# lh3/pangene

Measured on AMD Instinct MI355X. Metric: M PAF hits/sec through filter+overlap+graph, higher is better.
Workload: dtype int32

## Files before the change

include/pangene_hip.h:

```cpp
#ifndef PANGENE_HIP_H
#define PANGENE_HIP_H

#include <stddef.h>
#include <stdint.h>

#ifdef __cplusplus
extern "C" {
#endif

#define PGA_F_REV        0x001u
#define PGA_F_FLT        0x002u
#define PGA_F_ISO_SUB    0x004u
#define PGA_F_ISO_OV     0x008u
#define PGA_F_CHAIN      0x010u
#define PGA_F_PSEUDO     0x020u
#define PGA_F_VTX        0x040u
#define PGA_F_SHADOW     0x080u
#define PGA_F_REP        0x100u
#define PGA_F_WEAK_SHIFT 9
#define PGA_F_WEAK_MASK  0x600u

enum { PGA_FLT_PSEUDO = 0, PGA_FLT_VTX0 = 1, PGA_FLT_WEAK2 = 2, PGA_FLT_SHADOW = 3 };

enum {
	PGA_OK = 0,
	PGA_ERR_NO_DEVICE = -1,
	PGA_ERR_RANGE = -2,
	PGA_ERR_ARG = -3,
	PGA_ERR_NOMEM = -4,
	PGA_ERR_INVARIANT = -5
};

#define PGA_BLOCK_PLANES 10
typedef struct {
	int32_t n_hit, n_exon, n_ctg;
	int32_t max_cs, max_cm, max_score_adj;
	int32_t any_neg_score_adj, any_multi_exon;
	const int32_t *data;
	size_t n_words;
	const int32_t *vfirst;
	const int64_t *vbase;
} pga_genome_block_t;

#define PGA_ABI_VERSION 20u
typedef struct {
	uint32_t abi_version;
	int32_t n_genome;
	int32_t n_genome_global;
	const int32_t *genome_global;
	int32_t n_prot, n_gene;
	int64_t n_hit, n_exon;
	const pga_genome_block_t *block;
	const int32_t *prot_gid;
	const uint8_t *gene_pref;
} pga_shard_t;

typedef struct {
	double  min_ov_ratio;
	int32_t check_strand;
	int32_t drop_sgl_exon;
	int32_t reserved[4];
} pga_params_t;

typedef struct {
	uint32_t *flags;
	int32_t *rank, *score_dom, *pid_dom, *pid_dom0;
	int32_t *pos_x;
	int32_t *pos_y;
	uint64_t *flt_x_bits;
} pga_hit_state_t;

typedef struct {
	uint64_t x;
	int32_t  n_genome, tot_cnt;
	uint64_t sum_dist;
	int64_t  sum_s1, sum_s2;
} pga_arc_part_t;

typedef struct pga_ctx pga_ctx_t;

typedef struct {
	int64_t h1_head_tie;
	int64_t h2_cm_tie;
	int64_t h2_cs_tie;
	int64_t h3_dom_tie;
} pga_hazard_t;

#define PGA_HAZARD_CAP 4096

#define PGA_DECLARE(pfx) \
	 \
	int  pfx##_create(pga_ctx_t **ctx, const pga_shard_t *sh, const pga_params_t *par); \
	void pfx##_destroy(pga_ctx_t *ctx); \
	 \
	int  pfx##_begin(pga_ctx_t *ctx); \
	 \
	int  pfx##_ingest(pga_ctx_t *ctx, int32_t *stats); \
	 \
	int  pfx##_post_partials(pga_ctx_t *ctx, int32_t **max_ori, int64_t **sums); \
	 \
	int  pfx##_post_apply(pga_ctx_t *ctx, const uint8_t *prot_rep, const uint8_t *prot_pj, int64_t *n_pseudo); \
	 \
	int  pfx##_shadow(pga_ctx_t *ctx, int32_t cal_dom_sc, int32_t *stats); \
	 \
	int  pfx##_set_filter(pga_ctx_t *ctx, int32_t which); \
	 \
	int  pfx##_vtx_partials(pga_ctx_t *ctx, int32_t **cnt, uint64_t **records, int64_t *n_records); \
	 \
	int  pfx##_flag_vtx(pga_ctx_t *ctx, const int32_t *g2s, int32_t n_seg, int32_t then_filter); \
	 \
	int  pfx##_arc_round(pga_ctx_t *ctx, int32_t use_ori, int32_t **seg_cnt, pga_arc_part_t **arcs, int64_t *n_arcs); \
	 \
	int  pfx##_arc_merge(pga_ctx_t *ctx, const pga_arc_part_t *gathered, const int64_t *count, int32_t W, int64_t slot, \
	                     pga_arc_part_t **out, int64_t *n_out); \
	 \
	int  pfx##_arc_set_current(pga_ctx_t *ctx, const pga_arc_part_t *arcs, int64_t n_arc, int32_t n_seg, int32_t *deg); \
	 \
	int  pfx##_arc_round_local(pga_ctx_t *ctx, int32_t use_ori, int32_t n_seg, int32_t *seg_cnt, int32_t *deg); \
	int  pfx##_arc_round_finish(pga_ctx_t *ctx, int32_t n_seg, int32_t *seg_cnt, int32_t *deg);  \
	 \
	int  pfx##_arc_table(pga_ctx_t *ctx, const pga_arc_part_t **arcs, int64_t *n_arc); \
	 \
	int  pfx##_rep_pos(pga_ctx_t *ctx); \
	 \
	int  pfx##_n_local(pga_ctx_t *ctx, const int32_t *pairs, int64_t n, int32_t local_dist, int32_t local_count, \
	                   int32_t frag_mode, int32_t **cnt); \
	 \
	int  pfx##_branch_pairs(pga_ctx_t *ctx, const uint64_t *arc_x, const int32_t *arc_s1, int64_t n_arc, const int32_t *seg_gid, int32_t n_seg, \
	                        double branch_diff, int32_t local_dist, int32_t local_count, int32_t frag_mode, int32_t **cnt, int64_t *n_pairs); \
	int  pfx##_branch_decide(pga_ctx_t *ctx, double branch_diff, double branch_diff_dist, double branch_diff_cut, uint8_t *arc_weak, \
	                         int32_t *n_dist_loci, int64_t *n_flt1, int64_t *n_flt2); \
	 \
	int  pfx##_branch_decide_filter(pga_ctx_t *ctx, double branch_diff, double branch_diff_dist, double branch_diff_cut, int32_t do_filter, \
	                                int32_t max_tot_cnt, int32_t max_degree, int32_t max_dist_loci, uint8_t *del); \
	 \
	int  pfx##_mark_hits(pga_ctx_t *ctx, const uint64_t *arc_x, const uint8_t *arc_weak, int64_t n_arc, int64_t *n_marked, int32_t then_filter); \
	 \
	int  pfx##_override_order(pga_ctx_t *ctx, int32_t which, int32_t n_seg, const int32_t *seg_genome, const int32_t *seg_start, \
	                          const int64_t *seg_off, const int32_t *file_idx); \
	 \
	int  pfx##_set_head(pga_ctx_t *ctx, const int32_t *head_file); \
	 \
	int  pfx##_fetch(pga_ctx_t *ctx, void *dst_host, const void *src_backend, size_t nbytes); \
	int  pfx##_put(pga_ctx_t *ctx, void *dst_backend, const void *src_host, size_t nbytes); \
	int  pfx##_copy(pga_ctx_t *ctx, void *dst_backend, const void *src_backend, size_t nbytes); \
	 \
	int  pfx##_scratch(pga_ctx_t *ctx, size_t nbytes, void **ptr); \
	 \
	int  pfx##_sync(pga_ctx_t *ctx); \
	 \
	int  pfx##_fetch_later(pga_ctx_t *ctx, const void *src_backend, size_t nbytes, const void **host_view); \
	 \
	int  pfx##_ctg_counts(pga_ctx_t *ctx, int32_t *cnt); \
	int  pfx##_gene_matrix(pga_ctx_t *ctx, const int32_t *asm_of_ctg, int32_t n_asm, int32_t n_seg, int32_t *mat); \
	 \
	int  pfx##_download(pga_ctx_t *ctx, const pga_hit_state_t *out); \
	int  pfx##_hazards(pga_ctx_t *ctx, pga_hazard_t *out); \
	 \
	int  pfx##_hazard_segs(pga_ctx_t *ctx, int32_t *segs, int32_t cap, int64_t *n_total); \
	 \
	int  pfx##_is_device(void); \
	 \
	int  pfx##_host_alloc(size_t nbytes, void **ptr); \
	void pfx##_host_free(void *ptr); \
	const char *pfx##_strerror(int code);

PGA_DECLARE(pga)

typedef struct { int32_t bo, walk, st_off, en_off; } pga_call_rec_t;
typedef struct {
	const int32_t *step; const int64_t *walk_off; int32_t n_walk; int32_t n_seg;
	const int32_t *bub_vs, *bub_ve; int32_t n_bub;
} pga_call_in_t;
typedef struct {
	int64_t n_rec; const pga_call_rec_t *rec; const int32_t *rep, *cnt;
	int64_t n_gene; const int32_t *gene_bub, *gene_seg; const int64_t *gene_first;
} pga_call_out_t;
int pga_call_bubbles(const pga_call_in_t *in, pga_call_out_t *out);

typedef struct {
	const uint32_t *bits; const int32_t *order;
	int32_t n_gene, n_asm, n_perm;
} pga_curves_in_t;
typedef struct { const int32_t *count; } pga_curves_out_t;
int pga_pan_curves(const pga_curves_in_t *in, pga_curves_out_t *out);

typedef struct {
	const uint32_t *bits;
	int32_t n_item, n_asm;
} pga_shared_in_t;
typedef struct { const int32_t *shared; } pga_shared_out_t;
int pga_pan_shared(const pga_shared_in_t *in, pga_shared_out_t *out);

typedef struct {
	const uint32_t *bits;
	int32_t n_gene, n_asm, min_count, r_permille, sign;
	int64_t max_pair;
} pga_assoc_in_t;
typedef struct {
	int64_t n_pair;
	const int32_t *pair;
	const int32_t *count;
} pga_assoc_out_t;
int pga_pan_assoc(const pga_assoc_in_t *in, pga_assoc_out_t *out);

typedef struct {
	const uint32_t *bits;
	const uint32_t *label;
	int32_t n_gene, n_col, min_count, n_perm;
	uint32_t seed;
	uint32_t *perm_rows;
} pga_trait_in_t;
typedef struct { const int32_t *a, *s, *k; } pga_trait_out_t;
int pga_pan_trait(const pga_trait_in_t *in, pga_trait_out_t *out);
int32_t pga_trait_batch(void);

typedef struct {
	const int32_t *q;
	int32_t n, method;
} pga_join_in_t;
typedef struct { const int64_t *rec; int32_t n_rec; } pga_join_out_t;
int pga_pan_join(const pga_join_in_t *in, pga_join_out_t *out);

typedef struct {
	const uint32_t *bits;
	int32_t n_item, n_asm, metric, method;
	uint32_t seed;
	int32_t first, n_rep;
	int32_t *draws;
} pga_boot_in_t;
typedef struct { const int64_t *rec; int32_t n_rec; } pga_boot_out_t;
int pga_pan_boot(const pga_boot_in_t *in, pga_boot_out_t *out);
int32_t pga_boot_batch(int32_t n_asm);

typedef struct {
	const uint8_t *op;
	const uint32_t *bits;
	const int8_t *label;
	int32_t n_gene, n_leaf, n_row;
} pga_pairs_in_t;
typedef struct { const int32_t *out; } pga_pairs_out_t;
int pga_pan_pairs(const pga_pairs_in_t *in, pga_pairs_out_t *out);

typedef struct {
	const uint32_t *bits;
	const int16_t *c2;
	int32_t n_gene, n_col, min_count, n_perm;
	uint32_t seed;
	int16_t *perm_rows;
	int32_t *d_rows;
} pga_qtrait_in_t;
typedef struct { const int32_t *a, *d, *k; } pga_qtrait_out_t;
int pga_pan_qtrait(const pga_qtrait_in_t *in, pga_qtrait_out_t *out);
int32_t pga_qtrait_batch(void);

typedef struct {
	const int32_t *q;
	int32_t n, k, max_iter;
} pga_medoids_in_t;
typedef struct {
	const int32_t *medoid, *label, *dist, *size;
	const int64_t *sums, *rec;
	int64_t td;
	int32_t n_rec, n_swap, converged;
} pga_medoids_out_t;
int pga_pan_medoids(const pga_medoids_in_t *in, pga_medoids_out_t *out);

typedef struct {
	const int32_t *q;
	const uint32_t *label;
	int32_t n, shift, q_max, n1, n_perm;
	uint32_t seed;
	int64_t *a_rows, *b_rows;
	uint32_t *perm_rows;
} pga_permanova_in_t;
typedef struct { int64_t t, a, b, k; } pga_permanova_out_t;
int pga_pan_permanova(const pga_permanova_in_t *in, pga_permanova_out_t *out);
int32_t pga_permanova_batch(void);

typedef struct {
	const int32_t *a, *b;
	int32_t n, max_a, max_b, n_perm;
	uint32_t seed;
	int64_t *z_rows;
	uint16_t *ord_rows;
} pga_mantel_in_t;
typedef struct { int64_t z, n_ge, n_le; } pga_mantel_out_t;
int pga_pan_mantel(const pga_mantel_in_t *in, pga_mantel_out_t *out);
int32_t pga_mantel_batch(void);

typedef struct {
	const uint8_t *op;
	const uint32_t *bits;
	const int32_t *par;
	int32_t n_gene, n_leaf, gain, loss, mode;
	uint64_t *st_rows;
} pga_gainloss_in_t;
typedef struct { const int32_t *gene; const int64_t *node; } pga_gainloss_out_t;
int pga_pan_gainloss(const pga_gainloss_in_t *in, pga_gainloss_out_t *out);
int32_t pga_gainloss_chunk(int32_t n_leaf);

typedef struct {
	const uint8_t *op;
	const uint32_t *bits;
	const int32_t *par;
	int32_t n_gene, n_leaf, gain, loss, mode;
	int32_t min_events, r_permille, sign;
	int64_t max_pair;
	uint32_t *ev_rows;
	int64_t ev_cap;
} pga_coevo_in_t;
typedef struct { const int32_t *events; int64_t n_pair; const int32_t *pair; } pga_coevo_out_t;
int pga_pan_coevo(const pga_coevo_in_t *in, pga_coevo_out_t *out);
int32_t pga_coevo_chunk(int32_t n_leaf);

struct pga_branch_par_s; struct pga_loop_xchg_s;
typedef struct {
	const char *name;
	int  (*create)(pga_ctx_t **, const pga_shard_t *, const pga_params_t *);
	void (*destroy)(pga_ctx_t *);
	int  (*begin)(pga_ctx_t *);
	int  (*ingest)(pga_ctx_t *, int32_t *);
	int  (*post_partials)(pga_ctx_t *, int32_t **, int64_t **);
	int  (*post_apply)(pga_ctx_t *, const uint8_t *, const uint8_t *, int64_t *);
	int  (*shadow)(pga_ctx_t *, int32_t, int32_t *);
	int  (*set_filter)(pga_ctx_t *, int32_t);
	int  (*vtx_partials)(pga_ctx_t *, int32_t **, uint64_t **, int64_t *);
	int  (*flag_vtx)(pga_ctx_t *, const int32_t *, int32_t, int32_t);
	int  (*arc_round)(pga_ctx_t *, int32_t, int32_t **, pga_arc_part_t **, int64_t *);
	int  (*arc_merge)(pga_ctx_t *, const pga_arc_part_t *, const int64_t *, int32_t, int64_t, pga_arc_part_t **, int64_t *);
	int  (*arc_set_current)(pga_ctx_t *, const pga_arc_part_t *, int64_t, int32_t, int32_t *);
	int  (*rep_pos)(pga_ctx_t *);
	int  (*n_local)(pga_ctx_t *, const int32_t *, int64_t, int32_t, int32_t, int32_t, int32_t **);
	int  (*branch_pairs)(pga_ctx_t *, const uint64_t *, const int32_t *, int64_t, const int32_t *, int32_t, double, int32_t, int32_t, int32_t, int32_t **, int64_t *);
	int  (*branch_decide)(pga_ctx_t *, double, double, double, uint8_t *, int32_t *, int64_t *, int64_t *);
	int  (*mark_hits)(pga_ctx_t *, const uint64_t *, const uint8_t *, int64_t, int64_t *, int32_t);
	int  (*override_order)(pga_ctx_t *, int32_t, int32_t, const int32_t *, const int32_t *, const int64_t *, const int32_t *);
	int  (*set_head)(pga_ctx_t *, const int32_t *);
	int  (*fetch)(pga_ctx_t *, void *, const void *, size_t);
	int  (*put)(pga_ctx_t *, void *, const void *, size_t);
	int  (*copy)(pga_ctx_t *, void *, const void *, size_t);
	int  (*scratch)(pga_ctx_t *, size_t, void **);
	int  (*download)(pga_ctx_t *, const pga_hit_state_t *);
	int  (*hazards)(pga_ctx_t *, pga_hazard_t *);
	int  (*is_device)(void);
	const char *(*strerror)(int);
	int  (*timing_reset)(pga_ctx_t *);
	int  (*timing_get)(pga_ctx_t *, int32_t, double *, int64_t *, int64_t *);
	int  (*sync)(pga_ctx_t *);
	int  (*fetch_later)(pga_ctx_t *, const void *, size_t, const void **);
	int  (*hazard_segs)(pga_ctx_t *, int32_t *, int32_t, int64_t *);
	int  (*host_alloc)(size_t, void **);
	void (*host_free)(void *);
	int  (*arc_round_local)(pga_ctx_t *, int32_t, int32_t, int32_t *, int32_t *);
	int  (*ctg_counts)(pga_ctx_t *, int32_t *);
	int  (*gene_matrix)(pga_ctx_t *, const int32_t *, int32_t, int32_t, int32_t *);
	int  (*arc_table)(pga_ctx_t *, const pga_arc_part_t **, int64_t *);
	int  (*arc_round_finish)(pga_ctx_t *, int32_t, int32_t *, int32_t *);
	int  (*branch_decide_filter)(pga_ctx_t *, double, double, double, int32_t, int32_t, int32_t, int32_t, uint8_t *);
	int  (*branch_loop)(pga_ctx_t *, int32_t, const struct pga_branch_par_s *, const int32_t *, const int32_t *, const int32_t *, uint8_t *, const struct pga_loop_xchg_s *, int32_t *, int32_t *);
	void (*host_trim)(size_t);
	int  (*set_device)(int32_t);
	int  (*device_count)(void);
	int  (*arc_round_x)(pga_ctx_t *, int32_t, int32_t, const struct pga_loop_xchg_s *, int32_t *, int32_t *, int64_t *);
	int  (*copy_gbps)(size_t, int32_t, double *);
	int  (*warm)(void);
	int  (*reserve)(int64_t, int64_t, int32_t, int32_t, int32_t, int64_t);
	int  (*stage)(const void *, size_t);
	void (*stage_drop)(const void *);
	int  (*call_bubbles)(const pga_call_in_t *, pga_call_out_t *);
	int  (*pan_curves)(const pga_curves_in_t *, pga_curves_out_t *);
	int  (*pan_shared)(const pga_shared_in_t *, pga_shared_out_t *);
	int  (*pan_assoc)(const pga_assoc_in_t *, pga_assoc_out_t *);
	int  (*pan_trait)(const pga_trait_in_t *, pga_trait_out_t *);
	int  (*pan_join)(const pga_join_in_t *, pga_join_out_t *);
	int  (*pan_boot)(const pga_boot_in_t *, pga_boot_out_t *);
	int  (*pan_pairs)(const pga_pairs_in_t *, pga_pairs_out_t *);
	int  (*pan_qtrait)(const pga_qtrait_in_t *, pga_qtrait_out_t *);
	int  (*pan_medoids)(const pga_medoids_in_t *, pga_medoids_out_t *);
	int  (*pan_permanova)(const pga_permanova_in_t *, pga_permanova_out_t *);
	int  (*pan_mantel)(const pga_mantel_in_t *, pga_mantel_out_t *);
	int  (*final_arcs)(pga_ctx_t *, const void **, int64_t *);
	int  (*pan_gainloss)(const pga_gainloss_in_t *, pga_gainloss_out_t *);
	int  (*pan_coevo)(const pga_coevo_in_t *, pga_coevo_out_t *);
} pga_backend_t;

const pga_backend_t *pga_backend(void);

typedef struct pga_loop_xchg_s {
	void *user;
	int32_t rank, world;
	int64_t arc_cap_hint;
	int (*allreduce_i32_sum)(void *user, void *buf, int64_t count);
	int (*allgather)(void *user, const void *in, void *out, int64_t bytes_per_rank);
} pga_loop_xchg_t;
void pga_host_trim(size_t keep_bytes);
int pga_set_device(int32_t device);
int pga_device_count(void);
int pga_copy_gbps(size_t bytes, int32_t reps, double *gbps);
int pga_warm(void);

typedef struct pga_branch_par_s {
	double branch_diff, branch_diff_dist, branch_diff_cut; int32_t local_dist, local_count, frag_mode, use_ori;
	int32_t pre_on, pre_max_tot_cnt, pre_max_degree, pre_max_dist_loci;
	int32_t final_on;
} pga_branch_par_t;
int pga_arc_round_x(pga_ctx_t *ctx, int32_t use_ori, int32_t n_seg, const pga_loop_xchg_t *x, int32_t *seg_cnt, int32_t *deg, int64_t *n_arc);
int pga_branch_loop(pga_ctx_t *ctx, int32_t n_round, const pga_branch_par_t *par, const int32_t *max_tot_cnt, const int32_t *max_degree,
                    const int32_t *max_dist_loci, uint8_t *seg_alive, const pga_loop_xchg_t *x, int32_t *seg_cnt , int32_t *n_dist_loci );

int pga_final_arcs(pga_ctx_t *ctx, const void **host_view, int64_t *n_arc);

int pga_set_stream(pga_ctx_t *ctx, void *hip_stream);
void *pga_active_stream(void);

int pga_reserve(int64_t n_hit, int64_t n_exon, int32_t n_prot, int32_t n_gene, int32_t n_genome, int64_t raw_words);
int pga_stage_h2d(const void *host, size_t bytes);
void pga_stage_drop(const void *host);
int pga_timing_reset(pga_ctx_t *ctx);
int pga_timing_get(pga_ctx_t *ctx, int32_t which, double *total_ms, int64_t *n_launch, int64_t *units);

#ifdef __cplusplus
}
#endif
#endif
```

pangene_amd/csrc/hip/k_stage_b.hpp:

```cpp
#pragma once

__global__ __launch_bounds__(BLOCK) void k_post_part(const uint32_t *flags, const int32_t *pid, const int32_t *rank, const int32_t *sori, const int32_t *sadj,
                                                       const int32_t *nex, int n, int P, int32_t *max_ori, unsigned long long *sums)
{
	int h = blockIdx.x * BLOCK + threadIdx.x;
	if (h >= n) return;
	int p = pid[h];
	const int so = sori[h];
	if (max_ori[p] < so) atomicMax(&max_ori[p], so);
	if (rank[h] == 0 && !(flags[h] & PGA_F_FLT)) {
		int w = nex[h] == 1 ? 0 : 1;
		atomicAdd(&sums[p], (unsigned long long)(long long)sadj[h]);
		atomicAdd(&sums[(int64_t)(2 + w) * P + p], 1ull);
		atomicAdd(&sums[(int64_t)(4 + w) * P + p], (unsigned long long)(long long)sori[h]);
	}
}
constexpr int PP_T = 1024;
__global__ __launch_bounds__(PP_T) void k_post_part_lds(const uint32_t *flags, const int32_t *pid, const int32_t *rank, const int32_t *sori, const int32_t *sadj,
                                                          const int32_t *nex, int n, int P, int p_tiles, int PT , int32_t *max_ori, unsigned long long *sums)
{
	extern __shared__ unsigned long long pp_lds[];
	unsigned long long *s_adj = pp_lds, *s_o0 = pp_lds + PT, *s_o1 = pp_lds + 2 * (size_t)PT;
	unsigned int *s_cnt = (unsigned int *)(pp_lds + 3 * (size_t)PT);
	const int t = blockIdx.x % p_tiles, chunk = blockIdx.x / p_tiles, n_chunk = gridDim.x / p_tiles;
	const int p0 = t * PT, p1 = p0 + PT < P ? p0 + PT : P;
	for (int i = threadIdx.x; i < PT; i += PP_T) s_adj[i] = 0, s_o0[i] = 0, s_o1[i] = 0, s_cnt[i] = 0;
	__syncthreads();
	const int64_t per = ((int64_t)n + n_chunk - 1) / n_chunk, h0 = (int64_t)chunk * per, h1 = h0 + per < n ? h0 + per : n;
	for (int64_t h = h0 + threadIdx.x; h < h1; h += PP_T) {
		const int p = pid[h], so = sori[h];
		if (t == 0 && max_ori[p] < so) atomicMax(&max_ori[p], so);
		if (p < p0 || p >= p1 || rank[h] != 0 || (flags[h] & PGA_F_FLT)) continue;
		const int w = nex[h] == 1 ? 0 : 1, i = p - p0;
		atomicAdd(&s_adj[i], (unsigned long long)(long long)sadj[h]);
		{
			const unsigned old = atomicAdd(&s_cnt[i], w ? 65536u : 1u);
			if ((w ? old >> 16 : old & 0xffffu) == 0x7fffu) { atomicAdd(&sums[(int64_t)(2 + w) * P + p], 0x8000ull); atomicSub(&s_cnt[i], w ? 0x80000000u : 0x8000u); }
		}
		atomicAdd(w ? &s_o1[i] : &s_o0[i], (unsigned long long)(long long)so);
	}
	__syncthreads();
	for (int i = threadIdx.x; i < p1 - p0; i += PP_T) {
		const unsigned int cw = s_cnt[i];
		const unsigned long long a = s_adj[i], o0 = s_o0[i], o1 = s_o1[i];
		const int p = p0 + i;
		if (a) atomicAdd(&sums[p], a);
		if (cw & 0xffffu) atomicAdd(&sums[(int64_t)2 * P + p], (unsigned long long)(cw & 0xffffu));
		if (cw >> 16) atomicAdd(&sums[(int64_t)3 * P + p], (unsigned long long)(cw >> 16));
		if (o0) atomicAdd(&sums[(int64_t)4 * P + p], o0);
		if (o1) atomicAdd(&sums[(int64_t)5 * P + p], o1);
	}
}
__global__ __launch_bounds__(BLOCK) void k_post_count(unsigned long long *sums, int P)
{
	const int p = blockIdx.x * BLOCK + threadIdx.x;
	if (p < P) sums[(int64_t)P + p] = sums[(int64_t)2 * P + p] + sums[(int64_t)3 * P + p];
}

__global__ __launch_bounds__(BLOCK) void k_post_apply(uint32_t *flags, const int32_t *pid, const int32_t *nex, int32_t *sdom, int n,
                                                        const int32_t *max_ori, const uint8_t *rep, const uint8_t *pj, int64_t *cnt)
{
	int h = blockIdx.x * BLOCK + threadIdx.x;
	if (h >= n) return;
	int p = pid[h];
	int mo = max_ori[p];
	if (sdom[h] > mo) sdom[h] = mo;
	uint32_t f = flags[h], nf = rep[p] ? (f | PGA_F_REP) : (f & ~PGA_F_REP);
	if (!(f & (PGA_F_FLT | PGA_F_PSEUDO)) && nex[h] == 1 && pj[p]) {
		nf |= PGA_F_PSEUDO;
		if (cnt) atomicAdd((unsigned long long *)cnt, 1ull);
	}
	if (nf != f) flags[h] = nf;
}

__global__ __launch_bounds__(BLOCK) void k_set_filter(uint32_t *flags, int n, int which)
{
	int h = blockIdx.x * BLOCK + threadIdx.x;
	if (h >= n) return;
	uint32_t f = flags[h];
	bool hit = which == PGA_FLT_PSEUDO ? (f & PGA_F_PSEUDO) != 0
	         : which == PGA_FLT_VTX0 ? (f & PGA_F_VTX) == 0
	         : which == PGA_FLT_WEAK2 ? ((f & PGA_F_WEAK_MASK) >> PGA_F_WEAK_SHIFT) == 2
	         : (f & PGA_F_SHADOW) != 0;
	if (hit && !(f & PGA_F_FLT)) flags[h] = f | PGA_F_FLT;
}
```

pangene_amd/csrc/hip/pga_backend.hip:

```cpp
#include <hip/hip_runtime.h>
#include <hip/hip_ext.h>
#include <stdint.h>
#include <stdio.h>
#include <string.h>
#include <time.h>
#include <vector>
#include <mutex>
#include <atomic>
#include <condition_variable>
#include <algorithm>
#include "pangene_hip.h"
#include "dev_prims.hpp"

using namespace pgd;

#define HIPCHK(x) do { hipError_t e_ = (x); if (e_ != hipSuccess) { \
	fprintf(stderr, "[E::pga] %s:%d: %s\n", __FILE__, __LINE__, hipGetErrorString(e_)); return PGA_ERR_NO_DEVICE; } } while (0)

static bool env_has(const char *name, const char *word)
{
	const char *e = getenv(name);
	const size_t n = strlen(word);
	for (; e && *e; ) { const char *c = strchr(e, ','); const size_t len = c ? (size_t)(c - e) : strlen(e); if (len == n && strncmp(e, word, n) == 0) return true; e = c ? c + 1 : nullptr; }
	return false;
}
static long long xloop_cap(int which)
{
	const char *e = getenv("PANGENE_XLOOP_CAP");
	if (!e) return 0;
	if (which == 0) return atoll(e);
	const char *c = strchr(e, ',');
	return c ? atoll(c + 1) : 0;
}
static bool poison_on() { static const bool f = getenv("PANGENE_POISON") != nullptr; return f; }

#define F_HEAD 0x80000000u
#define F_MULTI 0x40000000u
#define F_CSTIE 0x20000000u
#define F_MEMBER 0x10000000u
#define F_PUBLIC 0x7ffu

#include "pga_host_context.hpp"

extern "C" int pga_is_device(void) { return 1; }

extern "C" int pga_host_alloc(size_t nbytes, void **ptr)
{
	*ptr = nullptr;
	return hipHostMalloc(ptr, nbytes ? nbytes : 1, hipHostMallocDefault) == hipSuccess ? 0 : PGA_ERR_NOMEM;
}
extern "C" void pga_host_free(void *ptr) { if (ptr) (void)hipHostFree(ptr); }

extern "C" int pga_set_device(int32_t device) { if (hipSetDevice(device) != hipSuccess) return PGA_ERR_NO_DEVICE; g_last_dev.store(device); return 0; }
extern "C" int pga_device_count(void) { int n = 0; return hipGetDeviceCount(&n) == hipSuccess ? n : 0; }

static void pan_release_all();

extern "C" void pga_host_trim(size_t keep_bytes)
{
	if (keep_bytes == 0) {
		pan_release_all();
		std::lock_guard<std::mutex> lk(g_dev_mu);
		for (DevBlock &b : g_dev_cache) (void)hipFree(b.p);
		g_dev_cache.clear();
	}
	std::lock_guard<std::mutex> lk(g_pin_mu);
	size_t kept = 0, n_keep = 0;
	for (; n_keep < g_pin_cache.size() && kept + g_pin_cache[n_keep].cap <= keep_bytes; ++n_keep) kept += g_pin_cache[n_keep].cap;
	for (size_t i = n_keep; i < g_pin_cache.size(); ++i) (void)hipHostFree(g_pin_cache[i].p);
	g_pin_cache.resize(n_keep);
}

extern "C" const char *pga_strerror(int code)
{
	switch (code) {
	case PGA_OK: return "ok";
	case PGA_ERR_NO_DEVICE: return "no usable HIP device / HIP runtime error (this library has no CPU fallback)";
	case PGA_ERR_RANGE: return "value out of range for the device layout";
	case PGA_ERR_ARG: return "bad argument";
	case PGA_ERR_NOMEM: return "out of device memory";
	case PGA_ERR_INVARIANT: return "reference invariant violated";
	}
	return "unknown";
}

#include "k_common.hpp"
#include "k_perm.hpp"
#include "k_ingest.hpp"
#include "k_sweep.hpp"
#include "k_segsort.hpp"
#include "k_stage_b.hpp"
#include "k_vertex.hpp"
#include "k_arcs.hpp"
#include "k_branch.hpp"
#include "k_genes.hpp"
#include "k_order.hpp"
#include "k_call.hpp"
#include "k_curves.hpp"
#include "k_dist.hpp"
#include "k_assoc.hpp"
#include "k_trait.hpp"
#include "k_qtrait.hpp"
#include "k_permanova.hpp"
#include "k_mantel.hpp"
#include "k_join.hpp"
#include "k_medoids.hpp"
#include "k_boot.hpp"
#include "k_pairs.hpp"
#include "k_gainloss.hpp"
#include "k_coevo.hpp"
#include "pga_host_common.hpp"
#include "pga_host_stage_a.hpp"
#include "pga_host_stage_b.hpp"
#include "pga_host_arcs.hpp"
#include "pga_host_branch.hpp"
#include "pga_host_order.hpp"
#include "pga_host_io.hpp"
#include "pga_host_call.hpp"
#include "pga_host_pan.hpp"
#include "pga_host_curves.hpp"
#include "pga_host_dist.hpp"
#include "pga_host_assoc.hpp"
#include "pga_host_trait.hpp"
#include "pga_host_qtrait.hpp"
#include "pga_host_permanova.hpp"
#include "pga_host_mantel.hpp"
#include "pga_host_join.hpp"
#include "pga_host_medoids.hpp"
#include "pga_host_boot.hpp"
#include "pga_host_pairs.hpp"
#include "pga_host_gainloss.hpp"
#include "pga_host_coevo.hpp"

extern "C" const pga_backend_t *pga_backend(void)
{
	static const pga_backend_t b = {
		"hip-gfx950", pga_create, pga_destroy, pga_begin, pga_ingest, pga_post_partials, pga_post_apply, pga_shadow, pga_set_filter,
		pga_vtx_partials, pga_flag_vtx, pga_arc_round, pga_arc_merge, pga_arc_set_current, pga_rep_pos, pga_n_local, pga_branch_pairs, pga_branch_decide, pga_mark_hits, pga_override_order, pga_set_head, pga_fetch, pga_put, pga_copy, pga_scratch,
		pga_download, pga_hazards, pga_is_device, pga_strerror, pga_timing_reset, pga_timing_get, pga_sync, pga_fetch_later, pga_hazard_segs, pga_host_alloc, pga_host_free, pga_arc_round_local, pga_ctg_counts, pga_gene_matrix, pga_arc_table, pga_arc_round_finish, pga_branch_decide_filter, pga_branch_loop, pga_host_trim, pga_set_device, pga_device_count, pga_arc_round_x, pga_copy_gbps, pga_warm, pga_reserve, pga_stage_h2d, pga_stage_drop, pga_call_bubbles, pga_pan_curves, pga_pan_shared, pga_pan_assoc, pga_pan_trait, pga_pan_join, pga_pan_boot, pga_pan_pairs,
		pga_pan_qtrait, pga_pan_medoids, pga_pan_permanova, pga_pan_mantel, pga_final_arcs, pga_pan_gainloss, pga_pan_coevo
	};
	return &b;
}
#include "pga_host_selftest.hpp"
```

pangene_amd/csrc/hip/pga_host_common.hpp:

```cpp
#pragma once


static int sync_st(pga_ctx *c)
{
	static const bool poll = [] { const char *e = getenv("PANGENE_WAIT"); return !(e && strcmp(e, "sync") == 0); }();
	++c->sync_epoch;
	if (poll) {
		timespec t0; clock_gettime(CLOCK_MONOTONIC, &t0);
		for (unsigned long long it = 1;; ++it) {
			const hipError_t e = hipStreamQuery(c->st);
			if (e == hipSuccess) return 0;
			if (e != hipErrorNotReady) HIPCHK(e);
			__builtin_ia32_pause();
			if ((it & 0x3f) == 0) {
				timespec t; clock_gettime(CLOCK_MONOTONIC, &t);
				if ((t.tv_sec - t0.tv_sec) + (t.tv_nsec - t0.tv_nsec) * 1e-9 > 200e-6) break;
			}
		}
	}
	HIPCHK(hipStreamSynchronize(c->st));
	return 0;
}

static int bits_for(uint32_t maxv) { int b = 1; while (b < 32 && (maxv >> b)) ++b; return b; }

static int make_sweep_view(pga_ctx *c, SweepView *v)
{
	v->A = c->recA, v->B = c->recB, v->C = c->recC, v->sori = c->sori, v->exon = c->exon, v->flags = c->flags, v->pdom = c->pdom, v->sdom = c->sdom, v->pdom0 = c->pdom0;
	v->n = c->N, v->min_ov = c->par.min_ov_ratio, v->check_strand = c->par.check_strand, v->hz = c->dcnt + 4, v->stage_c = c->any_multi;
	v->init_dom = c->sweep_init ? 1 : 0;
	v->literal = c->exon_regular && getenv("PANGENE_MERGE_LITERAL") == nullptr ? 0 : 1;
	v->gate = c->gate;
	v->xmap = nullptr;
	v->slow_cnt = nullptr, v->slow_list = (int32_t *)c->pool.get(S_SLOW, sizeof(int32_t) * (size_t)c->N);
	v->hz_list = (int32_t *)c->pool.get(S_HZLIST, sizeof(int32_t) * PGA_HAZARD_CAP);
	if (!v->slow_list || !v->hz_list) return PGA_ERR_NOMEM;
	return 0;
}

constexpr int SW_LEAN_BELOW = 1024;
static int measure_list_density(pga_ctx *c)
{
	c->density_known = true;
	if (c->N == 0) return 0;
	const char *e = getenv("PANGENE_SWEEP_LISTS");
	if (e && (strcmp(e, "lds") == 0 || strcmp(e, "global") == 0)) { c->lists_in_lds = e[0] == 'l'; return 0; }
	const int nt = (int)nblk(c->N, SW_TILE), stride = std::max(1, nt / 256), ns = (nt + stride - 1) / stride;
	HIPCHK(hipMemsetAsync(c->dcnt + 16, 0, sizeof(int64_t), c->st));
	hipLaunchKernelGGL(k_list_density, dim3(ns), dim3(SW_TILE), 0, c->st, c->recA, c->recC, c->N, stride, c->dcnt + 16);
	HIPCHK(hipMemcpyAsync(c->h_cnt + 16, c->dcnt + 16, sizeof(int64_t), hipMemcpyDeviceToHost, c->st));
	{ const int rc = sync_st(c); if (rc) return rc; }
	c->lists_in_lds = c->h_cnt[16] >= (int64_t)SW_LEAN_BELOW * ns, c->list_density = (double)c->h_cnt[16] / ns, c->density_tiles = ns;
	if (getenv("PANGENE_TIMING")) fprintf(stderr, "[pga] exon lists of the sweeps: %.0f a tile to stage (%d tiles sampled) -> %s\n", (double)c->h_cnt[16] / ns, ns, c->lists_in_lds ? "LDS (k_sweep)" : "global memory (k_sweep_lean)");
	return 0;
}

static void pack_records(pga_ctx *c)
{
	if (c->N) hipLaunchKernelGGL(k_pack_rec, dim3(nblk(c->N)), dim3(BLOCK), 0, c->st, c->seg, c->cs, c->ce, c->pm, c->rk, c->gid, c->cds, c->rank, c->nex, c->offx,
	                             c->pid, c->sori, c->N, c->recA, c->recB, c->recC, c->flags);
}

template <int MODE> static int launch_sweep(pga_ctx *c, int timed_which)
{
	SweepView v;
	if (c->N == 0) return 0;
	{ const int rc = make_sweep_view(c, &v); if (rc) return rc; }
	TimedLaunch t; t.which = timed_which; t.units = c->N;
	constexpr int reps = 1;
	static_assert(MODE == 0 || MODE == 1 || MODE == 3, "sweep modes");
	static const bool no_compact = env_has("PANGENE_LIVE", "fullsweep");
	if (MODE == 0 && c->live_on && c->z_valid && !no_compact) v.A = c->cA, v.B = c->cB, v.C = c->cC, v.n = c->NL, v.xmap = c->cx;
	const int n_sw = v.n;
	const bool timed = (timed_which == 0 || timed_which == 1) && c->timing_on;
	if (timed) {
		HIPCHK(hipEventCreate(&t.a)); HIPCHK(hipEventCreate(&t.b));
		if (reps != 1) HIPCHK(hipEventRecord(t.a, c->st));
	}
	c->walk_valid = false, c->ha_valid = false, c->shadow_queued = false;
	const int nt = std::max(1, (int)nblk(n_sw, SW_TILE));
	v.prof = nullptr; v.dbg = 0;
#ifdef PGA_SW_PROFILE
	{ const char *e = getenv("PGA_SW_DBG"); v.dbg = e ? atoi(e) : 0; }
	HIPCHK(hipMalloc((void **)&v.prof, sizeof(long long) * SW_NSTAMP * SW_NW * (size_t)nt)); HIPCHK(hipMemset(v.prof, 0, sizeof(long long) * SW_NSTAMP * SW_NW * (size_t)nt));
#endif
	for (int rep = 0; rep < reps; ++rep) {
		v.slow_cnt = c->dcnt + 12 + (c->sweep_seq & 1);
		hipEvent_t ea = timed && reps == 1 ? t.a : nullptr, eb = timed && reps == 1 ? t.b : nullptr;
		if (c->any_multi && MODE != 0 && !c->lists_in_lds) hipExtLaunchKernelGGL((k_sweep_lean<MODE == 0 ? 1 : MODE>), dim3(nt), dim3(SW_TILE), 0, c->st, ea, eb, 0, v);
		else if (c->any_multi) hipExtLaunchKernelGGL((k_sweep<MODE, true>), dim3(nt), dim3(SW_TILE), 0, c->st, ea, eb, 0, v);
		else hipExtLaunchKernelGGL((k_sweep<MODE, false>), dim3(nt), dim3(SW_TILE), 0, c->st, ea, eb, 0, v);
		hipLaunchKernelGGL((k_sweep_slow<MODE>), dim3((unsigned)std::min<int64_t>(2 * c->n_cu, std::max<int64_t>(64, nblk(n_sw)))), dim3(BLOCK), 0, c->st, v, (long long *)(c->dcnt + 12 + ((c->sweep_seq + 1) & 1)), MODE == 0 ? c->ga_ctl : (int32_t *)nullptr);
		++c->sweep_seq;
	}
#ifdef PGA_SW_PROFILE
	{
		std::vector<long long> hp((size_t)SW_NSTAMP * SW_NW * nt);
		HIPCHK(hipStreamSynchronize(c->st));
		HIPCHK(hipMemcpy(hp.data(), v.prof, hp.size() * sizeof(long long), hipMemcpyDeviceToHost));
		(void)hipFree(v.prof);
		double d[SW_NSTAMP] = { 0 };
		for (size_t w = 0; w < (size_t)SW_NW * nt; ++w)
			for (int k = 1; k < 10; ++k) { const long long x = hp[w * SW_NSTAMP + k], y = hp[w * SW_NSTAMP + k - 1]; if (x && y) d[k] += (double)(x - y); }
		const double q = 1.0 / ((double)SW_NW * nt);
		{ double mx = 0, sm = 0; for (size_t w = 0; w < (size_t)SW_NW * nt; ++w) mx += (double)hp[w * SW_NSTAMP + 10], sm += (double)hp[w * SW_NSTAMP + 11]; fprintf(stderr, "[sweep<%d> epilogue merges: steps of the longest lane %.1f, of all lanes %.1f per wave]\n", MODE, mx * q, sm * q); }
		fprintf(stderr, "[sweep<%d> profile, n %d, ticks/wave] records->LDS %.0f | barrier %.0f | want+scan %.0f | barrier+offsets+sources %.0f | barrier+gather %.0f | barrier %.0f | runs %.0f | list+eval %.0f | finish %.0f\n", MODE, c->N,
		        d[1] * q, d[2] * q, d[3] * q, d[4] * q, d[5] * q, d[6] * q, d[7] * q, d[8] * q, d[9] * q);
	}
#endif
	if (timed) {
		if (reps != 1) HIPCHK(hipEventRecord(t.b, c->st));
		c->timed.push_back(t);
	}
	return 0;
}

static int radix_sort_pool(pga_ctx *c, uint64_t *keys, uint32_t *vals, int64_t n, int n_bits, uint64_t **kres, uint32_t **vres)
{
	RadixBufs b;
	if (n > std::max<int64_t>(2 * (int64_t)c->N + 2, (int64_t)c->P + 2)) return PGA_ERR_ARG;
	b.k_alt = (uint64_t *)c->pool.get(S_KEY_B, 0);
	b.v_alt = (uint32_t *)c->pool.get(S_VAL_B, 0);
	b.table = (uint32_t *)c->pool.get(S_TABLE, 0);
	b.tile_buf = (int32_t *)c->pool.get(S_TILE, tile_buf_bytes(n));
	if (!b.k_alt || !b.v_alt || !b.table || !b.tile_buf) return PGA_ERR_NOMEM;
	device_radix_sort(keys, vals, n, n_bits, b, kres, vres, c->st);
	return 0;
}

extern "C" void pga_destroy(pga_ctx_t *c)
{
	if (c == nullptr) return;
	if (c->st) (void)hipStreamSynchronize(c->st);
	if (getenv("PANGENE_TIMING")) {
		size_t n_own = 0, b_own = 0;
		for (size_t i = 0; i < c->pool.p.size(); ++i) if (c->pool.p[i] && c->pool.own[i]) ++n_own, b_own += c->pool.cap[i];
		fprintf(stderr, "[pga_destroy] %d hits: temporaries used %.1f of %.1f MB of their arena, %zu slots (%.1f MB) had to be allocated on their own\n",
		        c->N, c->pool.arena_off / 1048576.0, c->pool.arena_cap / 1048576.0, n_own, b_own / 1048576.0);
	}
	for (auto &t : c->timed) { (void)hipEventDestroy(t.a); (void)hipEventDestroy(t.b); }
	if (c->span_a) (void)hipEventDestroy(c->span_a);
	for (void *q : c->owned) (void)hipFree(q);
	dev_big_free(c->arena, c->arena_cap), c->arena = nullptr;
	c->pool.release();
	for (int k = 0; k < 2; ++k) if (c->ov_ev[k]) { (void)hipEventDestroy(c->ov_ev[k]); c->ov_ev[k] = nullptr; }
	c->pin.release();
	if (c->g2s_done) (void)hipEventDestroy(c->g2s_done);
	if (c->z_ev) (void)hipEventDestroy(c->z_ev);
	if (c->own_stream && c->st) (void)hipStreamDestroy(c->st);
	delete c;
}

static hipStream_t g_active_stream = nullptr;

extern "C" void *pga_active_stream(void) { return (void *)g_active_stream; }

extern "C" int pga_set_stream(pga_ctx_t *c, void *hip_stream)
{
	if (c == nullptr) return PGA_ERR_ARG;
	if (c->st) HIPCHK(hipStreamSynchronize(c->st));
	if (c->own_stream && c->st) (void)hipStreamDestroy(c->st);
	c->st = (hipStream_t)hip_stream, c->own_stream = false;
	g_active_stream = c->st;
	return 0;
}

static void zero_multi(pga_ctx *c, void *p0, size_t b0, void *p1 = nullptr, size_t b1 = 0, void *p2 = nullptr, size_t b2 = 0, void *p3 = nullptr, size_t b3 = 0)
{
	ZeroList z = { { p0, p1, p2, p3 }, { (b0 + 3) / 4, (b1 + 3) / 4, (b2 + 3) / 4, (b3 + 3) / 4 } };
	const unsigned long long tot = z.dwords[0] + z.dwords[1] + z.dwords[2] + z.dwords[3];
	if (tot) hipLaunchKernelGGL(k_zero_multi, dim3((unsigned)((tot + BLOCK - 1) / BLOCK)), dim3(BLOCK), 0, c->st, z);
}

template <class T> static int upload(pga_ctx *c, T *dst, const T *src, size_t n)
{
	if (n == 0) return 0;
	HIPCHK(hipMemcpyAsync(dst, src, n * sizeof(T), hipMemcpyHostToDevice, c->st));
	return 0;
}

#define TRY(x) do { int rc_ = (x); if (rc_) return rc_; } while (0)

static int stage_upload(pga_ctx *c, void *d0, const void *s0, size_t n0, void *d1 = nullptr, const void *s1 = nullptr, size_t n1 = 0);
```

pangene_amd/csrc/hip/pga_host_context.hpp:

```cpp
#pragma once


static inline size_t tile_buf_bytes(int64_t n) { return std::max<size_t>(sizeof(int64_t) * (size_t)(scan_tiles(std::max<int64_t>(rs_table_len(n), n)) + 8), 256 * sizeof(uint32_t) + 64); }

static inline unsigned nblk(int64_t n, int per = BLOCK) { return (unsigned)((n + per - 1) / per); }

struct DevBlock { void *p; size_t cap; int dev; };
static std::atomic<int> g_last_dev{-1};
static int cur_dev() { int d = 0; return hipGetDevice(&d) == hipSuccess ? d : 0; }
static std::mutex g_dev_mu;
static std::vector<DevBlock> g_dev_cache;
static std::condition_variable g_dev_cv; static int g_dev_reserving = 0;
static bool dev_cache_on() { static const bool on = [] { const char *e = getenv("PANGENE_DEV_CACHE"); return !(e && *e == '0'); }(); return on; }

static void *dev_big_alloc(size_t want, size_t *got)
{
	{
		std::unique_lock<std::mutex> lk(g_dev_mu);
		g_dev_cv.wait(lk, [] { return g_dev_reserving == 0; });
		size_t best = (size_t)-1;
		const int dev = cur_dev();
		for (size_t i = 0; i < g_dev_cache.size(); ++i)
			if (g_dev_cache[i].dev == dev && g_dev_cache[i].cap >= want && g_dev_cache[i].cap <= 2 * want + ((size_t)64 << 20) && (best == (size_t)-1 || g_dev_cache[i].cap < g_dev_cache[best].cap)) best = i;
		if (best != (size_t)-1) {
			DevBlock b = g_dev_cache[best];
			g_dev_cache.erase(g_dev_cache.begin() + (long)best);
			*got = b.cap;
			return b.p;
		}
	}
	void *q = nullptr;
	if (dev_cache_on() && want >= ((size_t)1 << 20)) {
		const size_t padded = (want + want / 8 + ((size_t)64 << 20) - 1) & ~(((size_t)64 << 20) - 1);
		if (hipMalloc(&q, padded) == hipSuccess) { *got = padded; return q; }
		(void)hipGetLastError(), q = nullptr;
	}
	if (hipMalloc(&q, want) != hipSuccess) {
		(void)hipGetLastError();
		{
			std::lock_guard<std::mutex> lk(g_dev_mu);
			for (DevBlock &b : g_dev_cache) (void)hipFree(b.p);
			g_dev_cache.clear();
		}
		if (hipMalloc(&q, want) != hipSuccess) { (void)hipGetLastError(); return nullptr; }
	}
	*got = want;
	return q;
}

static void dev_big_free(void *p, size_t cap)
{
	if (p == nullptr) return;
	if (dev_cache_on() && cap >= ((size_t)1 << 20)) {
		std::lock_guard<std::mutex> lk(g_dev_mu);
		if (g_dev_cache.size() >= 2) {
			size_t small = 0;
			for (size_t i = 1; i < g_dev_cache.size(); ++i) if (g_dev_cache[i].cap < g_dev_cache[small].cap) small = i;
			if (g_dev_cache[small].cap >= cap) { (void)hipFree(p); return; }
			(void)hipFree(g_dev_cache[small].p);
			g_dev_cache.erase(g_dev_cache.begin() + (long)small);
		}
		g_dev_cache.push_back(DevBlock{p, cap, cur_dev()});
		return;
	}
	(void)hipFree(p);
}

struct DevPool {
	std::vector<void *> p; std::vector<size_t> cap; std::vector<char> own;
	char *arena = nullptr; size_t arena_cap = 0, arena_off = 0;
	void *get(int slot, size_t bytes)
	{
		if ((int)p.size() <= slot) p.resize(slot + 1, nullptr), cap.resize(slot + 1, 0), own.resize(slot + 1, 0);
		if (bytes == 0) bytes = 16;
		if (cap[slot] < bytes) {
			if (p[slot] && own[slot]) (void)hipFree(p[slot]);
			size_t want = (bytes + bytes / 4 + 256 + 255) & ~(size_t)255;
			if (arena && arena_off + want <= arena_cap) { p[slot] = arena + arena_off, arena_off += want, own[slot] = 0; }
			else if (hipMalloc(&p[slot], want) == hipSuccess) { own[slot] = 1; if (poison_on()) (void)hipMemset(p[slot], 0x5a, want); }
			else { p[slot] = nullptr; cap[slot] = 0; own[slot] = 0; return nullptr; }
			cap[slot] = want;
		}
		return p[slot];
	}
	void release()
	{
		for (size_t i = 0; i < p.size(); ++i) if (p[i] && own[i]) (void)hipFree(p[i]);
		dev_big_free(arena, arena_cap);
		p.clear(); cap.clear(); own.clear(); arena = nullptr; arena_cap = arena_off = 0;
	}
};

struct PinBlock { char *p; size_t cap; };
static std::mutex g_pin_mu;
static std::vector<PinBlock> g_pin_cache;
struct PinArena {
	std::vector<PinBlock> blocks; size_t off = 0;
	void *get(size_t bytes)
	{
		bytes = (bytes + 255) & ~(size_t)255;
		if (blocks.empty() || off + bytes > blocks.back().cap) {
			PinBlock b = { nullptr, 0 };
			{
				std::lock_guard<std::mutex> lk(g_pin_mu);
				for (size_t i = 0; i < g_pin_cache.size(); ++i)
					if (g_pin_cache[i].cap >= bytes) { b = g_pin_cache[i]; g_pin_cache.erase(g_pin_cache.begin() + (long)i); break; }
			}
			if (b.p == nullptr) {
				b.cap = std::max<size_t>(bytes, (size_t)8 << 20);
				if (hipHostMalloc((void **)&b.p, b.cap, hipHostMallocDefault) != hipSuccess) return nullptr;
			}
			blocks.push_back(b), off = 0;
		}
		void *r = blocks.back().p + off;
		off += bytes;
		if (poison_on()) memset(r, 0x5a, bytes);
		return r;
	}
	void release()
	{
		std::lock_guard<std::mutex> lk(g_pin_mu);
		for (PinBlock &b : blocks) { if (g_pin_cache.size() < 16) g_pin_cache.push_back(b); else (void)hipHostFree(b.p); }
		blocks.clear(), off = 0;
	}
};

enum {
	S_KEY_A, S_KEY_B, S_VAL_A, S_VAL_B, S_TABLE, S_TILE, S_I32_A, S_I32_B, S_I32_C, S_TAB_A, S_TAB_B, S_TAB_C, S_TAB_D,
	S_TDIST, S_TS1, S_TS2, S_TGEN, S_SDIST, S_SS1, S_SS2, S_SGEN, S_HEAD, S_SLOT, S_ARCS, S_SEGCNT, S_BITS, S_TRIPLES,
	S_WALK_VAL, S_WALK_PREV, S_PERM, S_OVPOS, S_OVFILE, S_RUNSTART, S_CDN, S_MG_KEY, S_MG_VAL, S_MG_SRC, S_MG_OUT, S_MG_HEAD, S_MG_SLOT, S_MG_RUN, S_BR_S1, S_BR_GID, S_BR_VS, S_BR_VE, S_BR_PC, S_BR_POFF, S_BR_GRP, S_BR_NDL, S_BR_SEGGID, S_PAIRS, S_NLCNT, S_ARCX, S_ARCW, S_WEAKNEW, S_RP_SEG, S_RP_R, S_RP_CM, S_RP_POS, S_RP_IV, S_DL, S_SCRATCH, S_UPLOAD, S_RAW, S_ARC_STAGE, S_GMETA, S_GOFF, S_DEG, S_BIGLIST, S_STAGE_SID, S_STATS, S_G2S, S_MISC, S_SLOW, S_HZLIST, S_VWK, S_XG_BUF, S_XG_OUT, S_XG_OUT2, S_XSTAT, S_GSLIST, S_UPLOAD2, S_BINS, S_FIN_ID,
	S_COUNT
};

constexpr int LIVE_CNT_N = 1024;
struct TimedLaunch { hipEvent_t a, b; int which; int64_t units; };

struct pga_ctx {
	hipStream_t st = nullptr; bool own_stream = false;
	int32_t n_genome = 0, n_genome_global = 0, P = 0, Q = 0, n_seg_ctg = 0;
	int32_t N = 0, E = 0;
	int n_cu = 256;
	uint32_t sweep_seq = 0;
	pga_params_t par;
	std::vector<int32_t> h_goff, h_ggl;
	int32_t *fidx = 0, *gnm = 0, *seg = 0, *pid = 0, *gid = 0, *cs = 0, *ce = 0, *cm = 0, *cds = 0, *nex = 0, *offx = 0, *sori = 0, *sadj = 0, *pm = 0;
	int32_t *rk = 0;
	int sc_bits = 64;
	int rk_shift = -1;
	int32_t *hrank = 0;
	bool any_multi = true;
	bool exon_regular = true;
	double list_density = 0; int64_t density_tiles = 0;
	bool lists_in_lds = true, density_known = false;
	int rp_form = 0;
	int32_t *vfirst = 0; int64_t *vbase = 0;
	int4 *recA = 0, *recB = 0, *recC = 0;
	int32_t *rank = 0, *sdom = 0, *pdom = 0, *pdom0 = 0; uint32_t *flags = 0;
	int32_t *yperm = 0, *goff = 0, *ggl = 0, *ctg_base = 0, *inv = 0, *headpos = 0, *eoff = 0; int64_t *woff = 0;
	int cs_bits = 1, cm_bits = 1, seg_bits = 1, ctg_bits = 1;
	bool inv_valid = false;
	bool sweep_init = false;
	bool bin_on = false; int32_t *up_grouped = nullptr; int4 *bins = nullptr; int bin_n_small = 0, bin_n_big = 0, bin_np_small = 64, bin_np_big = 64, bin_ctg_bits = 1;
	bool gs_ok = false; int gs_np = 64; int32_t *gs_list = nullptr; int gs_n[3] = { 0, 0, 0 }, gs_np_of[3] = { 64, 64, 64 };
	int2 *exon = 0; int32_t *prot_gid = 0; uint8_t *gene_pref = 0;
	int32_t *max_ori = 0; int64_t *sums = 0; int32_t *vtx_cnt = 0; int32_t *g2s = 0; int32_t n_seg = 0;
	uint64_t sync_epoch_reset = 0;
	bool gf_ok = false;
	bool gf_k32 = false; int gf_pos_bits = 0;
	bool x_redo = false;
	int64_t x_pairs_seen = 0, x_arcs_seen = 0;
	int64_t x_pairs_run = 0, x_arcs_run = 0;
	int64_t x_pair_floor = 0, x_arc_floor = 0;
	int64_t *dcnt = 0;
	int64_t *h_cnt = 0;
	int64_t *h_box = 0;
	void *h_stage = nullptr; size_t h_stage_cap = 0;
	void *h_fetch = nullptr; size_t h_fetch_cap = 0;
	int32_t *h_g2s = nullptr; size_t h_g2s_cap = 0; hipEvent_t g2s_done = nullptr;
	DevPool pool; PinArena pin;
	bool walk_valid = false;
	int32_t *zx = 0, *zy = 0, *zg = 0; int2 *zst = 0; int32_t *zpos = 0, *zoff = 0;
	bool live_on = false;
	int32_t NL = 0;
	int32_t *lx = 0;
	int32_t *ylist_buf = 0;
	const int32_t *ylist = 0;
	bool z_early = false; hipEvent_t z_ev = nullptr;
	int32_t *ga_ctl = 0;
	int4 *cA = 0, *cB = 0, *cC = 0; int32_t *cx = 0;
	int2 *tg = 0; bool tg_valid = false;
	int64_t *live_cnt = 0;
	int64_t live_hint = -1;
	int4 *wrec = 0; bool wrec_valid = false;
	uint32_t *hfk = 0, *hbk = 0; int4 *hfp = 0, *hbp = 0;
	bool z_valid = false, ha_valid = false; uint32_t round_tag = 0; int ha_ori = -1;
	Gate gate = Gate{nullptr, 0};
	int32_t *loopctl = nullptr;
	int loop_round = 0;
	bool in_loop = false;
	bool loop_room_given = false;
	bool loop_gated = false;
	int32_t *h_loopctl = nullptr;
	int32_t *h_ov = nullptr; size_t h_ov_cap = 0;
	hipEvent_t ov_ev[2] = { nullptr, nullptr }; bool ov_ev_used[2] = { false, false }; unsigned ov_seq = 0;
	bool zposy_stale = false;
	const pga_arc_part_t *cur_tab = nullptr; int64_t cur_tab_n = 0;
	bool table_sparse = false;
	int32_t *h_round = nullptr; size_t h_round_cap = 0;
	void *h_fin = nullptr; int64_t h_fin_cap = 0, fin_cap = 0, fin_n = 0; bool fin_on = false;
	int ride_want = 0, ride_cpg = 1, ride_done = 0; uint32_t ride_tag = 0;
	bool shadow_queued = false;
	unsigned long long sync_epoch = 0, arc_epoch = 0; bool arc_deferred = false, arc_done = false, force_sort_once = false, sweep_done = false; std::vector<int32_t> def_host;
	int4 *yrecA = 0, *yrecB = 0; bool yrec_valid = false;
	int64_t br_np_seen = 0;
	int64_t br_n = 0, br_np = 0, br_cap = 0; int32_t br_S = 0;
	struct { double diff; int32_t local_dist, local_count, frag_mode; } br_par = { 0, 0, 0, 0 };
	int32_t *h_ndl = nullptr; size_t h_ndl_cap = 0;
	std::vector<TimedLaunch> timed; bool timing_on = false;
	bool timing_rounds = false;
	hipEvent_t span_a = nullptr;
	std::vector<void *> owned; void *arena = nullptr; size_t arena_cap = 0;
	std::vector<std::pair<void **, size_t>> plan;
};

template <class T> static int dalloc(pga_ctx *c, T **p, size_t n)
{
	c->plan.emplace_back((void **)p, (((n ? n : 1) * sizeof(T)) + 255) & ~(size_t)255);
	return 0;
}

static int dalloc_commit(pga_ctx *c)
{
	size_t tot = 0;
	if (getenv("PANGENE_NO_ARENA")) {
		for (auto &e : c->plan) { void *q = nullptr; if (hipMalloc(&q, e.second) != hipSuccess) return PGA_ERR_NOMEM; *e.first = q; c->owned.push_back(q); if (poison_on()) (void)hipMemset(q, 0x5a, e.second); }
		c->plan.clear();
		return 0;
	}
	for (auto &e : c->plan) tot += e.second;
	size_t got = 0;
	void *base = dev_big_alloc(tot ? tot : 256, &got);
	if (base == nullptr) return PGA_ERR_NOMEM;
	c->arena = base, c->arena_cap = got;
	if (poison_on()) (void)hipMemset(base, 0x5a, tot ? tot : 256);
	size_t off = 0;
	for (auto &e : c->plan) *e.first = (char *)base + off, off += e.second;
	c->plan.clear();
	return 0;
}
```

pangene_amd/csrc/hip/pga_host_selftest.hpp:

```cpp
#pragma once


extern "C" int pga_selftest_sort(uint64_t *keys, uint32_t *vals, int64_t n, int32_t n_bits)
{
	int ndev = 0;
	if (hipGetDeviceCount(&ndev) != hipSuccess || ndev <= 0) return PGA_ERR_NO_DEVICE;
	uint64_t *ka, *kb; uint32_t *va, *vb, *table; int32_t *tile;
	HIPCHK(hipMalloc((void **)&ka, sizeof(uint64_t) * (size_t)(n + 1))); HIPCHK(hipMalloc((void **)&kb, sizeof(uint64_t) * (size_t)(n + 1)));
	HIPCHK(hipMalloc((void **)&va, sizeof(uint32_t) * (size_t)(n + 1))); HIPCHK(hipMalloc((void **)&vb, sizeof(uint32_t) * (size_t)(n + 1)));
	HIPCHK(hipMalloc((void **)&table, sizeof(uint32_t) * (size_t)(rs_table_len(n) + 1)));
	HIPCHK(hipMalloc((void **)&tile, tile_buf_bytes(n)));
	HIPCHK(hipMemcpy(ka, keys, sizeof(uint64_t) * (size_t)n, hipMemcpyHostToDevice));
	HIPCHK(hipMemcpy(va, vals, sizeof(uint32_t) * (size_t)n, hipMemcpyHostToDevice));
	RadixBufs b = { kb, vb, table, tile };
	uint64_t *kr; uint32_t *vr;
	device_radix_sort(ka, va, n, n_bits, b, &kr, &vr, 0);
	HIPCHK(hipDeviceSynchronize());
	HIPCHK(hipMemcpy(keys, kr, sizeof(uint64_t) * (size_t)n, hipMemcpyDeviceToHost));
	HIPCHK(hipMemcpy(vals, vr, sizeof(uint32_t) * (size_t)n, hipMemcpyDeviceToHost));
	(void)hipFree(ka); (void)hipFree(kb); (void)hipFree(va); (void)hipFree(vb); (void)hipFree(table); (void)hipFree(tile);
	return 0;
}

extern "C" int pga_selftest_merge(const pga_arc_part_t *gathered, const int64_t *count, int32_t W, int64_t slot_sz, pga_arc_part_t *out, int64_t *n_out)
{
	int ndev = 0;
	if (hipGetDeviceCount(&ndev) != hipSuccess || ndev <= 0) return PGA_ERR_NO_DEVICE;
	pga_ctx c;
	HIPCHK(hipStreamCreateWithFlags(&c.st, hipStreamNonBlocking));
	TRY(dalloc(&c, &c.dcnt, 16)); TRY(dalloc_commit(&c));
	HIPCHK(hipHostMalloc((void **)&c.h_cnt, 16 * sizeof(int64_t), hipHostMallocDefault));
	pga_arc_part_t *dg = nullptr, *res = nullptr;
	HIPCHK(hipMalloc((void **)&dg, sizeof(pga_arc_part_t) * (size_t)(W * slot_sz + 1)));
	HIPCHK(hipMemcpy(dg, gathered, sizeof(pga_arc_part_t) * (size_t)(W * slot_sz), hipMemcpyHostToDevice));
	int rc = pga_arc_merge(&c, dg, count, W, slot_sz, &res, n_out);
	if (rc == 0 && *n_out) rc = hipMemcpyAsync(out, res, sizeof(pga_arc_part_t) * (size_t)*n_out, hipMemcpyDeviceToHost, c.st) == hipSuccess ? 0 : PGA_ERR_NO_DEVICE;
	(void)hipStreamSynchronize(c.st);
	(void)hipFree(dg); (void)hipFree(c.dcnt); (void)hipHostFree(c.h_cnt);
	c.pool.release();
	(void)hipStreamDestroy(c.st);
	return rc;
}

__device__ __forceinline__ int64_t cal_perm(int64_t i, int64_t n, int64_t window)
{
	const int64_t base = i & ~(window - 1), span = base + window <= n ? window : 0;
	return span ? base + (((i - base) * 40503 + 12345) & (window - 1)) : i;
}
__global__ __launch_bounds__(BLOCK) void k_cal_read16(const int4 *__restrict__ src, int64_t n, int32_t *sink)
{
	int acc = 0;
	for (int64_t i = (int64_t)blockIdx.x * BLOCK + threadIdx.x; i < n; i += (int64_t)gridDim.x * BLOCK) { const int4 v = src[i]; acc ^= v.x ^ v.y ^ v.z ^ v.w; }
	if (acc == 0x7fffffff) sink[0] = acc;
}
__global__ __launch_bounds__(BLOCK) void k_cal_read4(const int32_t *__restrict__ src, int64_t n, int32_t *sink)
{
	int acc = 0;
	for (int64_t i = (int64_t)blockIdx.x * BLOCK + threadIdx.x; i < n; i += (int64_t)gridDim.x * BLOCK) acc ^= src[i];
	if (acc == 0x7fffffff) sink[0] = acc;
}
__global__ __launch_bounds__(BLOCK) void k_cal_gather4(const int32_t *__restrict__ src, int64_t n, int64_t window, int32_t *sink)
{
	int acc = 0;
	for (int64_t i = (int64_t)blockIdx.x * BLOCK + threadIdx.x; i < n; i += (int64_t)gridDim.x * BLOCK) acc ^= src[cal_perm(i, n, window)];
	if (acc == 0x7fffffff) sink[0] = acc;
}
__global__ __launch_bounds__(BLOCK) void k_cal_gather16(const int4 *__restrict__ src, int64_t n, int64_t window, int32_t *sink)
{
	int acc = 0;
	for (int64_t i = (int64_t)blockIdx.x * BLOCK + threadIdx.x; i < n; i += (int64_t)gridDim.x * BLOCK) { const int4 v = src[cal_perm(i, n, window)]; acc ^= v.x ^ v.w; }
	if (acc == 0x7fffffff) sink[0] = acc;
}
__global__ __launch_bounds__(BLOCK) void k_cal_write16(int4 *__restrict__ dst, int64_t n)
{
	for (int64_t i = (int64_t)blockIdx.x * BLOCK + threadIdx.x; i < n; i += (int64_t)gridDim.x * BLOCK) dst[i] = make_int4((int)i, 1, 2, 3);
}
__global__ __launch_bounds__(BLOCK) void k_cal_write4(int32_t *__restrict__ dst, int64_t n)
{
	for (int64_t i = (int64_t)blockIdx.x * BLOCK + threadIdx.x; i < n; i += (int64_t)gridDim.x * BLOCK) dst[i] = (int)i;
}
__global__ __launch_bounds__(BLOCK) void k_cal_scatter4(int32_t *__restrict__ dst, int64_t n, int64_t window)
{
	for (int64_t i = (int64_t)blockIdx.x * BLOCK + threadIdx.x; i < n; i += (int64_t)gridDim.x * BLOCK) dst[cal_perm(i, n, window)] = (int)i;
}
__global__ __launch_bounds__(BLOCK) void k_cal_scatter16(int4 *__restrict__ dst, int64_t n, int64_t window)
{
	for (int64_t i = (int64_t)blockIdx.x * BLOCK + threadIdx.x; i < n; i += (int64_t)gridDim.x * BLOCK) dst[cal_perm(i, n, window)] = make_int4((int)i, 1, 2, 3);
}

extern "C" int pga_selftest_traffic(int64_t n, int64_t window)
{
	int ndev = 0;
	if (hipGetDeviceCount(&ndev) != hipSuccess || ndev <= 0) return PGA_ERR_NO_DEVICE;
	if (n < 1024) return PGA_ERR_ARG;
	if (window <= 0) { window = 1; while (window * 2 <= n) window *= 2; }
	if (window & (window - 1)) return PGA_ERR_ARG;
	int4 *a = nullptr, *b = nullptr; int32_t *sink = nullptr;
	HIPCHK(hipMalloc((void **)&a, sizeof(int4) * (size_t)n)); HIPCHK(hipMalloc((void **)&b, sizeof(int4) * (size_t)n)); HIPCHK(hipMalloc((void **)&sink, 256));
	HIPCHK(hipMemset(a, 1, sizeof(int4) * (size_t)n)); HIPCHK(hipMemset(b, 2, sizeof(int4) * (size_t)n));
	HIPCHK(hipDeviceSynchronize());
	const unsigned grid = (unsigned)std::min<int64_t>((n + BLOCK - 1) / BLOCK, (int64_t)256 * 64);
	hipLaunchKernelGGL(k_cal_read16, dim3(grid), dim3(BLOCK), 0, 0, (const int4 *)a, n, sink);
	hipLaunchKernelGGL(k_cal_read4, dim3(grid), dim3(BLOCK), 0, 0, (const int32_t *)b, n, sink);
	hipLaunchKernelGGL(k_cal_gather4, dim3(grid), dim3(BLOCK), 0, 0, (const int32_t *)a, n, window, sink);
	hipLaunchKernelGGL(k_cal_gather16, dim3(grid), dim3(BLOCK), 0, 0, (const int4 *)b, n, window, sink);
	hipLaunchKernelGGL(k_cal_write16, dim3(grid), dim3(BLOCK), 0, 0, a, n);
	hipLaunchKernelGGL(k_cal_write4, dim3(grid), dim3(BLOCK), 0, 0, (int32_t *)b, n);
	hipLaunchKernelGGL(k_cal_scatter4, dim3(grid), dim3(BLOCK), 0, 0, (int32_t *)a, n, window);
	hipLaunchKernelGGL(k_cal_scatter16, dim3(grid), dim3(BLOCK), 0, 0, b, n, window);
	HIPCHK(hipDeviceSynchronize());
	(void)hipFree(a); (void)hipFree(b); (void)hipFree(sink);
	return 0;
}

extern "C" int pga_selftest_scan(const int32_t *in, const int32_t *seg, int32_t *out, int64_t n, int32_t mode)
{
	int ndev = 0;
	if (hipGetDeviceCount(&ndev) != hipSuccess || ndev <= 0) return PGA_ERR_NO_DEVICE;
	int32_t *di, *ds, *dout; int64_t *tile;
	HIPCHK(hipMalloc((void **)&di, sizeof(int32_t) * (size_t)(n + 1))); HIPCHK(hipMalloc((void **)&ds, sizeof(int32_t) * (size_t)(n + 1)));
	HIPCHK(hipMalloc((void **)&dout, sizeof(int32_t) * (size_t)(n + 1))); HIPCHK(hipMalloc((void **)&tile, sizeof(int64_t) * (size_t)(scan_tiles(n) + 8)));
	HIPCHK(hipMemcpy(di, in, sizeof(int32_t) * (size_t)n, hipMemcpyHostToDevice));
	if (seg) HIPCHK(hipMemcpy(ds, seg, sizeof(int32_t) * (size_t)n, hipMemcpyHostToDevice));
	if (mode == 0) device_scan<I32>(InI32{di}, OutExclI32{dout}, n, (I32 *)tile, OpSum{}, I32{0}, 0);
	else if (mode == 1) device_scan<I32>(InI32{di}, OutExclI32{dout}, n, (I32 *)tile, OpMax{}, I32{-1}, 0);
	else device_scan<SegMax>(InSegMax{ds, di}, OutSegMax{dout}, n, (SegMax *)tile, OpSegMax{}, SegMax{SEG_EMPTY, 0}, 0);
	HIPCHK(hipDeviceSynchronize());
	HIPCHK(hipMemcpy(out, dout, sizeof(int32_t) * (size_t)n, hipMemcpyDeviceToHost));
	(void)hipFree(di); (void)hipFree(ds); (void)hipFree(dout); (void)hipFree(tile);
	return 0;
}

typedef struct {
	int32_t *recA, *recB, *recC;
	uint32_t *flags;
	int32_t *fidx, *gnm, *yperm;
	int32_t *headpos;
	uint32_t f_head, f_multi, f_cstie;
	int32_t route;
	int32_t n_unit[3];
	int32_t n_cu;
} pga_selftest_stage_a_t;
extern "C" int pga_selftest_stage_a(pga_ctx_t *c, pga_selftest_stage_a_t *out)
{
	if (c == nullptr || out == nullptr) return PGA_ERR_ARG;
	TRY(sync_st(c));
	const size_t N = (size_t)c->N, GL = (size_t)c->n_genome;
	auto fetch = [&](void *dst, const void *src, size_t bytes) { return (dst == nullptr || bytes == 0 || hipMemcpy(dst, src, bytes, hipMemcpyDeviceToHost) == hipSuccess) ? 0 : PGA_ERR_NO_DEVICE; };
	TRY(fetch(out->recA, c->recA, sizeof(int4) * N)); TRY(fetch(out->recB, c->recB, sizeof(int4) * N)); TRY(fetch(out->recC, c->recC, sizeof(int4) * N));
	TRY(fetch(out->flags, c->flags, sizeof(uint32_t) * N));
	TRY(fetch(out->fidx, c->fidx, sizeof(int32_t) * N)); TRY(fetch(out->gnm, c->gnm, sizeof(int32_t) * N)); TRY(fetch(out->yperm, c->yperm, sizeof(int32_t) * N));
	if (N) TRY(fetch(out->headpos, c->headpos, sizeof(int32_t) * (GL + 1)));
	out->f_head = F_HEAD, out->f_multi = F_MULTI, out->f_cstie = F_CSTIE;
	out->route = c->bin_on ? 2 : c->gs_ok ? 1 : 0, out->n_cu = c->n_cu;
	for (int k = 0; k < 3; ++k) out->n_unit[k] = out->route == 1 ? c->gs_n[k] : 0;
	if (out->route == 2) out->n_unit[0] = c->bin_n_small, out->n_unit[1] = c->bin_n_big;
	return 0;
}

extern "C" int pga_selftest_arc_final(const pga_arc_part_t *in, int64_t n, int32_t *out)
{
	int ndev = 0;
	if (hipGetDeviceCount(&ndev) != hipSuccess || ndev <= 0) return PGA_ERR_NO_DEVICE;
	if (n <= 0 || in == nullptr || out == nullptr) return PGA_ERR_ARG;
	pga_arc_part_t *di; int4 *dout;
	HIPCHK(hipMalloc((void **)&di, sizeof(pga_arc_part_t) * (size_t)n)); HIPCHK(hipMalloc((void **)&dout, sizeof(int4) * (size_t)n));
	HIPCHK(hipMemcpy(di, in, sizeof(pga_arc_part_t) * (size_t)n, hipMemcpyHostToDevice));
	hipLaunchKernelGGL(k_arc_final_probe, dim3(nblk(n)), dim3(BLOCK), 0, 0, (const pga_arc_part_t *)di, n, dout);
	HIPCHK(hipDeviceSynchronize());
	HIPCHK(hipMemcpy(out, dout, sizeof(int4) * (size_t)n, hipMemcpyDeviceToHost));
	(void)hipFree(di); (void)hipFree(dout);
	return 0;
}
```

pangene_amd/csrc/hip/pga_host_stage_b.hpp:

```cpp
#pragma once


extern "C" int pga_post_partials(pga_ctx_t *c, int32_t **max_ori, int64_t **sums)
{
	zero_multi(c, c->max_ori, sizeof(int32_t) * (size_t)std::max(1, c->P), c->sums, sizeof(int64_t) * 6 * (size_t)std::max(1, c->P));
	static const bool pp_atomics = env_has("PANGENE_POST", "atomics");
	static const bool pp_force = env_has("PANGENE_POST", "lds");
	bool lds_done = false;
	if (c->N && c->P && !pp_atomics && (c->N >= (1 << 19) || pp_force)) {
		const size_t room = (size_t)144 << 10;
		const int p_tiles = (size_t)c->P * 28 <= room ? 1 : (size_t)((c->P + 1) / 2) * 28 <= room ? 2 : 0;
		if (p_tiles) {
			const int PT = (c->P + p_tiles - 1) / p_tiles;
			const size_t lds = (size_t)PT * 28 + 16;
			static size_t lds_set = 0;
			bool ok = true;
			if (lds > lds_set) { ok = hipFuncSetAttribute(reinterpret_cast<const void *>(k_post_part_lds), hipFuncAttributeMaxDynamicSharedMemorySize, (int)lds) == hipSuccess; if (ok) lds_set = lds; else (void)hipGetLastError(); }
			if (ok) {
				const int n_chunk = (int)std::max<int64_t>(1, std::min<int64_t>(c->n_cu, c->N / 32768));
				hipLaunchKernelGGL(k_post_part_lds, dim3((unsigned)(n_chunk * p_tiles)), dim3(PP_T), lds, c->st, c->flags, c->pid, c->rank, c->sori, c->sadj, c->nex, c->N, c->P, p_tiles, PT,
				                   c->max_ori, (unsigned long long *)c->sums);
				lds_done = true;
			}
		}
	}
	if (c->N && !lds_done) hipLaunchKernelGGL(k_post_part, dim3(nblk(c->N)), dim3(BLOCK), 0, c->st, c->flags, c->pid, c->rank, c->sori, c->sadj, c->nex, c->N, c->P,
	                             c->max_ori, (unsigned long long *)c->sums);
	if (c->N && c->P) hipLaunchKernelGGL(k_post_count, dim3(nblk(c->P)), dim3(BLOCK), 0, c->st, (unsigned long long *)c->sums, c->P);
	*max_ori = c->max_ori, *sums = c->sums;
	return 0;
}

extern "C" int pga_post_apply(pga_ctx_t *c, const uint8_t *prot_rep, const uint8_t *prot_pj, int64_t *n_pseudo)
{
	c->yrec_valid = false, c->wrec_valid = false;
	uint8_t *d = (uint8_t *)c->pool.get(S_MISC, 2 * (size_t)c->P + 16);
	if (!d) return PGA_ERR_NOMEM;
	c->walk_valid = false, c->ha_valid = false;
	TRY(stage_upload(c, d, prot_rep, (size_t)c->P, d + c->P, prot_pj, (size_t)c->P));
	if (n_pseudo) HIPCHK(hipMemsetAsync(c->dcnt + 2, 0, sizeof(int64_t), c->st));
	if (c->N) hipLaunchKernelGGL(k_post_apply, dim3(nblk(c->N)), dim3(BLOCK), 0, c->st, c->flags, c->pid, c->nex, c->sdom, c->N, c->max_ori, d, d + c->P, n_pseudo ? c->dcnt + 2 : (int64_t *)nullptr);
	if (n_pseudo) {
		HIPCHK(hipMemcpyAsync(c->h_cnt, c->dcnt, 16 * sizeof(int64_t), hipMemcpyDeviceToHost, c->st));
		TRY(sync_st(c));
		*n_pseudo = c->h_cnt[2];
	}
	return 0;
}

extern "C" int pga_shadow(pga_ctx_t *c, int32_t cal_dom_sc, int32_t *stats)
{
	c->yrec_valid = false, c->wrec_valid = false;
	if (cal_dom_sc) TRY(launch_sweep<1>(c, -1)); else TRY(launch_sweep<0>(c, 2));
	if (stats) {
		int32_t *d_stats = (int32_t *)c->pool.get(S_STATS, sizeof(int32_t) * 4 * (size_t)c->n_genome + 16);
		if (!d_stats) return PGA_ERR_NOMEM;
		HIPCHK(hipMemsetAsync(d_stats, 0, sizeof(int32_t) * 2 * (size_t)c->n_genome + 16, c->st));
		if (c->N) hipLaunchKernelGGL(k_count_shadow, dim3(nblk(c->N)), dim3(BLOCK), 0, c->st, c->flags, c->gnm, c->N, d_stats);
		HIPCHK(hipMemcpyAsync(stats, d_stats, sizeof(int32_t) * 2 * (size_t)c->n_genome, hipMemcpyDeviceToHost, c->st));
		return sync_st(c);
	}
	return 0;
}

extern "C" int pga_set_filter(pga_ctx_t *c, int32_t which)
{
	if (which < 0 || which > 3) return PGA_ERR_ARG;
	const bool queued = c->shadow_queued;
	c->shadow_queued = false;
	if (queued && which == PGA_FLT_SHADOW) return 0;
	c->walk_valid = false, c->ha_valid = false;
	if (c->N) hipLaunchKernelGGL(k_set_filter, dim3(nblk(c->N)), dim3(BLOCK), 0, c->st, c->flags, c->N, which);
	return 0;
}

static int check_invariant(pga_ctx *c, bool flushed = false)
{
	if (!flushed) hipLaunchKernelGGL(k_mail_flush, dim3(1), dim3(64), 0, c->st, c->dcnt, c->h_box);
	TRY(sync_st(c));
	return c->h_cnt[3] ? PGA_ERR_INVARIANT : 0;
}

extern "C" int pga_vtx_partials(pga_ctx_t *c, int32_t **cnt, uint64_t **records, int64_t *n_records)
{
	const int N = c->N, Q = c->Q, GL = c->n_genome;
	const int64_t wpg = (Q + 31) / 32, n_slot = (int64_t)std::max(1, Q) * VTX_K;
	const int nw = (c->n_genome_global + 63) / 64;
	static const long long first_cap = [] { const char *e = getenv("PANGENE_VTX_SPILL_CAP"); return e && atoll(e) > 0 ? atoll(e) : 65536ll; }();
	long long ovf_cap = first_cap;
	uint32_t *bits = (uint32_t *)c->pool.get(S_BITS, sizeof(uint32_t) * (size_t)(wpg * GL) + 16);
	if (!bits) return PGA_ERR_NOMEM;
	*n_records = 0, *cnt = c->vtx_cnt;
	for (int attempt = 0;; ++attempt) {
		const size_t b_tab = sizeof(int32_t) * (size_t)n_slot, b_bits = sizeof(uint64_t) * (size_t)n_slot * (size_t)nw, b_rec = sizeof(uint64_t) * (size_t)(n_slot + ovf_cap) * (size_t)(1 + nw);
		char *blk = (char *)c->pool.get(S_TRIPLES, 2 * b_tab + b_bits + b_rec + 64);
		if (!blk) return PGA_ERR_NOMEM;
		int32_t *dom_tab = (int32_t *)blk, *slot = (int32_t *)(blk + b_tab);
		unsigned long long *pbits = (unsigned long long *)(blk + 2 * b_tab), *rec = (unsigned long long *)(blk + 2 * b_tab + b_bits);
		zero_multi(c, bits, sizeof(uint32_t) * (size_t)(wpg * GL) + 16, c->vtx_cnt, sizeof(int32_t) * 2 * (size_t)std::max(1, Q), c->dcnt, sizeof(int64_t), pbits, b_bits);
		HIPCHK(hipMemsetAsync(dom_tab, 0xff, b_tab, c->st));
		HIPCHK(hipMemsetAsync(c->live_cnt, 0, sizeof(int64_t) * LIVE_CNT_N, c->st));
		*records = (uint64_t *)rec;
		if (N == 0) return sync_st(c);
		{
			static const bool vx_atomics = env_has("PANGENE_POST", "atomics"), vx_force = env_has("PANGENE_POST", "lds");
			const size_t lds = sizeof(int) * 2 * (size_t)std::max(1, Q);
			static size_t lds_set = 0;
			bool ok = !vx_atomics && (N >= (1 << 19) || vx_force) && lds <= ((size_t)144 << 10);
			if (ok && lds > lds_set) { ok = hipFuncSetAttribute(reinterpret_cast<const void *>(k_vtx1_lds), hipFuncAttributeMaxDynamicSharedMemorySize, (int)lds) == hipSuccess; if (ok) lds_set = lds; else (void)hipGetLastError(); }
			if (ok) {
				const int n_chunk = (int)std::max<int64_t>(1, std::min<int64_t>(2 * c->n_cu, N / 32768));
				hipLaunchKernelGGL(k_vtx1_lds, dim3((unsigned)n_chunk), dim3(VX_T), lds, c->st, c->flags, c->gnm, c->gid, c->rank, c->pdom, N, Q, c->vtx_cnt, bits, wpg, c->dcnt, c->live_cnt);
			} else
			hipLaunchKernelGGL(k_vtx1, dim3(nblk(N)), dim3(BLOCK), 0, c->st, c->flags, c->gnm, c->gid, c->rank, c->pdom, N, Q, c->vtx_cnt, bits, wpg, c->dcnt, c->live_cnt);
		}
		hipLaunchKernelGGL(k_live_sum, dim3(1), dim3(BLOCK), 0, c->st, (const int64_t *)c->live_cnt, c->dcnt);
		hipLaunchKernelGGL(k_vtx_fold, dim3(nblk(N)), dim3(BLOCK), 0, c->st, c->flags, c->gnm, c->gid, c->rank, c->pdom, c->prot_gid, c->ggl, N, bits, wpg,
		                   dom_tab, pbits, nw, rec + n_slot * (1 + nw), ovf_cap, c->dcnt);
		I32 *tile = (I32 *)c->pool.get(S_TILE, tile_buf_bytes(n_slot));
		if (!tile) return PGA_ERR_NOMEM;
		device_scan<I32>(InDomSet{dom_tab}, OutExclI32{slot}, n_slot, tile, OpSum{}, I32{0}, c->st);
		hipLaunchKernelGGL(k_vtx_compact, dim3(nblk(n_slot)), dim3(BLOCK), 0, c->st, dom_tab, slot, n_slot, pbits, nw, rec, c->dcnt, c->h_box);
		TRY(sync_st(c));
		if (c->h_cnt[3]) return PGA_ERR_INVARIANT;
		c->live_hint = c->h_cnt[8];
		const int64_t n_rec = c->h_cnt[10], n_ovf = c->h_cnt[0];
		if (n_ovf > ovf_cap) {
			if (ovf_cap >= (long long)N) return PGA_ERR_RANGE;
			ovf_cap = attempt == 0 ? std::min<long long>(N, 2 * n_ovf + 64) : (long long)N;
			continue;
		}
		if (n_ovf) {
			HIPCHK(hipMemcpyAsync(rec + n_rec * (1 + nw), rec + n_slot * (1 + nw), sizeof(uint64_t) * (size_t)n_ovf * (size_t)(1 + nw), hipMemcpyDeviceToDevice, c->st));
			TRY(sync_st(c));
		}
		*n_records = n_rec + n_ovf;
		c->z_early = !c->z_valid;
		return 0;
	}
}

static int stage_upload(pga_ctx *c, void *d0, const void *s0, size_t n0, void *d1, const void *s1, size_t n1)
{
	const size_t a0 = (n0 + 15) & ~(size_t)15, nb = a0 + n1;
	if (nb == 0) return 0;
	if (c->h_g2s_cap < nb) {
		if (c->h_g2s) HIPCHK(hipStreamSynchronize(c->st));
		c->h_g2s = (int32_t *)c->pin.get(nb + nb / 2 + 64);
		if (!c->h_g2s) return PGA_ERR_NOMEM;
		c->h_g2s_cap = nb + nb / 2;
	}
	if (!c->g2s_done) HIPCHK(hipEventCreateWithFlags(&c->g2s_done, hipEventDisableTiming));
	else HIPCHK(hipEventSynchronize(c->g2s_done));
	char *h = (char *)c->h_g2s;
	if (n0) memcpy(h, s0, n0);
	if (n1) memcpy(h + a0, s1, n1);
	if (nb <= ((size_t)1 << 20)) {
		char *hd = nullptr;
		HIPCHK(hipHostGetDevicePointer((void **)&hd, h, 0));
		CopyIn l = { { d0, d1 }, { (const uint32_t *)hd, (const uint32_t *)(hd + a0) }, { n0, n1 } };
		hipLaunchKernelGGL(k_copy_in, dim3(nblk((std::max(n0, n1) + 3) / 4)), dim3(BLOCK), 0, c->st, l);
	} else {
		if (n0) HIPCHK(hipMemcpyAsync(d0, h, n0, hipMemcpyHostToDevice, c->st));
		if (n1) HIPCHK(hipMemcpyAsync(d1, h + a0, n1, hipMemcpyHostToDevice, c->st));
	}
	HIPCHK(hipEventRecord(c->g2s_done, c->st));
	return 0;
}
```

pangene_amd/csrc/host/graph_driver.cpp:

```cpp
#include <sys/mman.h>
#include <sys/time.h>
#include <sys/resource.h>
#include <algorithm>
#include <cmath>
#include <cstdlib>
#include <cstring>
#include <atomic>
#include <climits>
#include <condition_variable>
#include <mutex>
#include <thread>
#include "pg_internal.hpp"
#include "ksort_exact.hpp"

int pg_verbose = 3;

namespace pgx {

pg_exchange_t g_xchg; bool g_has_xchg = false;
static int64_t g_n_coll = 0;
double g_phase[PH_COUNT];
static int g_err = 0; static char g_errstr[256] = "";
static double g_path_sec = 0.0, g_upload_sec = 0.0, g_pack_sec = 0.0, g_t_path0 = 0.0; static int64_t g_path_hits = 0; static int g_attempts = 0;

// ... 232 lines not shown
		if (ext->packs[(size_t)j].buf == nullptr) todo.push_back(j), hits += d->genome[j].n_hit;
	}
	unsigned nt = hits > 100000 ? host_threads(64u) : 1u;
	if (nt > todo.size()) nt = (unsigned)todo.size();
	if (nt <= 1) { for (int32_t j : todo) pack_one(d, ext, j); }
	else {
		std::atomic<size_t> next{0};
		std::vector<std::thread> th;
		for (unsigned t = 0; t < nt; ++t)
			th.emplace_back([&]() { for (;;) { const size_t i = next.fetch_add(1); if (i >= todo.size()) break; pack_one(d, ext, todo[i]); } });
		for (auto &x : th) x.join();
	}
	std::lock_guard<std::mutex> lk(ext->slab_mu);
	ext->pack_sec += (now_sec() - t0) * time_share;
}

static std::mutex g_slab_mu;
static std::vector<HostSlab> g_slab_cache;
static size_t g_slab_cached = 0;
static const size_t SLAB_BYTES = [] { const char *e = std::getenv("PANGENE_SLAB_MB"); return (size_t)(e && std::atoi(e) > 0 ? std::atoi(e) : 64) << 20; }();
static const size_t SLAB_CACHE_MAX = (size_t)4 << 30;

static std::condition_variable g_slab_cv;
static int g_prefetch_left = 0;

static std::atomic<bool> g_device_up{false};
bool device_is_up() { return g_device_up.load(); }

static HostSlab slab_get(size_t min_bytes, bool allow_pin = true)
{
	allow_pin = allow_pin && g_device_up.load();
	{
		std::unique_lock<std::mutex> lk(g_slab_mu);
		for (;;) {
			for (size_t i = 0; i < g_slab_cache.size(); ++i)
				if (g_slab_cache[i].cap >= min_bytes) {
					HostSlab s = g_slab_cache[i];
					g_slab_cache.erase(g_slab_cache.begin() + (long)i);
					g_slab_cached -= s.cap, s.off = 0, s.fresh = false, s.pending = 0, s.closed = false, s.staged = false;
					return s;
				}
			if (g_prefetch_left <= 0 || min_bytes > SLAB_BYTES) break;
			g_slab_cv.wait(lk);
		}
	}
	HostSlab s;
	s.cap = std::max(min_bytes, SLAB_BYTES);
	const pga_backend_t *be = backend_default();
	void *q = nullptr;
	if (allow_pin && be->host_alloc && be->host_alloc(s.cap, &q) == 0) s.pinned = true;
	else {
		void *m = nullptr;
		if (posix_memalign(&m, (size_t)2 << 20, s.cap) == 0) { (void)madvise(m, s.cap, MADV_HUGEPAGE); q = m; }
		else q = std::malloc(s.cap);
		s.pinned = false;
	}
	s.p = (char *)q;
	s.fresh = true;
	return s;
}

void slab_prefetch(size_t bytes, std::thread *helper)
{
	const pga_backend_t *be = backend_default();
	if (be->host_alloc == nullptr || !be->is_device() || !g_device_up.load()) return;
	{ const char *e = std::getenv("PANGENE_PIN_BUDGET_MB"); if (e && std::atoi(e) <= 0) return; }
	size_t have = 0;
	int n = 0;
	{
		std::lock_guard<std::mutex> lk(g_slab_mu);
		for (const HostSlab &c : g_slab_cache) have += c.cap;
		if (bytes > have) n = (int)std::min<size_t>((bytes - have + SLAB_BYTES - 1) / SLAB_BYTES, SLAB_CACHE_MAX / SLAB_BYTES);
		g_prefetch_left += n;
	}
	if (n == 0) return;
	*helper = std::thread([be, n]() {
		std::atomic<int> next{0};
		auto lock_slabs = [&]() {
			while (next.fetch_add(1) < n) {
				void *q = nullptr;
				const bool ok = be->host_alloc(SLAB_BYTES, &q) == 0;
				std::lock_guard<std::mutex> lk(g_slab_mu);
				--g_prefetch_left;
				if (ok) { HostSlab s; s.p = (char *)q, s.cap = SLAB_BYTES, s.pinned = true; g_slab_cache.push_back(s), g_slab_cached += s.cap; }
				g_slab_cv.notify_all();
			}
		};
		std::thread second(lock_slabs);
		lock_slabs();
		second.join();
	});
}

static void stage_slab(DataExt *ext, char *p, size_t n)
{
	const pga_backend_t *be = backend_default();
	static const bool off = [] { const char *e = std::getenv("PANGENE_STAGE"); return e && *e == '0'; }();
	bool ok = !off && be->stage != nullptr && be->is_device() && g_device_up.load() && n > 0 && be->stage(p, n) == 0;
	if (ok) return;
	std::lock_guard<std::mutex> lk(ext->slab_mu);
	for (HostSlab &x : ext->slabs) if (x.p == p) x.staged = false;
}

static void *block_alloc(DataExt *ext, size_t bytes)
{
	bytes = (bytes + 255) & ~(size_t)255;
	char *st_p = nullptr; size_t st_n = 0;
	void *r;
	{
		std::lock_guard<std::mutex> lk(ext->slab_mu);
		if (ext->slabs.empty() || ext->slabs.back().off + bytes > ext->slabs.back().cap) {
			if (!ext->slabs.empty()) {
				HostSlab &prev = ext->slabs.back();
				prev.closed = true;
				if (prev.pending == 0 && prev.pinned && !prev.staged && prev.off) prev.staged = true, st_p = prev.p, st_n = prev.off;
			}
			static const size_t PIN_BUDGET = [] { const char *e = std::getenv("PANGENE_PIN_BUDGET_MB"); return (size_t)(e ? std::max(0, std::atoi(e)) : 192) << 20; }();
			size_t fresh = 0;
			for (const HostSlab &x : ext->slabs) if (x.pinned && x.fresh) fresh += x.cap;
			HostSlab ns = slab_get(bytes, fresh + SLAB_BYTES <= PIN_BUDGET);
			ext->slabs.push_back(ns);
		}
		HostSlab &s = ext->slabs.back();
		r = s.p + s.off;
		s.off += bytes;
		++s.pending;
	}
	if (st_p) stage_slab(ext, st_p, st_n);
	return r;
}

static void block_done(DataExt *ext, const void *buf)
{
	char *st_p = nullptr; size_t st_n = 0;
	{
		std::lock_guard<std::mutex> lk(ext->slab_mu);
		for (HostSlab &x : ext->slabs)
			if (x.p && (const char *)buf >= x.p && (const char *)buf < x.p + x.cap) {
				if (x.pending > 0) --x.pending;
				if (x.closed && x.pending == 0 && x.pinned && !x.staged && x.off) x.staged = true, st_p = x.p, st_n = x.off;
				break;
			}
	}
	if (st_p) stage_slab(ext, st_p, st_n);
}

static void slab_put(HostSlab &s)
{
	if (s.p == nullptr) return;
	std::lock_guard<std::mutex> lk(g_slab_mu);
	if (s.pinned && g_slab_cached + s.cap <= SLAB_CACHE_MAX) g_slab_cache.push_back(s), g_slab_cached += s.cap;
	else if (s.pinned) backend_default()->host_free(s.p);
	else std::free(s.p);
	s.p = nullptr;
}

void trim_host_caches(size_t keep)
{
	const pga_backend_t *be = backend_default();
	{
		std::lock_guard<std::mutex> lk(g_slab_mu);
		std::sort(g_slab_cache.begin(), g_slab_cache.end(), [](const HostSlab &a, const HostSlab &b) { return a.cap > b.cap; });
		size_t kept = 0, n_keep = 0;
		for (; n_keep < g_slab_cache.size() && kept + g_slab_cache[n_keep].cap <= keep; ++n_keep) kept += g_slab_cache[n_keep].cap;
		for (size_t i = n_keep; i < g_slab_cache.size(); ++i) {
			if (g_slab_cache[i].pinned) be->host_free(g_slab_cache[i].p); else std::free(g_slab_cache[i].p);
		}
		g_slab_cache.resize(n_keep);
		g_slab_cached = kept;
	}
	if (be->host_trim) be->host_trim(keep / 4);
}

void free_packs(DataExt *ext, bool wait)
{
	std::vector<GenomePack> old_packs;
	old_packs.swap(ext->packs);
	ext->packs.resize(old_packs.size());
	std::vector<HostSlab> plain;
	for (HostSlab &s : ext->slabs)
		if (s.p && s.staged) { if (backend_default()->stage_drop) backend_default()->stage_drop(s.p); s.staged = false; }
	{
		std::lock_guard<std::mutex> lk(g_slab_mu);
		const pga_backend_t *be = backend_default();
		for (HostSlab &s : ext->slabs) {
			if (s.p == nullptr) continue;
			if (s.pinned && g_slab_cached + s.cap <= SLAB_CACHE_MAX) g_slab_cache.push_back(s), g_slab_cached += s.cap;
			else if (s.pinned) be->host_free(s.p);
			else plain.push_back(s);
		}
		ext->slabs.clear();
	}
	auto drop = [](std::vector<HostSlab> pl, std::vector<GenomePack> pk) { for (HostSlab &s : pl) std::free(s.p); pk.clear(); };
	if (wait || (plain.empty() && old_packs.size() < 64)) { drop(std::move(plain), std::move(old_packs)); return; }
	try { std::thread(drop, plain, old_packs).detach(); }
	catch (const std::system_error &) { drop(std::move(plain), std::move(old_packs)); }
}

static int build_backend(const pg_opt_t *opt, pg_data_t *d, DataExt *ext)
{
	const double t_bb0 = now_sec();
	ext->be = backend_default();
	ext->local_genomes.clear();
	ext->is_local.resize((size_t)d->n_genome, 1);
	ext->hits_sorted.resize((size_t)d->n_genome, 0);
	ext->pos_valid = false, ext->host_full = false, ext->order_touched = false, ext->pos_sig = 0;
	for (int32_t j = 0; j < d->n_genome; ++j)
		if (ext->is_local[(size_t)j]) ext->local_genomes.push_back(j);
	const int32_t nl = (int32_t)ext->local_genomes.size();
	static const bool check_first = [] { const char *e = std::getenv("PANGENE_PACK_CHECK"); return e && std::strcmp(e, "first") == 0; }();
	if (ext->packs.size() < (size_t)d->n_genome) ext->packs.resize((size_t)d->n_genome);
	std::vector<uint8_t> had((size_t)d->n_genome, 0);
	for (int32_t j = 0; j < d->n_genome; ++j) had[(size_t)j] = ext->packs[(size_t)j].buf != nullptr;
	std::vector<int32_t> stale;
	std::thread checker;
	struct Joiner { std::thread &t; ~Joiner() { if (t.joinable()) t.join(); } } joiner{checker};
	if (check_first) pack_genomes(d, ext, 0, d->n_genome);
	else {
		try { checker = std::thread([&]() { stale_packs(d, ext, 0, d->n_genome, stale, &had); }); }
		catch (const std::system_error &) { stale_packs(d, ext, 0, d->n_genome, stale, &had); }
		pack_genomes(d, ext, 0, d->n_genome, 1.0, false);
	}
	static const bool timing = std::getenv("PANGENE_TIMING") != nullptr;
	double t1 = t_bb0, t2 = t_bb0;
	int rc = 0;
	for (int attempt = 0;; ++attempt) {
		auto verdict = [&]() -> bool {
			if (attempt > 0 || check_first) return false;
			if (checker.joinable()) checker.join();
			if (stale.empty()) return false;
			if (ext->ctx) ext->be->destroy(ext->ctx), ext->ctx = nullptr;
			for (int32_t j : stale) ext->packs[(size_t)j] = GenomePack();
			pack_genomes(d, ext, 0, d->n_genome, 1.0, false);
			if (timing) std::fprintf(stderr, "[build_backend] %zu pack(s) no longer matched their genome: packed and uploaded again\n", stale.size());
			return true;
		};
		int64_t N = 0, E = 0;
		ext->hit_off.assign((size_t)nl + 1, 0);
		std::vector<pga_genome_block_t> blk((size_t)nl);
		int err = 0;
		bool limit = false;
		for (int32_t k = 0; k < nl && !err; ++k) {
			const GenomePack &pk = ext->packs[(size_t)ext->local_genomes[(size_t)k]];
			if (pk.err) { err = pk.err; break; }
			blk[(size_t)k] = pk.blk;
			N += pk.blk.n_hit, E += pk.blk.n_exon;
			ext->hit_off[(size_t)k + 1] = N;
		}
		if (!err && (d->n_gene >= (1 << 20) || d->n_genome >= (1 << 24) || E >= INT32_MAX || N >= INT32_MAX)) err = PGA_ERR_RANGE, limit = true;
		if (err) {
			if (verdict()) continue;
			if (!limit) free_packs(ext, false);
			return err;
		}
		ext->vreal.assign((size_t)nl, std::vector<int32_t>()), ext->n_vctg.assign((size_t)nl, 0);
		for (int32_t k = 0; k < nl; ++k) {
			const GenomePack &pk = ext->packs[(size_t)ext->local_genomes[(size_t)k]];
			ext->n_vctg[(size_t)k] = pk.blk.n_ctg;
			if (!pk.vreal.empty()) ext->vreal[(size_t)k] = pk.vreal;
		}
		if (pg_verbose >= 3) {
			int64_t n_cut = 0, n_piece = 0, n_g = 0;
			for (int32_t k = 0; k < nl; ++k) {
				const GenomePack &pk = ext->packs[(size_t)ext->local_genomes[(size_t)k]];
				if (pk.vreal.empty()) continue;
				++n_g;
				for (size_t v = 0; v < pk.vfirst.size(); ++v) n_piece += pk.vfirst[v] != (int32_t)v, n_cut += v + 1 < pk.vfirst.size() && pk.vfirst[v] == (int32_t)v && pk.vfirst[v + 1] == (int32_t)v;
			}
			if (n_g) std::fprintf(stderr, "[M::%s] 64-bit coordinates: %lld genome(s) with virtual contigs, %lld contig(s) cut, %lld extra piece(s)\n", __func__, (long long)n_g, (long long)n_cut, (long long)n_piece);
		}
		std::vector<int32_t> pgid((size_t)d->n_prot);
		std::vector<uint8_t> gpref((size_t)d->n_gene);
		for (int32_t p = 0; p < d->n_prot; ++p) pgid[(size_t)p] = d->prot[p].gid;
		for (int32_t q = 0; q < d->n_gene; ++q) gpref[(size_t)q] = d->gene[q].preferred;
		pga_shard_t sh;
		std::memset(&sh, 0, sizeof(sh));
		sh.abi_version = PGA_ABI_VERSION;
		sh.n_genome = nl, sh.n_genome_global = d->n_genome, sh.genome_global = ext->local_genomes.data();
		sh.n_prot = d->n_prot, sh.n_gene = d->n_gene, sh.n_hit = N, sh.n_exon = E;
		sh.block = blk.data(), sh.prot_gid = pgid.data(), sh.gene_pref = gpref.data();
		pga_params_t par;
		std::memset(&par, 0, sizeof(par));
		par.min_ov_ratio = opt->min_ov_ratio;
		par.check_strand = !!(opt->flag & PG_F_CHECK_STRAND);
		par.drop_sgl_exon = !!(opt->flag & PG_F_DROP_SGL_EXON);
		if (ext->ctx) ext->be->destroy(ext->ctx), ext->ctx = nullptr;
		ext->n_hit_local = N;
		t1 = now_sec();
		rc = ext->be->create(&ext->ctx, &sh, &par);
		if (rc == 0) g_device_up.store(true);
		t2 = now_sec();
		if (verdict()) continue;
		break;
	}
	size_t n_pin = 0, n_plain = 0, n_fresh = 0;
	for (const HostSlab &x : ext->slabs) { if (x.pinned) ++n_pin; else ++n_plain; if (x.fresh) ++n_fresh; }
	free_packs(ext, false);
	if (timing) {
		std::fprintf(stderr, "[build_backend] tables %.3f ms, create %.3f ms, release of the host blocks %.3f ms; block slabs: %zu page-locked, %zu plain, %zu new in this read\n", (t1 - t_bb0) * 1e3, (t2 - t1) * 1e3, (now_sec() - t2) * 1e3, n_pin, n_plain, n_fresh);
	}
	return rc;
}

int sync_host(pg_data_t *d, bool full)
{
	DataExt *ext = ext_of(d, false);
	if (ext == nullptr || ext->ctx == nullptr) return g_err;
	if (!ext->host_stale && !(full && !ext->host_full)) return g_err;
	Phase ph(PH_SYNC_HOST);
	const int64_t N = ext->n_hit_local;
	uint64_t sig_now = ext->pos_sig;
	if (ext->order_touched) {
		exact_shutdown(ext);
		sig_now = order_signature(ext);
		if (sig_now != ext->pos_sig) ext->pos_valid = false;
		ext->order_touched = false;
	}
	const bool need_pos = !ext->pos_valid;
	const size_t nbits = (size_t)((N + 63) / 64) + 1, n_arr = (full ? 5 : 0) + (need_pos ? 2 : 0);
	HostSlab land = slab_get(sizeof(int32_t) * (size_t)N * n_arr + sizeof(uint64_t) * nbits + 64);
	if (land.p == nullptr) { set_error(PGA_ERR_NOMEM, "sync_host"); return g_err; }
	int32_t *w = (int32_t *)land.p;
	uint32_t *flags = nullptr;
	int32_t *rank = nullptr, *sdom = nullptr, *pdom = nullptr, *pdom0 = nullptr, *pxl = nullptr, *py = nullptr;
	if (full) flags = (uint32_t *)w, rank = w + (size_t)N, sdom = w + 2 * (size_t)N, pdom = w + 3 * (size_t)N, pdom0 = w + 4 * (size_t)N, w += 5 * (size_t)N;
	if (need_pos) pxl = w, py = w + (size_t)N, w += 2 * (size_t)N;
	uint64_t *bits = (uint64_t *)(land.p + ((((char *)w - land.p) + 7) & ~(size_t)7));
	pga_hit_state_t st = { flags, rank, sdom, pdom, pdom0, pxl, py, bits };
	{
		const int rc = ext->be->download(ext->ctx, &st);
		if (rc) { slab_put(land); set_error(rc, "download"); return rc; }
	}
	ext->flt_bits.assign(bits, bits + nbits);
	if (need_pos && ext->pos_x.size() != (size_t)N) ext->pos_x.resize((size_t)N);
	struct Land { HostSlab &s; ~Land() { slab_put(s); } } land_guard{land};
	const int32_t *px = ext->pos_x.data();
	ext->y_file.resize((size_t)d->n_genome);
	ext->file_of_host.resize((size_t)d->n_genome);
	ext->host_of_file.resize((size_t)d->n_genome);
	if (need_pos) ext->host_order_valid = false;
	const bool move = full && !ext->host_order_valid;
	auto do_genome = [&](size_t k) {
		int32_t j = ext->local_genomes[k];
		pg_genome_t *g = &d->genome[j];
		const int64_t off = ext->hit_off[k];
		if (need_pos) {
			if (g->n_hit > 0) std::memcpy(ext->pos_x.data() + off, pxl + off, sizeof(int32_t) * (size_t)g->n_hit);
			ext->y_file[(size_t)j].assign((size_t)g->n_hit, 0);
			for (int32_t f = 0; f < g->n_hit; ++f) ext->y_file[(size_t)j][(size_t)py[(size_t)(off + f)]] = f;
		}
		if (move) {
			pg_hit_t *a = (pg_hit_t *)std::malloc(sizeof(pg_hit_t) * (size_t)(g->n_hit > 0 ? g->n_hit : 1));
			if (!ext->hits_sorted[(size_t)j]) {
				for (int32_t f = 0; f < g->n_hit; ++f) a[px[(size_t)(off + f)]] = g->hit[f];
			} else {
				const int32_t *old = ext->file_of_host[(size_t)j].data();
				for (int32_t h = 0; h < g->n_hit; ++h) a[px[(size_t)(off + old[h])]] = g->hit[h];
			}
			if (!ext->arena_owns(g->hit)) std::free(g->hit);
			else {
				const uintptr_t a0 = ((uintptr_t)g->hit + 4095) & ~(uintptr_t)4095, a1 = ((uintptr_t)g->hit + sizeof(pg_hit_t) * (size_t)g->m_hit) & ~(uintptr_t)4095;
				if (a1 > a0) (void)madvise((void *)a0, a1 - a0, MADV_DONTNEED);
			}
			g->hit = a, g->m_hit = g->n_hit;
			ext->hits_sorted[(size_t)j] = 1;
			ext->file_of_host[(size_t)j].assign((size_t)g->n_hit, 0);
			ext->host_of_file[(size_t)j].assign((size_t)g->n_hit, 0);
			for (int32_t f = 0; f < g->n_hit; ++f) {
				ext->file_of_host[(size_t)j][(size_t)px[(size_t)(off + f)]] = f;
				ext->host_of_file[(size_t)j][(size_t)f] = px[(size_t)(off + f)];
			}
		}
		if (!full) return;
		for (int32_t f = 0; f < g->n_hit; ++f) {
			const size_t s = (size_t)(off + f);
			pg_hit_t *h = &g->hit[px[s]];
			const uint32_t fl = flags[s];
			h->flt = !!(fl & PGA_F_FLT), h->flt_iso_sub_self = !!(fl & PGA_F_ISO_SUB), h->flt_iso_ov = !!(fl & PGA_F_ISO_OV);
			h->flt_chain = !!(fl & PGA_F_CHAIN), h->pseudo = !!(fl & PGA_F_PSEUDO), h->vtx = !!(fl & PGA_F_VTX);
			h->shadow = !!(fl & PGA_F_SHADOW), h->rep = !!(fl & PGA_F_REP), h->weak_br = (fl & PGA_F_WEAK_MASK) >> PGA_F_WEAK_SHIFT;
			h->rank = rank[s], h->score_dom = sdom[s], h->pid_dom = pdom[s], h->pid_dom0 = pdom0[s];
		}
	};
	if (need_pos || full) {
		const size_t ng = ext->local_genomes.size();
		unsigned nt = N > 200000 ? host_threads(16u) : 1u;
		if (nt > ng) nt = (unsigned)ng;
		if (nt <= 1) { for (size_t k = 0; k < ng; ++k) do_genome(k); }
		else {
			std::vector<std::thread> th;
			for (unsigned t = 0; t < nt; ++t)
				th.emplace_back([&, t]() { for (size_t k = ng * t / nt; k < ng * (t + 1) / nt; ++k) do_genome(k); });
			for (auto &x : th) x.join();
		}
	}
	if (move) ext->host_order_valid = true;
	if (need_pos) ext->pos_sig = sig_now;
	ext->pos_valid = true;
	ext->host_stale = false;
	ext->host_full = full;
	return 0;
}

static const char *trace_path() { static const char *p = std::getenv("PANGENE_TRACE"); return (p && *p) ? p : nullptr; }
static uint64_t fnv1a(const void *data, size_t n, uint32_t mask)
{
	uint64_t h = 1469598103934665603ull;
	const uint32_t *w = (const uint32_t *)data;
	for (size_t i = 0; i < n; ++i) {
		uint32_t v = w[i] & mask;
		for (int b = 0; b < 4; ++b) h = (h ^ (v & 0xffu)) * 1099511628211ull, v >>= 8;
	}
	return h;
}
static int trace_state(DataExt *ext, const char *step, int round, bool first = false)
{
	if (trace_path() == nullptr || ext == nullptr || ext->ctx == nullptr) return 0;
	const size_t N = (size_t)ext->n_hit_local;
	std::vector<uint32_t> flags(N + 1);
	std::vector<int32_t> rank(N + 1), sdom(N + 1), pdom(N + 1), pdom0(N + 1), px(N + 1), py(N + 1);
	pga_hit_state_t st = { flags.data(), rank.data(), sdom.data(), pdom.data(), pdom0.data(), px.data(), py.data(), nullptr };
	BE_CALL(ext->be->download(ext->ctx, &st), "download(trace)");
	static const bool diff_on = std::getenv("PANGENE_TRACE_DIFF") != nullptr;
	if (diff_on) {
		static std::vector<uint32_t> prev;
		if (prev.size() == N && !first) {
			int64_t n_any = 0, n_walk = 0, n_weak = 0, n_flt = 0;
			std::vector<uint8_t> tile((N + 255) / 256 + 1, 0);
			size_t k = 0;
			for (size_t f = 0; f < N; ++f) {
				const uint32_t x = (flags[f] ^ prev[f]) & 0x7ffu;
				if (!x) continue;
				++n_any, n_walk += (x & (PGA_F_FLT | PGA_F_SHADOW)) != 0, n_weak += (x & PGA_F_WEAK_MASK) != 0, n_flt += (x & PGA_F_FLT) != 0;
				while (k + 1 < ext->hit_off.size() && (int64_t)f >= ext->hit_off[k + 1]) ++k;
				tile[(size_t)(ext->hit_off[k] + px[f]) >> 8] = 1;
			}
			int64_t n_tile = 0;
			for (uint8_t t : tile) n_tile += t;
			int64_t n_live = 0, n_wk = 0;
			for (size_t f = 0; f < N; ++f) n_live += !(flags[f] & PGA_F_FLT), n_wk += !(flags[f] & (PGA_F_FLT | PGA_F_SHADOW));
			std::fprintf(stderr, "[trace_diff] %-18s %3d: %lld of %zu hits changed their flag word (walkable test %lld, flt %lld, weak_br %lld); %lld of %zu tiles of 256 hits dirty; live (flt == 0) %lld = %.3f, walkable %lld = %.3f\n", step, round,
			             (long long)n_any, N, (long long)n_walk, (long long)n_flt, (long long)n_weak, (long long)n_tile, tile.size(), (long long)n_live, (double)n_live / (double)(N ? N : 1), (long long)n_wk, (double)n_wk / (double)(N ? N : 1));
		}
		else {
			int64_t n_live = 0, n_wk = 0;
			for (size_t f = 0; f < N; ++f) n_live += !(flags[f] & PGA_F_FLT), n_wk += !(flags[f] & (PGA_F_FLT | PGA_F_SHADOW));
			std::fprintf(stderr, "[trace_diff] %-18s %3d: %zu hits; live (flt == 0) %lld = %.3f, walkable %lld = %.3f\n", step, round, N, (long long)n_live, (double)n_live / (double)(N ? N : 1), (long long)n_wk, (double)n_wk / (double)(N ? N : 1));
		}
		prev.assign(flags.begin(), flags.begin() + (long)N);
	}
	std::FILE *fp = std::fopen(trace_path(), first ? "w" : "a");
	if (fp == nullptr) return 0;
	std::fprintf(fp, "%s\t%d\tflags=%016llx\trank=%016llx\tscore_dom=%016llx\tpid_dom=%016llx\tpid_dom0=%016llx\tpos_x=%016llx\tpos_y=%016llx\n", step, round,
	             (unsigned long long)fnv1a(flags.data(), N, 0x7ffu), (unsigned long long)fnv1a(rank.data(), N, ~0u), (unsigned long long)fnv1a(sdom.data(), N, ~0u),
	             (unsigned long long)fnv1a(pdom.data(), N, ~0u), (unsigned long long)fnv1a(pdom0.data(), N, ~0u), (unsigned long long)fnv1a(px.data(), N, ~0u),
	             (unsigned long long)fnv1a(py.data(), N, ~0u));
	std::fclose(fp);
	return 0;
}

static bool exact_early(const DataExt *ext)
{
	if (exact_mode() == 2) return true;
	for (const ExactSeg &s : ext->xsegs) if (s.full) return true;
	return false;
}

static int post_process_impl(const pg_opt_t *opt, pg_data_t *d)
{
	DataExt *ext = ext_of(d, true);
	double t0 = now_sec();
	if (ext->read_failed) { set_error(PGA_ERR_NOMEM, "pg_post_process: a pg_read_paf ran out of memory, the data set is incomplete"); return PGA_ERR_NOMEM; }
	if (!(ext->rerun && ext->ctx)) {
		g_pack_sec = ext->pack_sec, ext->pack_sec = 0.0;
		BE_CALL(build_backend(opt, d, ext), "create");
		g_pack_sec += ext->pack_sec, ext->pack_sec = 0.0;
		ext->route_verbose = -1;
		if (sharded()) {
			int32_t v = pg_verbose;
			void *scr;
			BE_CALL(ext->be->scratch(ext->ctx, 16, &scr), "scratch");
			BE_CALL(ext->be->put(ext->ctx, scr, &v, sizeof(v)), "put");
			BE_CALL(xreduce(ext->be, ext->ctx, scr, 1, PG_X_I32, PG_X_MAX), "allreduce(log level)");
			BE_CALL(ext->be->fetch(ext->ctx, &v, scr, sizeof(v)), "fetch");
			ext->route_verbose = v;
		}
		const double tx0 = now_sec();
		const bool cs_opt = !!(opt->flag & PG_F_CHECK_STRAND);
		if (!(ext->xsegs_n_genome == d->n_genome && ext->exact_mode_of_segs == exact_mode() && ext->extra_ctgs.empty() && ext->xreplayed && ext->check_strand == cs_opt && ext->min_ov_ratio == opt->min_ov_ratio)) {
			ext->check_strand = cs_opt, ext->min_ov_ratio = opt->min_ov_ratio;
			exact_init(d, ext);
			ext->exact_mode_of_segs = exact_mode();
		}
		if (std::getenv("PANGENE_TIMING")) std::fprintf(stderr, "[post_process] exact_init %.3f ms\n", (now_sec() - tx0) * 1e3);
	} else if (ext->exact_mode_of_segs != exact_mode() || ext->check_strand != !!(opt->flag & PG_F_CHECK_STRAND) || ext->min_ov_ratio != opt->min_ov_ratio) {
		exact_shutdown(ext);
		ext->check_strand = !!(opt->flag & PG_F_CHECK_STRAND), ext->min_ov_ratio = opt->min_ov_ratio;
		exact_init(d, ext);
		ext->exact_mode_of_segs = exact_mode();
	}
	ext->rerun = false;
	g_upload_sec = now_sec() - t0;
	const pga_backend_t *be = ext->be;
	pga_ctx_t *ctx = ext->ctx;
	g_t_path0 = now_sec();
	for (int i = 0; i < PH_COUNT; ++i) g_phase[i] = 0;
	exact_begin(ext);
	{ Phase ph(PH_BEGIN); BE_CALL(be->begin(ctx), "begin"); }
	if (exact_early(ext)) { Phase ph(PH_EXACT); BE_CALL(exact_sort(ext, 0), "override_order"); }
	const int32_t nl = (int32_t)ext->local_genomes.size(), P = d->n_prot;
	if (pg_verbose >= 3)
		std::fprintf(stderr, "[M::%s::%s] %d genes and %d proteins; %ld hits of %d genomes on backend '%s'\n", __func__, stamp(),
		             d->n_gene, d->n_prot, (long)ext->n_hit_local, nl, be->name);

	std::vector<int32_t> st4((size_t)nl * 4);
	{ Phase ph(PH_INGEST); BE_CALL(be->ingest(ctx, pg_verbose >= 3 ? st4.data() : nullptr), "ingest"); }
	BE_CALL(trace_state(ext, "ingest", 0, true), "trace");
	Phase ph_post(PH_POST);
	if (pg_verbose >= 3)
		for (int32_t k = 0; k < nl; ++k) {
			const pg_genome_t *g = &d->genome[ext->local_genomes[(size_t)k]];
			std::fprintf(stderr, "[M::pg_read_paf::%s] [%d] %s: %d kept and %d+%d+%d+%d filtered\n", stamp(), ext->local_genomes[(size_t)k],
			             g->label ? g->label : "-", g->n_hit, st4[(size_t)k*4], st4[(size_t)k*4+1], st4[(size_t)k*4+2], st4[(size_t)k*4+3]);
		}

	int32_t *b_max; int64_t *b_sum;
	BE_CALL(be->post_partials(ctx, &b_max, &b_sum), "post_partials");
	BE_CALL(xreduce(be, ext->ctx, b_max, P, PG_X_I32, PG_X_MAX), "allreduce(max_score_ori)");
	BE_CALL(xreduce(be, ext->ctx, b_sum, 6 * (int64_t)P, PG_X_I64, PG_X_SUM), "allreduce(protein sums)");
	static thread_local std::vector<int32_t> mx;
	static thread_local std::vector<int64_t> sm;
	mx.resize((size_t)P), sm.resize((size_t)P * 6);
	if (P) {
		const void *mx_view = nullptr;
		BE_CALL(be->fetch_later(ctx, b_max, sizeof(int32_t) * (size_t)P, &mx_view), "fetch_later");
		BE_CALL(be->fetch(ctx, sm.data(), b_sum, sizeof(int64_t) * (size_t)P * 6), "fetch");
		std::memcpy(mx.data(), mx_view, sizeof(int32_t) * (size_t)P);
	}
	const double tp0 = now_sec();
	static thread_local std::vector<pg128_t> z;
	z.resize((size_t)P);
	for (int32_t i = 0; i < d->n_gene; ++i) d->gene[i].rep_pid = -1;
	for (int32_t i = 0; i < P; ++i) {
		d->prot[i].max_score_ori = mx[(size_t)i];
		d->prot[i].rep = 0;
		z[(size_t)i].x = ((uint64_t)sm[(size_t)i] << 32) + (uint64_t)sm[(size_t)P + (size_t)i];
		z[(size_t)i].y = (uint64_t)i;
		d->prot[i].n = (int32_t)(uint32_t)z[(size_t)i].x;
		d->prot[i].avg_score_adj = d->prot[i].n ? (int32_t)((double)(z[(size_t)i].x >> 32) / d->prot[i].n + .499) : 0;
	}
	const double tp1 = now_sec();
	ksort_exact(z.data(), z.size(), [](const pg128_t &a) { return a.x; });
	const double tp2 = now_sec();
	for (int32_t i = P - 1; i >= 0; --i) {
		int32_t pid = (int32_t)z[(size_t)i].y, gid = d->prot[pid].gid;
		if (d->gene[gid].rep_pid < 0) d->gene[gid].rep_pid = pid, d->prot[pid].rep = 1;
	}
	static thread_local std::vector<uint8_t> rep, pj;
	rep.resize((size_t)P), pj.assign((size_t)P, 0);
	for (int32_t i = 0; i < P; ++i) rep[(size_t)i] = (uint8_t)d->prot[i].rep;
	if (!(opt->flag & PG_F_NO_JOINT_PSEUDO)) {
		for (int32_t i = 0; i < P; ++i) {
			const int64_t c0 = sm[2 * (size_t)P + (size_t)i], c1 = sm[3 * (size_t)P + (size_t)i];
			const int64_t s0 = sm[4 * (size_t)P + (size_t)i], s1 = sm[5 * (size_t)P + (size_t)i];
			const int32_t ic1 = (int32_t)c1, ic0 = (int32_t)c0;
			bool a = ic1 > 0 && ic1 >= d->n_genome * opt->min_vertex_ratio && ((double)s1 / ic1) / ((double)s0 / ic0) >= 0.99;
			bool b = (ic1 == 0 || ic1 <= d->n_genome * opt->min_vertex_ratio) && (opt->flag & PG_F_DROP_SGL_EXON);
			pj[(size_t)i] = a || b;
		}
	}
	if (std::getenv("PANGENE_TIMING")) std::fprintf(stderr, "[post] host step between the fetch of the protein sums and post_apply: %.3f ms (%d proteins; sums -> keys %.3f, sort of the proteins %.3f, representatives + joint-pseudo predicate %.3f)\n", (now_sec() - tp0) * 1e3, P, (tp1 - tp0) * 1e3, (tp2 - tp1) * 1e3, (now_sec() - tp2) * 1e3);
	int64_t n_pj = 0;
	BE_CALL(be->post_apply(ctx, rep.data(), pj.data(), (!(opt->flag & PG_F_NO_JOINT_PSEUDO) && pg_verbose >= 3) ? &n_pj : nullptr), "post_apply");
	if (!(opt->flag & PG_F_NO_JOINT_PSEUDO) && pg_verbose >= 3)
		std::fprintf(stderr, "[M::%s::%s] %ld pseudogene hits identified jointly\n", __func__, stamp(), (long)n_pj);
	std::vector<int32_t> st2((size_t)nl * 2);
	BE_CALL(be->shadow(ctx, 0, pg_verbose >= 3 ? st2.data() : nullptr), "shadow");
	if (pg_verbose >= 3)
		for (int32_t k = 0; k < nl; ++k) {
			const pg_genome_t *g = &d->genome[ext->local_genomes[(size_t)k]];
			std::fprintf(stderr, "[M::%s::%s] genome[%d]: %s; %d hits remain, of which %d are shadowed\n", __func__, stamp(),
			             ext->local_genomes[(size_t)k], g->label ? g->label : "-", st2[(size_t)k*2], st2[(size_t)k*2+1]);
		}
	ext->host_stale = true;
	BE_CALL(trace_state(ext, "post_process", 0), "trace");
	return 0;
}

static void gen_g2s(pg_graph_t *q)
{
	const pg_data_t *d = q->d;
	std::free(q->g2s);
	q->g2s = (int32_t *)std::malloc(sizeof(int32_t) * (size_t)(d->n_gene > 0 ? d->n_gene : 1));
	for (int32_t i = 0; i < d->n_gene; ++i) q->g2s[i] = -1;
	for (int32_t i = 0; i < q->n_seg; ++i) q->g2s[q->seg[i].gid] = i;
}

static void arc_index(pg_graph_t *q)
{
	std::free(q->idx);
	q->idx = (uint64_t *)std::calloc((size_t)(q->n_seg > 0 ? q->n_seg * 2 : 1), sizeof(uint64_t));
	for (int32_t i0 = 0, i = 1; i <= q->n_arc; ++i)
		if (i == q->n_arc || q->arc[i].x >> 32 != q->arc[i0].x >> 32)
			q->idx[q->arc[i0].x >> 32] = (uint64_t)i0 << 32 | (uint32_t)(i - i0), i0 = i;
}

static int gen_vtx(const pg_opt_t *opt, pg_graph_t *q, DataExt *ext)
{
	pg_data_t *d = q->d;
	const pga_backend_t *be = ext->be;
	const int32_t Q = d->n_gene, G = d->n_genome;
	Phase ph_vtx(PH_VTX);
	int32_t *b_cnt; uint64_t *b_tri; int64_t n_tri;
	const double tv0 = now_sec();
	BE_CALL(be->vtx_partials(ext->ctx, &b_cnt, &b_tri, &n_tri), "vtx_partials");
	const double tv1 = now_sec();
	BE_CALL(xreduce(be, ext->ctx, b_cnt, 2 * (int64_t)Q, PG_X_I32, PG_X_SUM), "allreduce(n_dom,n_sub)");
	static thread_local std::vector<int32_t> cntv;
	cntv.assign((size_t)Q * 2, 0);
	const void *cntv_view = nullptr;
	if (Q) BE_CALL(be->fetch_later(ext->ctx, b_cnt, sizeof(int32_t) * (size_t)Q * 2, &cntv_view), "fetch_later");
	const uint64_t m20 = (1u << 20) - 1;
	const int64_t nw = ((int64_t)G + 63) / 64;
	static thread_local std::vector<uint64_t> pairs;
	pairs.resize((size_t)(n_tri * (1 + nw)));
	if (n_tri && !sharded()) BE_CALL(be->fetch(ext->ctx, pairs.data(), b_tri, sizeof(uint64_t) * pairs.size()), "fetch");
	const double tv2 = now_sec();
	if (sharded()) {
		BE_CALL(xgather(be, ext->ctx, b_tri, n_tri * (1 + nw), pairs), "allgather(vertex pairs)");
	}
	if (Q) {
		if (n_tri == 0 || sharded()) BE_CALL(be->sync(ext->ctx), "sync");
		std::memcpy(cntv.data(), cntv_view, sizeof(int32_t) * (size_t)Q * 2);
	}
	const int64_t n_rec = (int64_t)(pairs.size() / (size_t)(1 + nw));
	static thread_local std::vector<int64_t> sub_off, sub_rec, cur;
	sub_off.assign((size_t)Q + 1, 0);
	for (int64_t r = 0; r < n_rec; ++r) ++sub_off[(size_t)(pairs[(size_t)(r * (1 + nw))] >> 20) + 1];
	for (int32_t g = 0; g < Q; ++g) sub_off[(size_t)g + 1] += sub_off[(size_t)g];
	sub_rec.resize((size_t)n_rec);
	{
		cur.assign(sub_off.begin(), sub_off.end() - 1);
		for (int64_t r = 0; r < n_rec; ++r) sub_rec[(size_t)cur[(size_t)(pairs[(size_t)(r * (1 + nw))] >> 20)]++] = r;
	}
	static thread_local std::vector<uint64_t> marked;
	static thread_local std::vector<int32_t> mark_slot, ycnt;
	static thread_local std::vector<pg128_t> cnt;
	marked.clear(), mark_slot.assign((size_t)Q, -1), ycnt.assign((size_t)Q, 0), cnt.resize((size_t)Q);
	for (int32_t i = 0; i < Q; ++i) {
		cnt[(size_t)i].x = (uint64_t)(int64_t)d->prot[d->gene[i].rep_pid].avg_score_adj;
		cnt[(size_t)i].y = (uint64_t)i;
		cnt[(size_t)i].x += (uint64_t)cntv[(size_t)i] << 32;
		cnt[(size_t)i].y += (uint64_t)cntv[(size_t)Q + (size_t)i] << 32;
		if (d->gene[i].preferred) cnt[(size_t)i].x |= 1ULL << 63;
	}
	ksort_exact(cnt.data(), cnt.size(), [](const pg128_t &a) { return a.x; });
	q->n_seg = 0;
	if (q->m_seg < Q) {
		const int32_t old_m = q->m_seg;
		q->m_seg = Q + 16;
		q->seg = (pg_seg_t *)std::realloc(q->seg, sizeof(pg_seg_t) * (size_t)q->m_seg);
		std::memset((void *)(q->seg + old_m), 0, sizeof(pg_seg_t) * (size_t)(q->m_seg - old_m));
	}
	marked.reserve((size_t)nw * 1024);
	ext->vtx_sel_text.clear();
	for (int32_t i = Q - 1; i >= 0; --i) {
		const int32_t n_dom = (int32_t)(cnt[(size_t)i].x << 1 >> 33), n_sub = (int32_t)(cnt[(size_t)i].y >> 32);
		const int32_t gid = (int32_t)cnt[(size_t)i].y;
		const int32_t x = cntv[(size_t)gid], y = ycnt[(size_t)gid];
		if (opt->flag & PG_F_WRITE_VTX_SEL) {
			char line[512];
			std::snprintf(line, sizeof(line), "g\t%s\t%d\t%d\t%d\t%d\t%c\t%c\n", d->gene[gid].name, (int32_t)cnt[(size_t)i].x, x, y, n_sub,
			              "NY"[d->gene[gid].included], "NY"[d->gene[gid].preferred]);
			ext->vtx_sel_text += line;
		}
		if (d->gene[gid].included || (n_dom >= G * opt->min_vertex_ratio && y < x)) {
			if (q->n_seg >= q->m_seg) {
				int32_t old = q->m_seg;
				q->m_seg = q->n_seg + 1; q->m_seg += (q->m_seg >> 1) + 16;
				q->seg = (pg_seg_t *)std::realloc(q->seg, sizeof(pg_seg_t) * (size_t)q->m_seg);
				std::memset((void *)(q->seg + old), 0, sizeof(pg_seg_t) * (size_t)(q->m_seg - old));
			}
			pg_seg_t *p = &q->seg[q->n_seg++];
			p->gid = gid, p->n_dom = n_dom, p->n_sub = n_sub;
			if (x > 0)
				for (int64_t k = sub_off[(size_t)gid]; k < sub_off[(size_t)gid + 1]; ++k) {
					const uint64_t *rec = &pairs[(size_t)(sub_rec[(size_t)k] * (1 + nw))];
					const int32_t dom = (int32_t)(rec[0] & m20);
					if (mark_slot[(size_t)dom] < 0) mark_slot[(size_t)dom] = (int32_t)(marked.size() / (size_t)nw), marked.resize(marked.size() + (size_t)nw, 0);
					uint64_t *mk = &marked[(size_t)mark_slot[(size_t)dom] * (size_t)nw];
					for (int64_t w = 0; w < nw; ++w) {
						const uint64_t fresh = rec[1 + w] & ~mk[w];
						mk[w] |= fresh, ycnt[(size_t)dom] += __builtin_popcountll(fresh);
					}
				}
		}
	}
	if (std::getenv("PANGENE_TIMING")) std::fprintf(stderr, "[vtx] partials %.3f ms, fetch %.3f ms (records %ld / %ld), greedy %.3f ms\n", (tv1 - tv0) * 1e3, (tv2 - tv1) * 1e3, (long)n_tri, (long)n_rec, (now_sec() - tv2) * 1e3);
	{
		std::vector<int32_t> at((size_t)Q, -1);
		for (int32_t i = 0; i < q->n_seg; ++i) at[(size_t)q->seg[i].gid] = i;
		std::vector<pg_seg_t> tmp(q->seg, q->seg + q->n_seg);
		int32_t k = 0;
		for (int32_t g = 0; g < Q; ++g) if (at[(size_t)g] >= 0) q->seg[k++] = tmp[(size_t)at[(size_t)g]];
	}
	gen_g2s(q);
	if (pg_verbose >= 3)
		std::fprintf(stderr, "[M::%s::%s] selected %d vertices out of %d genes\n", "pg_gen_vtx", stamp(), q->n_seg, Q);
	return 0;
}

static int loop_allreduce(void *user, void *buf, int64_t count);
static int loop_allgather(void *user, const void *in, void *out, int64_t bytes);

static int gen_arc(const pg_opt_t *opt, pg_graph_t *q, DataExt *ext, bool defer = false)
{
	const pga_backend_t *be = ext->be;
	const int32_t S = q->n_seg;
	int32_t *b_seg; pga_arc_part_t *b_arc; int64_t n_loc;
	{ Phase ph(PH_EXACT); BE_CALL(exact_sort(ext, 1), "override_order"); }
	if (!sharded() && defer && route_v(ext) < 3 && be->arc_round_finish) {
		{ Phase ph(PH_ARC_DEV); BE_CALL(be->arc_round_local(ext->ctx, !!(opt->flag & PG_F_ORI_FOR_BRANCH), S, nullptr, nullptr), "arc_round"); }
		{ Phase ph(PH_EXACT); BE_CALL(exact_sort(ext, 0), "override_order"); }
		ext->arc_pending = true, ext->cur_arcs = nullptr, q->n_arc = 0;
		return 0;
	}
	std::vector<int32_t> sc((size_t)S * 2 + 1);
	ext->deg.assign((size_t)S * 2 + 1, 0);
	ext->arc_via_x = false;
	static const bool no_x = std::getenv("PANGENE_SHARDED_LOOP_HOST") != nullptr;
	if (sharded() && !no_x && be->arc_round_x && be->is_device() && ext->x_arc_slot > 0 && S > 0 && route_v(ext) < 3) {
		pga_loop_xchg_t lx;
		lx.user = ext, lx.rank = g_xchg.rank, lx.world = g_xchg.world, lx.arc_cap_hint = ext->x_arc_slot, lx.allreduce_i32_sum = loop_allreduce, lx.allgather = loop_allgather;
		int64_t n_arc = 0;
		int rc;
		{ Phase ph(PH_ARC_DEV); rc = be->arc_round_x(ext->ctx, !!(opt->flag & PG_F_ORI_FOR_BRANCH), S, &lx, sc.data(), ext->deg.data(), &n_arc); }
		if (rc < 0) { set_error(rc, "arc_round_x"); return rc; }
		if (rc == 0) {
			{ Phase ph(PH_EXACT); BE_CALL(exact_sort(ext, 0), "override_order"); }
			for (int32_t i = 0; i < S; ++i) q->seg[i].n_genome = sc[(size_t)i], q->seg[i].tot_cnt = sc[(size_t)S + (size_t)i];
			ext->cur_arcs = nullptr, q->n_arc = (int32_t)n_arc;
			ext->arc_via_x = true;
			return 0;
		}
	}
	if (!sharded()) {
		int64_t n_arc = 0;
		const pga_arc_part_t *tab = nullptr;
		{ Phase ph(PH_ARC_DEV); BE_CALL(be->arc_round_local(ext->ctx, !!(opt->flag & PG_F_ORI_FOR_BRANCH), S, sc.data(), ext->deg.data()), "arc_round"); }
		if (pg_verbose >= 3) BE_CALL(be->arc_table(ext->ctx, &tab, &n_arc), "arc_table");
		{ Phase ph(PH_EXACT); BE_CALL(exact_sort(ext, 0), "override_order"); }
		for (int32_t i = 0; i < S; ++i) q->seg[i].n_genome = sc[(size_t)i], q->seg[i].tot_cnt = sc[(size_t)S + (size_t)i];
		ext->cur_arcs = tab, q->n_arc = (int32_t)n_arc;
		return 0;
	}
	{ Phase ph(PH_ARC_DEV); BE_CALL(be->arc_round(ext->ctx, !!(opt->flag & PG_F_ORI_FOR_BRANCH), &b_seg, &b_arc, &n_loc), "arc_round"); }
	{ Phase ph(PH_EXACT); BE_CALL(exact_sort(ext, 0), "override_order"); }
	Phase ph_host(PH_ARC_HOST);
	const pga_arc_part_t *cur = b_arc;
	int64_t n_cur = n_loc;
	{
		const int W = g_xchg.world;
		std::vector<int32_t> mine((size_t)W, 0), all((size_t)S * 2 + (size_t)W);
		mine[(size_t)g_xchg.rank] = (int32_t)n_loc;
		void *scr;
		BE_CALL(be->scratch(ext->ctx, sizeof(int32_t) * ((size_t)S * 2 + (size_t)W), &scr), "scratch");
		if (S) BE_CALL(be->copy(ext->ctx, scr, b_seg, sizeof(int32_t) * (size_t)S * 2), "copy");
		BE_CALL(be->put(ext->ctx, (int32_t *)scr + (size_t)S * 2, mine.data(), sizeof(int32_t) * (size_t)W), "put");
		BE_CALL(xreduce(be, ext->ctx, scr, 2 * (int64_t)S + W, PG_X_I32, PG_X_SUM), "allreduce(seg counts, table sizes)");
		BE_CALL(be->fetch(ext->ctx, all.data(), scr, sizeof(int32_t) * all.size()), "fetch");
		std::copy(all.begin(), all.begin() + (size_t)S * 2, sc.begin());
		std::vector<int64_t> cnt((size_t)W);
		int64_t slot = 0, n_mg = 0;
		for (int r = 0; r < W; ++r) cnt[(size_t)r] = all[(size_t)S * 2 + (size_t)r], slot = std::max(slot, cnt[(size_t)r]);
		ext->x_arc_slot = std::max(ext->x_arc_slot, slot);
		pga_arc_part_t *merged = nullptr;
		if (slot) {
			const size_t bytes = (size_t)slot * sizeof(pga_arc_part_t);
			BE_CALL(be->scratch(ext->ctx, bytes * (size_t)(W + 1), &scr), "scratch");
			if (n_loc) BE_CALL(be->copy(ext->ctx, scr, b_arc, (size_t)n_loc * sizeof(pga_arc_part_t)), "copy");
			BE_CALL(xready(be, ext->ctx), "sync");
			++g_n_coll;
			BE_CALL(g_xchg.allgather(g_xchg.user, scr, (char *)scr + bytes, (int64_t)bytes, be->is_device()), "allgather(arcs)");
			BE_CALL(be->arc_merge(ext->ctx, (pga_arc_part_t *)((char *)scr + bytes), cnt.data(), W, slot, &merged, &n_mg), "arc_merge");
		}
		cur = merged, n_cur = n_mg;
	}
	BE_CALL(be->arc_set_current(ext->ctx, cur, n_cur, S, ext->deg.data()), "arc_set_current");
	for (int32_t i = 0; i < S; ++i) q->seg[i].n_genome = sc[(size_t)i], q->seg[i].tot_cnt = sc[(size_t)S + (size_t)i];
	ext->cur_arcs = cur, q->n_arc = (int32_t)n_cur;
	return 0;
}

static int arc_collect(const pg_opt_t *opt, pg_graph_t *q, DataExt *ext)
{
	if (!ext->arc_pending) return 0;
	ext->arc_pending = false;
	const int32_t S = q->n_seg;
	std::vector<int32_t> &sc = ext->sc_buf;
	if (sc.size() < (size_t)S * 2 + 1) sc.resize((size_t)S * 2 + 1);
	if (ext->deg.size() < (size_t)S * 2 + 1) ext->deg.resize((size_t)S * 2 + 1);
	int rc = ext->be->arc_round_finish(ext->ctx, S, sc.data(), ext->deg.data());
	if (rc < 0) { set_error(rc, "arc_round_finish"); return rc; }
	if (rc == 1) BE_CALL(ext->be->arc_round_local(ext->ctx, !!(opt->flag & PG_F_ORI_FOR_BRANCH), S, sc.data(), ext->deg.data()), "arc_round");
	for (int32_t i = 0; i < S; ++i) q->seg[i].n_genome = sc[(size_t)i], q->seg[i].tot_cnt = sc[(size_t)S + (size_t)i];
	return rc;
}

static int fetch_arcs(pg_graph_t *q, DataExt *ext, bool loop_final = false)
{
	Phase ph_host(PH_ARC_HOST);
	if (loop_final && ext->be->final_arcs != nullptr) {
		const void *view = nullptr;
		int64_t n = 0;
		if (ext->be->final_arcs(ext->ctx, &view, &n) == 0) {
			static_assert(sizeof(pg_arc_t) == 32, "the backend writes pg_arc_t records");
			q->n_arc = (int32_t)n;
			if (n > q->m_arc) {
				q->m_arc = (int32_t)n + ((int32_t)n >> 1) + 16;
				q->arc = (pg_arc_t *)std::realloc(q->arc, sizeof(pg_arc_t) * (size_t)q->m_arc);
			}
			if (n) std::memcpy(q->arc, view, sizeof(pg_arc_t) * (size_t)n);
			if (std::getenv("PANGENE_TIMING")) std::fprintf(stderr, "[fetch_arcs] the loop left the final table: %lld arcs, no wait\n", (long long)n);
			return 0;
		}
	}
	{
		int64_t n = 0;
		BE_CALL(ext->be->arc_table(ext->ctx, &ext->cur_arcs, &n), "arc_table");
		q->n_arc = (int32_t)n;
	}
	const pga_arc_part_t *part = nullptr;
	const size_t n_part = (size_t)q->n_arc;
	if (n_part) {
		const void *view = nullptr;
		BE_CALL(ext->be->fetch_later(ext->ctx, ext->cur_arcs, sizeof(pga_arc_part_t) * n_part, &view), "fetch_later");
		BE_CALL(ext->be->sync(ext->ctx), "sync");
		part = (const pga_arc_part_t *)view;
	}
	if ((int64_t)n_part > q->m_arc) {
		q->m_arc = (int32_t)n_part + ((int32_t)n_part >> 1) + 16;
		q->arc = (pg_arc_t *)std::realloc(q->arc, sizeof(pg_arc_t) * (size_t)q->m_arc);
	}
	for (size_t i = 0; i < n_part; ++i) {
		pg_arc_t *p = &q->arc[i];
		std::memset(p, 0, sizeof(*p));
		p->x = part[i].x, p->n_genome = part[i].n_genome, p->tot_cnt = part[i].tot_cnt;
		if (!ext->seg_renumber.empty()) {
			const uint32_t v = (uint32_t)(p->x >> 32), w = (uint32_t)p->x;
			p->x = (uint64_t)((uint32_t)ext->seg_renumber[v >> 1] << 1 | (v & 1u)) << 32 | ((uint32_t)ext->seg_renumber[w >> 1] << 1 | (w & 1u));
		}
		p->avg_dist = (int32_t)(int64_t)((double)(int64_t)part[i].sum_dist / part[i].tot_cnt + .499);
		p->s1 = (int32_t)((double)part[i].sum_s1 / part[i].n_genome + .499);
		p->s2 = (int32_t)((double)part[i].sum_s2 / part[i].n_genome + .499);
	}
	return 0;
}

static int flag_vtx(pg_graph_t *q, DataExt *ext) { return ext->be->flag_vtx(ext->ctx, q->g2s, q->n_seg, 1); }

static int flt_high_occ(int32_t max_avg_occ, int32_t max_degree, int32_t max_dist_loci, pg_graph_t *q, DataExt *ext)
{
	Phase ph(PH_FLT);
	int32_t n_high_occ = 0, n_high_deg = 0, n_high_loci = 0;
	for (int32_t i = 0; i < q->n_seg; ++i)
		if (q->seg[i].tot_cnt > max_avg_occ * q->d->n_genome) q->seg[i].del = 1, ++n_high_occ;
	for (int32_t v = 0; v < 2 * q->n_seg; ++v)
		if (ext->deg[(size_t)v] > max_degree && !q->seg[v >> 1].del) q->seg[v >> 1].del = 1, ++n_high_deg;
	for (int32_t i = 0; i < q->n_seg; ++i) {
		pg_seg_t *s = &q->seg[i];
		int32_t m = s->n_dist_loci[0] > s->n_dist_loci[1] ? s->n_dist_loci[0] : s->n_dist_loci[1];
		if (m > max_dist_loci && !s->del) s->del = 1, ++n_high_loci;
	}
	if (pg_verbose >= 3)
		std::fprintf(stderr, "[M::%s::%s] filtered %d high-occurrence segments, %d high-degree segments and %d segments connecting distant loci\n",
		             "pg_flt_high_occ", stamp(), n_high_occ, n_high_deg, n_high_loci);
	int32_t k = 0;
	for (int32_t i = 0; i < q->n_seg; ++i) {
		if (!q->seg[i].del) q->seg[k++] = q->seg[i];
		else if (pg_verbose >= 3)
			std::fprintf(stderr, "#del\t%s\tavg_occ=%.1f\tdist_deg=%d,%d\n", q->d->gene[q->seg[i].gid].name,
			             (double)q->seg[i].tot_cnt / q->d->n_genome, q->seg[i].n_dist_loci[0], q->seg[i].n_dist_loci[1]);
	}
	q->n_seg = k;
	gen_g2s(q);
	return flag_vtx(q, ext);
}

static int mark_branch_flt_arc(const pg_opt_t *opt, pg_graph_t *q, DataExt *ext)
{
	const pga_backend_t *be = ext->be;
	Phase ph_all(PH_BRANCH_HOST);
	std::vector<int32_t> ndl((size_t)q->n_seg * 2 + 1);
	int64_t n_flt1 = 0, n_flt2 = 0;
	for (int attempt = 0;; ++attempt) {
		BE_CALL(be->rep_pos(ext->ctx), "rep_pos");
		int32_t *b_cnt; int64_t np = 0;
		Phase ph(PH_NLOCAL);
		BE_CALL(be->branch_pairs(ext->ctx, nullptr, nullptr, 0, nullptr, q->n_seg, opt->branch_diff, opt->local_dist, opt->local_count,
		                         !!(opt->flag & PG_F_FRAG_MODE), &b_cnt, sharded() ? &np : nullptr), "branch_pairs");
		BE_CALL(xreduce(be, ext->ctx, b_cnt, np, PG_X_I32, PG_X_SUM), "allreduce(n_local)");
		BE_CALL(be->branch_decide(ext->ctx, opt->branch_diff, opt->branch_diff_dist, opt->branch_diff_cut, nullptr, ndl.data(), pg_verbose >= 3 ? &n_flt1 : nullptr, pg_verbose >= 3 ? &n_flt2 : nullptr), "branch_decide");
		g_phase[PH_BRANCH_HOST] -= now_sec() - ph.t0;
		const int rc = arc_collect(opt, q, ext);
		if (rc < 0) return rc;
		if (rc == 0 || attempt) break;
	}
	for (int32_t j = 0; j < q->n_seg; ++j) q->seg[j].n_dist_loci[0] = ndl[(size_t)j * 2], q->seg[j].n_dist_loci[1] = ndl[(size_t)j * 2 + 1];
	if (pg_verbose >= 3)
		std::fprintf(stderr, "[M::%s::%s] marked %ld locally diverged branches and %ld distantly diverged branches\n", "pg_mark_branch_flt_arc", stamp(), (long)n_flt1, (long)n_flt2);
	return 0;
}

static int mark_branch_flt_arc_fast(const pg_opt_t *opt, pg_graph_t *q, DataExt *ext, bool do_filter, int32_t max_tot_cnt, int32_t max_degree, int32_t max_dist_loci,
                                    std::vector<uint8_t> &del, bool *done)
{
	const pga_backend_t *be = ext->be;
	*done = false;
	static const bool host_only = std::getenv("PANGENE_ROUND_FILTER_HOST") != nullptr;
	if (host_only || sharded() || route_v(ext) >= 3 || be->branch_decide_filter == nullptr || !ext->arc_pending) return 0;
	const int32_t S = q->n_seg;
	{
		Phase ph(PH_NLOCAL);
		BE_CALL(be->rep_pos(ext->ctx), "rep_pos");
		int32_t *b_cnt;
		BE_CALL(be->branch_pairs(ext->ctx, nullptr, nullptr, 0, nullptr, S, opt->branch_diff, opt->local_dist, opt->local_count, !!(opt->flag & PG_F_FRAG_MODE), &b_cnt, nullptr), "branch_pairs");
		del.resize((size_t)S + 1);
		const int rc = be->branch_decide_filter(ext->ctx, opt->branch_diff, opt->branch_diff_dist, opt->branch_diff_cut, do_filter ? 1 : 0, max_tot_cnt, max_degree, max_dist_loci, del.data());
		if (rc == 2) return 0;
		if (rc != 0) { set_error(rc, "branch_decide_filter"); return rc; }
	}
	Phase ph(PH_BRANCH_HOST);
	ext->arc_pending = false;
	const int rc = be->arc_round_finish(ext->ctx, S, nullptr, nullptr);
	if (rc < 0) { set_error(rc, "arc_round_finish"); return rc; }
	if (rc == 1) {
		std::vector<int32_t> sc((size_t)S * 2 + 1);
		ext->deg.assign((size_t)S * 2 + 1, 0);
		BE_CALL(be->arc_round_local(ext->ctx, !!(opt->flag & PG_F_ORI_FOR_BRANCH), S, sc.data(), ext->deg.data()), "arc_round");
		for (int32_t i = 0; i < S; ++i) q->seg[i].n_genome = sc[(size_t)i], q->seg[i].tot_cnt = sc[(size_t)S + (size_t)i];
		return 0;
	}
	*done = true;
	return 0;
}

static int apply_round_filter(pg_graph_t *q, DataExt *ext, const std::vector<uint8_t> &del)
{
	Phase ph(PH_FLT);
	int32_t k = 0;
	for (int32_t i = 0; i < q->n_seg; ++i)
		if (!del[(size_t)i]) q->seg[k++] = q->seg[i];
	q->n_seg = k;
	gen_g2s(q);
	return flag_vtx(q, ext);
}

enum { RC_REDO = 1000 };
static int loop_allreduce(void *user, void *buf, int64_t count)
{
	DataExt *ext = (DataExt *)user;
	if (count == 0) return 0;
	const int rc = xready(ext->be, ext->ctx);
	++g_n_coll;
	return rc ? rc : g_xchg.allreduce(g_xchg.user, buf, count, PG_X_I32, PG_X_SUM, ext->be->is_device());
}
static int loop_allgather(void *user, const void *in, void *out, int64_t bytes)
{
	DataExt *ext = (DataExt *)user;
	const int rc = xready(ext->be, ext->ctx);
	++g_n_coll;
	return rc ? rc : g_xchg.allgather(g_xchg.user, in, out, bytes, ext->be->is_device());
}

static int branch_loop_fast(const pg_opt_t *opt, pg_graph_t *q, DataExt *ext, int32_t R, bool *done, bool pre = false, bool fin = false)
{
	*done = false;
	const pga_backend_t *be = ext->be;
	const bool shd = sharded();
	if (be->branch_loop == nullptr || route_v(ext) >= 3 || trace_path() != nullptr || (!shd && !ext->arc_pending) || R < 1 || ext->no_branch_loop) return 0;
	static const bool no_x = std::getenv("PANGENE_SHARDED_LOOP_HOST") != nullptr;
	if (shd && (no_x || !be->is_device())) return 0;
	if (shd && ext->skip_loop_once) { ext->skip_loop_once = false; return 0; }
	if (pre && shd && !ext->arc_via_x) return 0;
	const int n_sorts = 2 * R - 1 + (pre ? 1 : 0) + (fin ? 1 : 0);
	static const bool dbg = std::getenv("PANGENE_TIMING") != nullptr;
	bool quiet;
	{ Phase ph(PH_EXACT); quiet = exact_quiet(ext, n_sorts); }
	if (shd) {
		int32_t ok = (quiet && ext->n_hit_local > 0 && q->n_seg > 0) ? 1 : 0;
		void *scr;
		BE_CALL(be->scratch(ext->ctx, 16, &scr), "scratch");
		BE_CALL(be->put(ext->ctx, scr, &ok, sizeof(ok)), "put");
		BE_CALL(xreduce(be, ext->ctx, scr, 1, PG_X_I32, PG_X_SUM), "allreduce(vote)");
		BE_CALL(be->fetch(ext->ctx, &ok, scr, sizeof(ok)), "fetch");
		if (ok != g_xchg.world) { if (dbg) std::fprintf(stderr, "[branch_loop] %d of %d ranks can queue their rounds: host-driven rounds\n", ok, g_xchg.world); return 0; }
	}
	else if (!quiet) { if (dbg) std::fprintf(stderr, "[branch_loop] not quiet: the hit at array index 0 of some genome changes within the next %d sorts\n", n_sorts); return 0; }
	const int32_t S = q->n_seg, n = opt->n_branch_flt;
	std::vector<int32_t> m_tot((size_t)R), m_deg((size_t)R), m_loci((size_t)R);
	for (int32_t i = 0; i < R; ++i) {
		const double r = 1.0 + (double)(n - 1 - i) / n;
		m_tot[(size_t)i] = (int32_t)(opt->max_avg_occ * r + .499) * q->d->n_genome;
		m_deg[(size_t)i] = (int32_t)(opt->max_degree * r + .499);
		m_loci[(size_t)i] = (int32_t)(opt->max_dist_loci * r + .499);
	}
	pga_branch_par_t par;
	par.branch_diff = opt->branch_diff, par.branch_diff_dist = opt->branch_diff_dist, par.branch_diff_cut = opt->branch_diff_cut;
	par.local_dist = opt->local_dist, par.local_count = opt->local_count, par.frag_mode = !!(opt->flag & PG_F_FRAG_MODE), par.use_ori = !!(opt->flag & PG_F_ORI_FOR_BRANCH);
	par.pre_on = pre ? 1 : 0;
	par.pre_max_tot_cnt = opt->max_avg_occ * 2 * q->d->n_genome, par.pre_max_degree = opt->max_degree * 2, par.pre_max_dist_loci = opt->max_dist_loci;
	par.final_on = fin ? 1 : 0;
	std::vector<uint8_t> &alive = ext->del_buf;
	alive.assign((size_t)S + 1, 1);
	std::vector<int32_t> fin_sc, fin_ndl;
	if (fin) fin_sc.assign((size_t)S * 2 + 1, 0), fin_ndl.assign((size_t)S * 2 + 1, 0);
	pga_loop_xchg_t lx;
	lx.user = ext, lx.rank = g_xchg.rank, lx.world = g_xchg.world, lx.arc_cap_hint = ext->x_arc_slot, lx.allreduce_i32_sum = loop_allreduce, lx.allgather = loop_allgather;
	int rc;
	{ Phase ph(PH_NLOCAL); rc = be->branch_loop(ext->ctx, R, &par, m_tot.data(), m_deg.data(), m_loci.data(), alive.data(), shd ? &lx : nullptr, fin ? fin_sc.data() : nullptr, fin ? fin_ndl.data() : nullptr); }
	if (dbg) std::fprintf(stderr, "[branch_loop] %d rounds queued%s: backend status %d\n", R, shd ? " (sharded)" : "", rc);
	if (rc == 2) return 0;
	if (rc == 1) { ext->no_branch_loop = true; return RC_REDO; }
	if (rc == 3) { ext->skip_loop_once = true; return RC_REDO; }
	if (rc == 4) { if (++ext->loop_room_retries > 2) ext->no_branch_loop = true; return RC_REDO; }
	if (rc != 0) { set_error(rc, "branch_loop"); return rc; }
	ext->arc_pending = false;
	exact_skip(ext, n_sorts);
	Phase ph(PH_FLT);
	int32_t k = 0;
	if (fin) ext->seg_renumber.assign((size_t)S, -1);
	for (int32_t i = 0; i < S; ++i)
		if (alive[(size_t)i]) {
			if (fin) {
				pg_seg_t *sg = &q->seg[i];
				sg->n_genome = fin_sc[(size_t)i], sg->tot_cnt = fin_sc[(size_t)S + (size_t)i];
				sg->n_dist_loci[0] = fin_ndl[(size_t)i * 2], sg->n_dist_loci[1] = fin_ndl[(size_t)i * 2 + 1];
				ext->seg_renumber[(size_t)i] = k;
			}
			q->seg[k++] = q->seg[i];
		}
	q->n_seg = k;
	gen_g2s(q);
	if (!fin) BE_CALL(flag_vtx(q, ext), "flag_vtx");
	*done = true;
	return 0;
}

static int mark_branch_flt_hit(pg_graph_t *q, DataExt *ext)
{
	int64_t n = 0;
	{ Phase ph(PH_EXACT); BE_CALL(exact_sort(ext, 1), "override_order"); }
	{ Phase ph(PH_MARK_HITS); BE_CALL(ext->be->mark_hits(ext->ctx, nullptr, nullptr, q->n_arc, pg_verbose >= 3 ? &n : nullptr, 1), "mark_hits"); }
	{ Phase ph(PH_EXACT); BE_CALL(exact_sort(ext, 0), "override_order"); }
	if (pg_verbose >= 3)
		std::fprintf(stderr, "[M::%s::%s] marked %ld diverged hits\n", "pg_mark_branch_flt_hit", stamp(), (long)n);
	return 0;
}

static int graph_gen_impl(const pg_opt_t *opt, pg_graph_t *q)
{
	DataExt *ext = ext_of(q->d, false);
	if (ext == nullptr || ext->ctx == nullptr) { set_error(PGA_ERR_ARG, "pg_graph_gen: pg_post_process has not run"); return PGA_ERR_ARG; }
	const pga_backend_t *be = ext->be;
	pga_ctx_t *ctx = ext->ctx;
	ext->arc_pending = false;
	BE_CALL(be->set_filter(ctx, PGA_FLT_PSEUDO), "set_filter");
	BE_CALL(gen_vtx(opt, q, ext), "gen_vtx");
	if (!exact_early(ext)) { Phase ph(PH_EXACT); BE_CALL(exact_sort(ext, 0), "set_head"); }
	BE_CALL(flag_vtx(q, ext), "flag_vtx");
	BE_CALL(trace_state(ext, "gen_vtx+flag_vtx", 0), "trace");
	static const bool no_pre = env_word("PANGENE_LOOP", "nopre");
	static const bool no_fin = env_word("PANGENE_LOOP", "nofinal");
	const bool try_pre = !no_pre && opt->n_branch_flt >= 2 && ext->be->branch_loop != nullptr && route_v(ext) < 3 && trace_path() == nullptr && !ext->no_branch_loop &&
	                     (!sharded() || (ext->be->arc_round_x != nullptr && ext->be->is_device() && ext->x_arc_slot > 0 && std::getenv("PANGENE_SHARDED_LOOP_HOST") == nullptr));
	BE_CALL(gen_arc(opt, q, ext, try_pre), "gen_arc");
	BE_CALL(trace_state(ext, "gen_arc", 1), "trace");
	if (pg_verbose >= 3) std::fprintf(stderr, "[M::%s::%s] round-1 graph: %d genes and %d arcs\n", "pg_graph_gen", stamp(), q->n_seg, q->n_arc);
	int32_t i_first = 0;
	bool queued = false;
	bool queued_all = false;
	ext->seg_renumber.clear();
	if (try_pre) {
		if (!no_fin) {
			const int rc = branch_loop_fast(opt, q, ext, opt->n_branch_flt, &queued_all, true, true);
			if (rc) return rc;
			queued = queued_all;
		}
		const int rc = queued ? 0 : branch_loop_fast(opt, q, ext, opt->n_branch_flt - 1, &queued, true);
		if (rc) return rc;
		if (!queued) {
			const int rc2 = arc_collect(opt, q, ext);
			if (rc2 < 0) return rc2;
		}
	}
	if (!queued) {
		BE_CALL(flt_high_occ(opt->max_avg_occ * 2, opt->max_degree * 2, opt->max_dist_loci, q, ext), "flt_high_occ");
		BE_CALL(trace_state(ext, "flt_high_occ", 1), "trace");
		BE_CALL(gen_arc(opt, q, ext, opt->n_branch_flt > 0), "gen_arc");
		BE_CALL(trace_state(ext, "gen_arc", 2), "trace");
		if (pg_verbose >= 3) std::fprintf(stderr, "[M::%s::%s] round-2 graph: %d genes and %d arcs\n", "pg_graph_gen", stamp(), q->n_seg, q->n_arc);
		if (opt->n_branch_flt >= 2) {
			if (!no_fin && !no_pre) {
				const int rc = branch_loop_fast(opt, q, ext, opt->n_branch_flt, &queued_all, false, true);
				if (rc) return rc;
				queued = queued_all;
			}
			if (!queued) {
				const int rc = branch_loop_fast(opt, q, ext, opt->n_branch_flt - 1, &queued);
				if (rc) return rc;
			}
		}
	}
	if (queued_all) i_first = opt->n_branch_flt;
	else if (queued) {
		i_first = opt->n_branch_flt - 1;
		BE_CALL(gen_arc(opt, q, ext, true), "gen_arc");
	}
	for (int32_t i = i_first; i < opt->n_branch_flt; ++i) {
		double r = 1.0 + (double)(opt->n_branch_flt - 1 - i) / opt->n_branch_flt;
		int32_t max_avg_occ = (int32_t)(opt->max_avg_occ * r + .499);
		int32_t max_degree = (int32_t)(opt->max_degree * r + .499);
		int32_t max_dist_loci = (int32_t)(opt->max_dist_loci * r + .499);
		bool on_backend = false;
		if (i + 1 < opt->n_branch_flt)
			BE_CALL(mark_branch_flt_arc_fast(opt, q, ext, i > 0, max_avg_occ * q->d->n_genome, max_degree, max_dist_loci, ext->del_buf, &on_backend), "mark_branch_flt_arc");
		if (!on_backend) BE_CALL(mark_branch_flt_arc(opt, q, ext), "mark_branch_flt_arc");
		BE_CALL(mark_branch_flt_hit(q, ext), "mark_branch_flt_hit");
		BE_CALL(trace_state(ext, "mark_branch", i + 3), "trace");
		if (i > 0 && on_backend) BE_CALL(apply_round_filter(q, ext, ext->del_buf), "flt_high_occ");
		else if (i > 0) BE_CALL(flt_high_occ(max_avg_occ, max_degree, max_dist_loci, q, ext), "flt_high_occ");
		if (i > 0) BE_CALL(trace_state(ext, "flt_high_occ", i + 3), "trace");
		BE_CALL(gen_arc(opt, q, ext, i + 1 < opt->n_branch_flt), "gen_arc");
		BE_CALL(trace_state(ext, "gen_arc", i + 3), "trace");
	}
	BE_CALL(be->set_filter(ctx, PGA_FLT_SHADOW), "set_filter");
	BE_CALL(fetch_arcs(q, ext, queued_all), "fetch_arcs");
	if (queued_all) {
		ext->seg_renumber.clear();
		BE_CALL(flag_vtx(q, ext), "flag_vtx");
	}
	if (opt->min_arc_cnt > 1) {
		int32_t k = 0, n_aflt = 0;
		for (int32_t i = 0; i < q->n_arc; ++i) {
			if (q->arc[i].n_genome < opt->min_arc_cnt) { ++n_aflt; continue; }
			q->arc[k++] = q->arc[i];
		}
		q->n_arc = k;
		if (pg_verbose >= 3) std::fprintf(stderr, "[M::%s::%s] filtered %d low-occurrence arcs\n", "pg_graph_cut_low_arc", stamp(), n_aflt);
	}
	arc_index(q);
	if (pg_verbose >= 3) std::fprintf(stderr, "[M::%s::%s] round-3 graph: %d genes and %d arcs\n", "pg_graph_gen", stamp(), q->n_seg, q->n_arc);
	BE_CALL(exact_sort(ext, 1), "override_order");
	ext->host_stale = true;
	pga_hazard_t hz;
	if (exact_mode() == 0 && be->hazards(ctx, &hz) == 0 && (hz.h1_head_tie | hz.h2_cm_tie | hz.h3_dom_tie | hz.h2_cs_tie) && pg_verbose >= 2)
		std::fprintf(stderr, "[W::%s] tie-order hazards seen (head-tie %ld, cm-tie %ld, dominator-tie %ld, cs-tie at the local_count boundary %ld): output may differ from the reference's unstable sort order\n",
		             "pg_graph_gen", (long)hz.h1_head_tie, (long)hz.h2_cm_tie, (long)hz.h3_dom_tie, (long)hz.h2_cs_tie);
	return g_err;
}

}

using namespace pgx;

extern "C" {

void pg_opt_init(pg_opt_t *opt)
{
	std::memset(opt, 0, sizeof(*opt));
	opt->gene_delim = ':';
	opt->min_prot_iden = 0.5, opt->min_prot_ratio = 0.5, opt->score_adj_coef = 2.0;
	opt->min_ov_ratio = 0.5, opt->min_vertex_ratio = 0.05;
	opt->max_avg_occ = 10, opt->max_degree = 15, opt->max_dist_loci = 3;
	opt->n_branch_flt = 15, opt->min_arc_cnt = 1;
	opt->local_dist = 2000000, opt->local_count = 10;
	opt->branch_diff = 0.02, opt->branch_diff_dist = 0.05, opt->branch_diff_cut = 0.5;
}

void pg_post_process(const pg_opt_t *opt, pg_data_t *d)
{
	g_err = 0;
	g_t_path0 = now_sec();
	post_process_impl(opt, d);
	g_path_sec = now_sec() - g_t_path0;
	DataExt *ext = ext_of(d, false);
	g_path_hits = ext ? ext->n_hit_local : 0;
	int32_t n_pref = 0;
	for (int32_t i = 0; i < d->n_gene; ++i) n_pref += d->gene[i].preferred;
	if (pg_verbose >= 3) std::fprintf(stderr, "[M::%s] there are %d preferred genes\n", __func__, n_pref);
}

pg_graph_t *pg_graph_init(pg_data_t *d)
{
	pg_graph_t *g = (pg_graph_t *)std::calloc(1, sizeof(pg_graph_t));
	g->d = d;
	g->m_seg = d->n_gene > 0 ? d->n_gene : 1;
	g->seg = (pg_seg_t *)std::calloc((size_t)g->m_seg, sizeof(pg_seg_t));
	return g;
}

static int hazards_review(DataExt *ext, bool *need, bool *give_up)
{
	pga_hazard_t hz;
	const double th0 = now_sec();
	BE_CALL(ext->be->hazards(ext->ctx, &hz), "hazards");
	const double th1 = now_sec();
	double th2 = th1, th3 = th1;
	int32_t flags[2] = { 0, 0 };
	if (hz.h2_cm_tie + hz.h3_dom_tie + hz.h2_cs_tie > 0) {
		std::vector<int32_t> segs(PGA_HAZARD_CAP);
		int64_t n_total = 0;
		th2 = now_sec();
		BE_CALL(ext->be->hazard_segs(ext->ctx, segs.data(), (int32_t)segs.size(), &n_total), "hazard_segs");
		th3 = now_sec();
		const int64_t n_got = std::min<int64_t>(n_total, (int64_t)segs.size());
		if (n_total > n_got) flags[0] = flags[1] = 1;
		std::vector<int32_t> base(ext->local_genomes.size() + 1, 0);
		for (size_t k = 0; k < ext->local_genomes.size(); ++k) base[k + 1] = base[k] + (k < ext->n_vctg.size() ? ext->n_vctg[k] : ext->q_d->genome[ext->local_genomes[k]].n_ctg);
		std::sort(segs.begin(), segs.begin() + n_got);
		int64_t n_new = 0;
		for (int64_t i = 0; i < n_got; ++i) {
			if (i && segs[(size_t)i] == segs[(size_t)i - 1]) continue;
			const size_t k = (size_t)(std::upper_bound(base.begin(), base.end(), segs[(size_t)i]) - base.begin()) - 1;
			int32_t ctg_local = segs[(size_t)i] - base[k];
			if (k < ext->vreal.size() && !ext->vreal[k].empty() && (size_t)ctg_local < ext->vreal[k].size()) ctg_local = ext->vreal[k][(size_t)ctg_local];
			const std::pair<int32_t, int32_t> gc((int32_t)k, ctg_local);
			if (std::binary_search(ext->static_ctgs.begin(), ext->static_ctgs.end(), gc)) continue;
			auto it = std::lower_bound(ext->extra_ctgs.begin(), ext->extra_ctgs.end(), gc);
			if (it == ext->extra_ctgs.end() || *it != gc) ext->extra_ctgs.insert(it, gc), ++n_new;
			if (std::getenv("PANGENE_TIMING")) std::fprintf(stderr, "[hazard] local genome %d contig %d\n", gc.first, gc.second);
		}
		if (n_new) flags[0] = 1;
		if (pg_verbose >= 2)
			std::fprintf(stderr, "[M::%s::%s] tie-order hazards on this rank: %ld equal-cm neighbours, %ld equal-key dominators, %ld order-dependent local_count tests, on %ld contig(s) not yet following the exact order\n",
			             "pg_graph_gen", stamp(), (long)hz.h2_cm_tie, (long)hz.h3_dom_tie, (long)hz.h2_cs_tie, (long)n_new);
	}
	if (sharded()) {
		void *scr;
		BE_CALL(ext->be->scratch(ext->ctx, 16, &scr), "scratch");
		BE_CALL(ext->be->put(ext->ctx, scr, flags, sizeof(flags)), "put");
		BE_CALL(xreduce(ext->be, ext->ctx, scr, 2, PG_X_I32, PG_X_MAX), "allreduce(hazard)");
		BE_CALL(ext->be->fetch(ext->ctx, flags, scr, sizeof(flags)), "fetch");
	}
	*need = flags[0] != 0, *give_up = flags[1] != 0;
	if (std::getenv("PANGENE_TIMING")) std::fprintf(stderr, "[hazards_review] counters %.3f ms, list set-up %.3f ms, list fetch %.3f ms, rest %.3f ms (cm %ld dom %ld cs %ld)\n",
	                                               (th1 - th0) * 1e3, (th2 - th1) * 1e3, (th3 - th2) * 1e3, (now_sec() - th3) * 1e3, (long)hz.h2_cm_tie, (long)hz.h3_dom_tie, (long)hz.h2_cs_tie);
	return 0;
}

void pg_graph_gen(const pg_opt_t *opt, pg_graph_t *q)
{
	double t = now_sec();
	DataExt *ext = ext_of(q->d, false);
	if (ext) ext->q_d = q->d;
	auto run_graph = [&]() {
		int rc = graph_gen_impl(opt, q);
		if (rc == RC_REDO && ext) {
			if (pg_verbose >= 2) std::fprintf(stderr, "[M::%s::%s] the queued branch rounds met a case they leave to the host: repeating stages A-C with host-driven rounds\n", "pg_graph_gen", stamp());
			q->n_seg = 0, q->n_arc = 0;
			std::memset((void *)q->seg, 0, sizeof(pg_seg_t) * (size_t)q->m_seg);
			ext->rerun = true;
			rc = post_process_impl(opt, q->d);
			if (rc == 0) rc = graph_gen_impl(opt, q);
		}
		return rc;
	};
	if (g_err == 0 && run_graph() != 0) q->n_arc = 0;
	const double t_first = now_sec() - t;
	int n_attempt = 1;
	double t_review = 0.0;
	const double path_before = g_path_sec;
	for (int attempt = 0; g_err == 0 && ext && exact_mode() == 1; ++attempt) {
		bool need = false, give_up = false;
		const double tr0 = now_sec();
		const int rc_review = hazards_review(ext, &need, &give_up);
		t_review += now_sec() - tr0;
		if (rc_review != 0 || !need) break;
		const bool k_selective = std::getenv("PANGENE_ESCALATE_ALL") == nullptr;
		const bool all = !k_selective || give_up || attempt >= 2;
		if (pg_verbose >= 2)
			std::fprintf(stderr, "[M::%s::%s] repeating stages A-C with the reference's exact hit order on %s\n", __func__, stamp(),
			             all ? "every contig" : "the contigs where the ties occurred");
		if (all) exact_override(2);
		exact_shutdown(ext);
		exact_init(q->d, ext), ext->exact_mode_of_segs = exact_mode();
		q->n_seg = 0, q->n_arc = 0;
		std::memset((void *)q->seg, 0, sizeof(pg_seg_t) * (size_t)q->m_seg);
		ext->rerun = true;
		++n_attempt;
		if (post_process_impl(opt, q->d) != 0 || run_graph() != 0) q->n_arc = 0;
		if (all) { exact_override(-1); break; }
	}
	if (ext && (!ext->extra_ctgs.empty() || ext->exact_mode_of_segs != exact_mode())) {
		ext->extra_ctgs.clear();
		exact_shutdown(ext);
		exact_init(q->d, ext), ext->exact_mode_of_segs = exact_mode();
	}
	if (ext && !ext->vtx_sel_text.empty()) {
		std::fwrite(ext->vtx_sel_text.data(), 1, ext->vtx_sel_text.size(), out_stream());
		ext->vtx_sel_text.clear();
	}
	g_path_sec += now_sec() - t;
	g_attempts = n_attempt;
	if (std::getenv("PANGENE_TIMING")) {
		std::fprintf(stderr, "[phases]");
		for (int i = 0; i < PH_COUNT; ++i) std::fprintf(stderr, " %s %.2f", pg_phase_name(i), g_phase[i] * 1e3);
		std::fprintf(stderr, " | path %.2f ms (%d attempt%s; pg_post_process %.2f, pg_graph_gen's first attempt %.2f, hazard review %.2f ms)\n", g_path_sec * 1e3, n_attempt, n_attempt > 1 ? "s: tie-order hazards" : "", path_before * 1e3, t_first * 1e3, t_review * 1e3);
		if (ext && ext->ov_calls) std::fprintf(stderr, "[exact_sort] %lld order override(s) of %lld hits in all: lists %.2f ms, backend (copy + kernels + wait) %.2f ms\n", (long long)ext->ov_calls, (long long)ext->ov_hits, ext->ov_list_s * 1e3, ext->ov_backend_s * 1e3);
		if (ext) ext->ov_calls = ext->ov_hits = 0, ext->ov_list_s = ext->ov_backend_s = 0;
	}
}

void pg_graph_destroy(pg_graph_t *q)
{
	if (q == nullptr) return;
	std::free(q->g2s); std::free(q->seg); std::free(q->arc); std::free(q->idx);
	std::free(q);
}

int pg_last_error(void) { return g_err; }
const char *pg_last_error_str(void) { return g_errstr; }
double pg_last_path_seconds(void) { return g_path_sec; }
double pg_last_upload_seconds(void) { return g_upload_sec; }
double pg_last_pack_seconds(void) { return g_pack_sec; }

int pg_backend_is_device(void) { return backend_default()->is_device(); }
int pg_set_device(int32_t device) { const pga_backend_t *be = backend_default(); return be->set_device ? be->set_device(device) : 0; }
int pg_device_count(void) { const pga_backend_t *be = backend_default(); return be->device_count ? be->device_count() : 0; }

int pg_device_warm(void) { const pga_backend_t *be = backend_default(); return be->warm ? be->warm() : 0; }

double pg_device_copy_gbps(size_t bytes, int32_t reps)
{
	const pga_backend_t *be = backend_default();
	double g = -1.0;
	if (be->copy_gbps == nullptr || be->copy_gbps(bytes, reps, &g) != 0) return -1.0;
	return g;
}

void pg_trim_host_cache(size_t keep_bytes) { trim_host_caches(keep_bytes); }

int pg_shard_counts(const pg_data_t *d, int64_t *n_hit, int64_t *n_exon)
{
	DataExt *ext = ext_of(d, false);
	if (ext == nullptr) return PGA_ERR_ARG;
	int64_t h = 0, e = 0;
	for (int32_t j : ext->local_genomes) h += d->genome[j].n_hit, e += d->genome[j].n_exon;
	if (n_hit) *n_hit = h;
	if (n_exon) *n_exon = e;
	return 0;
}

int pg_sync_host(pg_data_t *d) { return sync_host(d, true); }

int pg_phase_times(double *out, int n)
{
	for (int i = 0; i < n && i < PH_COUNT; ++i) out[i] = g_phase[i];
	return PH_COUNT;
}

const char *pg_phase_name(int i)
{
	static const char *nm[PH_COUNT] = { "begin(sort)", "exact_order(host)", "ingest", "post", "vtx", "arc_round(device)", "arc_merge(host)",
	                                    "branch_mark(host)", "n_local", "mark_hits", "flt_high_occ", "sync_host(download)" };
	return i >= 0 && i < PH_COUNT ? nm[i] : "?";
}

int pg_rerun_resident(pg_data_t *d)
{
	DataExt *ext = ext_of(d, false);
	if (ext == nullptr || ext->ctx == nullptr) return PGA_ERR_ARG;
	ext->rerun = true;
	return 0;
}

int pg_kernel_timing(pg_data_t *d, int32_t which, double *total_ms, int64_t *n_launch, int64_t *units)
{
	DataExt *ext = ext_of(d, false);
	if (ext == nullptr || ext->ctx == nullptr || ext->be->timing_get == nullptr) return PGA_ERR_ARG;
	return ext->be->timing_get(ext->ctx, which, total_ms, n_launch, units);
}

int64_t pg_collective_count(void) { return g_n_coll; }

int pg_kernel_timing_reset(pg_data_t *d)
{
	DataExt *ext = ext_of(d, false);
	if (ext == nullptr || ext->ctx == nullptr || ext->be->timing_reset == nullptr) return PGA_ERR_ARG;
	return ext->be->timing_reset(ext->ctx);
}
int64_t pg_last_path_hits(void) { return g_path_hits; }
int pg_last_attempts(void) { return g_attempts; }

double pg_realtime(void)
{
	static double t0 = -1.0;
	const double t = now_sec();
	if (t0 < 0) t0 = t;
	return t - t0;
}

double pg_cputime(void)
{
	struct rusage r;
	getrusage(RUSAGE_SELF, &r);
	return r.ru_utime.tv_sec + r.ru_stime.tv_sec + 1e-6 * (r.ru_utime.tv_usec + r.ru_stime.tv_usec);
}

long pg_peakrss(void)
{
	struct rusage r;
	getrusage(RUSAGE_SELF, &r);
	return r.ru_maxrss * 1024L;
}

void pg_set_exchange(const pg_exchange_t *x)
{
	if (x) g_xchg = *x, g_has_xchg = true;
	else g_has_xchg = false;
}

}
```

pangene_amd/csrc/host/pg_internal.hpp:

```cpp
#pragma once
#include <cstdint>
#include <cstdio>
#include <algorithm>
#include <cstring>
#include <deque>
#include <memory>
#include <mutex>
#include <string>
#include <atomic>
#include <string_view>
#include <thread>
#include <unordered_map>
#include <vector>
#include "pangene_amd.h"
#include "pangene_hip.h"

namespace pgx {

unsigned host_threads(unsigned cap);
inline bool env_word(const char *name, const char *word)
{
	const char *e = std::getenv(name);
	const size_t n = std::strlen(word);
	while (e && *e) { const char *c = std::strchr(e, ','); const size_t len = c ? (size_t)(c - e) : std::strlen(e); if (len == n && std::strncmp(e, word, n) == 0) return true; e = c ? c + 1 : nullptr; }
	return false;
}
bool device_is_up();

class FlatIndex {
public:
	static inline uint64_t hash(std::string_view s) {
		uint64_t h = 0x9E3779B97F4A7C15ull ^ (uint64_t)s.size();
		const char *p = s.data();
		size_t n = s.size();
		for (; n >= 8; p += 8, n -= 8) { uint64_t w; std::memcpy(&w, p, 8); h = (h ^ w) * 0xff51afd7ed558ccdull; h ^= h >> 29; }
		if (n) { uint64_t w = 0; std::memcpy(&w, p, n); h = (h ^ w) * 0xff51afd7ed558ccdull; h ^= h >> 29; }
		return h ^ (h >> 32);
	}
	int32_t size() const { return (int32_t)ptr_.size(); }
	void reserve(size_t n) { ptr_.reserve(n), len_.reserve(n); size_t cap = 16; while (cap < 2 * n + 2) cap <<= 1; if (cap > tab_.size()) rehash(cap); }
	int32_t find(std::string_view s, uint64_t h) const {
		if (tab_.empty()) return -1;
		const size_t mask = tab_.size() - 1;
		for (size_t k = (size_t)h & mask;; k = (k + 1) & mask) {
			const Slot &t = tab_[k];
			if (t.id < 0) return -1;
			if (t.h == (uint32_t)(h >> 32) && len_[(size_t)t.id] == (uint32_t)s.size() && std::memcmp(ptr_[(size_t)t.id], s.data(), s.size()) == 0) return t.id;
		}
	}
	int32_t find(std::string_view s) const { return find(s, hash(s)); }
	int32_t add(const char *stable, size_t len, uint64_t h) {
		if (2 * (ptr_.size() + 1) > tab_.size()) rehash(tab_.empty() ? 16 : tab_.size() * 2);
		const int32_t id = (int32_t)ptr_.size();
		ptr_.push_back(stable), len_.push_back((uint32_t)len), hs_.push_back(h);
		place(h, id);
		return id;
	}
	const char *name(int32_t id) const { return ptr_[(size_t)id]; }
	std::string_view view(int32_t id) const { return std::string_view(ptr_[(size_t)id], len_[(size_t)id]); }
private:
	struct Slot { uint32_t h; int32_t id; };
	void place(uint64_t h, int32_t id) { const size_t mask = tab_.size() - 1; size_t k = (size_t)h & mask; while (tab_[k].id >= 0) k = (k + 1) & mask; tab_[k] = Slot{(uint32_t)(h >> 32), id}; }
	void rehash(size_t cap) { tab_.assign(cap, Slot{0, -1}); for (size_t i = 0; i < ptr_.size(); ++i) place(hs_[i], (int32_t)i); }
	std::vector<Slot> tab_;
	std::vector<const char *> ptr_; std::vector<uint32_t> len_; std::vector<uint64_t> hs_;
};

class NameDict {
public:
	int32_t size() const { return ix_.size(); }
	int32_t get(std::string_view s) const { return ix_.find(s); }
	int32_t put(std::string_view s, bool *absent) {
		const uint64_t h = FlatIndex::hash(s);
		const int32_t id = ix_.find(s, h);
		if (id >= 0) { if (absent) *absent = false; return id; }
		if (absent) *absent = true;
		return ix_.add(keep(s), s.size(), h);
	}
	const char *name(int32_t id) const { return ix_.name(id); }
	std::string_view view(int32_t id) const { return ix_.view(id); }
private:
	const char *keep(std::string_view s) {
		if (s.size() + 1 > left_) {
			const size_t b = std::max<size_t>(s.size() + 1, (size_t)64 << 10);
			blocks_.emplace_back(new char[b]);
			at_ = blocks_.back().get(), left_ = b;
		}
		char *p = at_;
		std::memcpy(p, s.data(), s.size()), p[s.size()] = 0;
		at_ += s.size() + 1, left_ -= s.size() + 1;
		return p;
	}
	FlatIndex ix_;
	std::vector<std::unique_ptr<char[]>> blocks_;
	char *at_ = nullptr; size_t left_ = 0;
};

struct ExactSeg {
	int32_t k = 0, start = 0;
	std::vector<int32_t> file;
	std::vector<uint64_t> cs, cm;
	std::vector<std::vector<int32_t>> hx, hy;
	std::vector<int32_t> heads;
	int cyc_start = -1, period = 0;
	int32_t pushed_id[2] = { -1, -1 };
	std::vector<int32_t> xid, yid;
	bool full = false;
};

struct GenomePack {
	pga_genome_block_t blk{};
	void *buf = nullptr;
	int err = 0;
	uint64_t sig = 0;
	std::vector<int32_t> vfirst, vreal;
	std::vector<int64_t> vbase;
};
struct HostSlab { char *p = nullptr; size_t cap = 0, off = 0; bool pinned = false, fresh = false;
	int pending = 0; bool closed = false, staged = false; };

struct DataExt {
	std::vector<uint8_t> is_local;
	struct HostArena { char *map = nullptr; size_t map_bytes = 0; char *base = nullptr; size_t bytes = 0; std::atomic<size_t> used{0}; };
	std::deque<HostArena> arenas;
	bool arena_owns(const void *p) const { for (const HostArena &a : arenas) if ((const char *)p >= a.base && (const char *)p < a.base + a.bytes) return true; return false; }
	std::vector<uint8_t> hits_sorted;
	const pga_backend_t *be = nullptr;
	pga_ctx_t *ctx = nullptr;
	std::vector<int32_t> local_genomes;
	std::vector<int64_t> hit_off;
	std::vector<std::vector<int32_t>> vreal;
	std::vector<int32_t> n_vctg;
	std::vector<std::vector<int32_t>> y_file;
	std::vector<ExactSeg> xsegs;
	std::vector<int32_t> deg;
	std::vector<int32_t> sc_buf;
	std::vector<uint8_t> del_buf;
	const pga_arc_part_t *cur_arcs = nullptr;
	std::string vtx_sel_text;
	int exact_mode_of_segs = -1;
	const pg_data_t *q_d = nullptr;
	std::vector<std::pair<int32_t, int32_t>> extra_ctgs;
	std::vector<std::pair<int32_t, int32_t>> static_ctgs;
	bool check_strand = false;
	double min_ov_ratio = 0.5;
	std::vector<std::thread> xworkers;
	std::atomic<size_t> xnext{0};
	bool xreplayed = false;
	int32_t xsegs_n_genome = -1;
	uint64_t xsegs_gen = 0;
	int x_sorts[2] = {0, 0};
	std::vector<int32_t> head_file;
	std::vector<int32_t> seg_renumber;
	int route_verbose = -1;
	bool skip_loop_once = false;
	int64_t x_arc_slot = 0;
	int loop_room_retries = 0;
	bool no_branch_loop = false;
	bool arc_via_x = false;
	bool arc_pending = false;
	bool rerun = false;
	bool read_failed = false;
	bool host_full = false;
	bool pos_valid = false;
	bool order_touched = false;
	int64_t ov_calls = 0, ov_hits = 0; double ov_list_s = 0, ov_backend_s = 0;
	uint64_t pos_sig = 0;
	std::vector<uint64_t> flt_bits;
	std::vector<int32_t> pos_x;
	std::vector<std::vector<int32_t>> file_of_host, host_of_file;
	bool host_order_valid = false;
	bool host_stale = false;
	std::vector<GenomePack> packs;
	double pack_sec = 0.0;
	std::vector<HostSlab> slabs;
	std::mutex slab_mu;
	int64_t n_hit_local = 0;
};

DataExt *ext_of(const pg_data_t *d, bool create);
void pack_genomes(const pg_data_t *d, DataExt *ext, int32_t j0, int32_t j1, double time_share = 1.0, bool verify = true);
void trim_host_caches(size_t keep_bytes);
void slab_prefetch(size_t bytes, std::thread *helper);
void free_packs(DataExt *ext, bool wait);
void ext_drop(const pg_data_t *d);

const pga_backend_t *backend_default();

extern pg_exchange_t g_xchg; extern bool g_has_xchg;
void set_error(int code, const char *where);

FILE *out_stream();
int read_lines(const char *fn, std::vector<std::string> &out);
int graph_matrix(pg_graph_t *q, std::vector<std::string> &names, std::vector<int32_t> &mat);
struct GfaMatrix {
	std::vector<std::string> seg, asm_a; std::unordered_map<std::string, int32_t> seg_h; std::vector<int32_t> mat;
	std::vector<int32_t> step, walk_asm; std::vector<int64_t> walk_off;
};
int gfa_matrix(const char *fn, GfaMatrix &m);

int dist_items_file(const char *gfa_fn, int32_t type, std::vector<std::string> &names, std::vector<uint32_t> &bits, int32_t &M, std::vector<std::string> *item_names = nullptr);
int dist_items_graph(pg_graph_t *q, int32_t type, std::vector<std::string> &names, std::vector<uint32_t> &bits, int32_t &M, std::vector<std::string> *item_names = nullptr);
int shared_count(const std::vector<uint32_t> &bits, int32_t M, int32_t A, int32_t *S);
int tree_joins(const std::vector<uint32_t> &bits, int32_t M, int32_t A, int32_t metric, int32_t method, int64_t *rec);
struct Traits { std::vector<std::string> name; std::vector<int8_t> lab; };
int read_traits(const char *fn, const std::vector<std::string> &asm_name, Traits &tr);

double now_sec();
const char *stamp();

int sync_host(pg_data_t *d, bool full);

int exact_mode();
void exact_override(int m);
void exact_init(const pg_data_t *d, DataExt *ext);
void exact_begin(DataExt *ext);
void exact_prefetch(const pg_data_t *d, DataExt *ext);
int exact_sort(DataExt *ext, int by_cm);
void exact_shutdown(DataExt *ext);
bool exact_quiet(DataExt *ext, int n);
void exact_skip(DataExt *ext, int n);
uint64_t order_signature(const DataExt *ext);

enum { PH_BEGIN, PH_EXACT, PH_INGEST, PH_POST, PH_VTX, PH_ARC_DEV, PH_ARC_HOST, PH_BRANCH_HOST, PH_NLOCAL, PH_MARK_HITS, PH_FLT, PH_SYNC_HOST, PH_COUNT };
extern double g_phase[PH_COUNT];
struct Phase { int id; double t0; explicit Phase(int i) : id(i), t0(now_sec()) {} ~Phase() { g_phase[id] += now_sec() - t0; } };

}

#include "pan_common.hpp"
```

Before: 219.0.

## Pick protein representatives on device and defer host readback past vertex stage

Moves per-gene representative selection and joint-pseudogene decisions from the host onto the GPU. A packed gene key is built with atomicMax in k_post_count, and a new k_post_rep kernel writes results into mapped pinned host memory. The post-process stage no longer downloads sums, waits, computes on the CPU and uploads flags; the host fields are filled lazily when gen_vtx or sync_host runs. A tie between two proteins at a gene's largest key falls back to rerunning the host path, which adds complexity and a rare redo cost.

```diff
diff --git a/include/pangene_hip.h b/include/pangene_hip.h
--- a/include/pangene_hip.h
+++ b/include/pangene_hip.h
@@ -42,7 +42,7 @@
 	const int64_t *vbase;
 } pga_genome_block_t;
 
-#define PGA_ABI_VERSION 20u
+#define PGA_ABI_VERSION 21u
 typedef struct {
 	uint32_t abi_version;
 	int32_t n_genome;
@@ -383,6 +383,7 @@
 	int  (*final_arcs)(pga_ctx_t *, const void **, int64_t *);
 	int  (*pan_gainloss)(const pga_gainloss_in_t *, pga_gainloss_out_t *);
 	int  (*pan_coevo)(const pga_coevo_in_t *, pga_coevo_out_t *);
+	int  (*post_front)(pga_ctx_t *, double, int32_t, int32_t, const int32_t **);
 } pga_backend_t;
 
 const pga_backend_t *pga_backend(void);
@@ -411,6 +412,8 @@
 
 int pga_final_arcs(pga_ctx_t *ctx, const void **host_view, int64_t *n_arc);
 
+int pga_post_front(pga_ctx_t *ctx, double min_cnt, int32_t joint_pseudo, int32_t drop_sgl_exon, const int32_t **host_view);
+
 int pga_set_stream(pga_ctx_t *ctx, void *hip_stream);
 void *pga_active_stream(void);
 
diff --git a/pangene_amd/csrc/hip/k_stage_b.hpp b/pangene_amd/csrc/hip/k_stage_b.hpp
--- a/pangene_amd/csrc/hip/k_stage_b.hpp
+++ b/pangene_amd/csrc/hip/k_stage_b.hpp
@@ -51,10 +51,51 @@
 		if (o1) atomicAdd(&sums[(int64_t)5 * P + p], o1);
 	}
 }
-__global__ __launch_bounds__(BLOCK) void k_post_count(unsigned long long *sums, int P)
+__global__ __launch_bounds__(BLOCK) void k_post_count(unsigned long long *sums, int P, const int32_t *prot_gid = nullptr, int Q = 0, unsigned long long *gene_key = nullptr)
 {
 	const int p = blockIdx.x * BLOCK + threadIdx.x;
-	if (p < P) sums[(int64_t)P + p] = sums[(int64_t)2 * P + p] + sums[(int64_t)3 * P + p];
+	if (p >= P) return;
+	const unsigned long long cnt = sums[(int64_t)2 * P + p] + sums[(int64_t)3 * P + p];
+	sums[(int64_t)P + p] = cnt;
+	if (gene_key) {
+		const int g = prot_gid[p];
+		if (g >= 0 && g < Q) atomicMax(&gene_key[g], (sums[p] << 32) + cnt);
+	}
+}
+
+struct PostFront {
+	const unsigned long long *sums; const int32_t *max_ori, *prot_gid; int P, Q;
+	double min_cnt;
+	int joint_pseudo, drop_sgl_exon;
+	const unsigned long long *gene_key; int32_t *gene_rep1 ;
+	uint8_t *rep, *pj;
+	int32_t *host;
+};
+__global__ __launch_bounds__(BLOCK) void k_post_rep(PostFront a)
+{
+	const int p = blockIdx.x * BLOCK + threadIdx.x;
+	if (p >= a.P) return;
+	const int64_t P = a.P;
+	const unsigned long long key = (a.sums[p] << 32) + a.sums[P + p];
+	const int32_t n = (int32_t)(uint32_t)key;
+	const int32_t avg = n ? cvt_i32_x86((double)(key >> 32) / n + .499) : 0;
+	const int g = a.prot_gid[p];
+	bool is_rep = false;
+	if (g >= 0 && g < a.Q && key == a.gene_key[g]) {
+		is_rep = atomicCAS(&a.gene_rep1[g], 0, p + 1) == 0;
+		if (is_rep) a.host[16 + 3 * P + g] = p;
+		else sys_store(&a.host[0], 1);
+	}
+	bool pj = false;
+	if (a.joint_pseudo) {
+		const int32_t ic0 = (int32_t)(long long)a.sums[2 * P + p], ic1 = (int32_t)(long long)a.sums[3 * P + p];
+		const long long s0 = (long long)a.sums[4 * P + p], s1 = (long long)a.sums[5 * P + p];
+		const bool x = ic1 > 0 && (double)ic1 >= a.min_cnt && ((double)s1 / (double)ic1) / ((double)s0 / (double)ic0) >= 0.99;
+		const bool y = (ic1 == 0 || (double)ic1 <= a.min_cnt) && a.drop_sgl_exon;
+		pj = x || y;
+	}
+	a.rep[p] = is_rep, a.pj[p] = pj;
+	a.host[16 + p] = a.max_ori[p], a.host[16 + P + p] = n, a.host[16 + 2 * P + p] = avg;
 }
 
 __global__ __launch_bounds__(BLOCK) void k_post_apply(uint32_t *flags, const int32_t *pid, const int32_t *nex, int32_t *sdom, int n,
diff --git a/pangene_amd/csrc/hip/pga_backend.hip b/pangene_amd/csrc/hip/pga_backend.hip
--- a/pangene_amd/csrc/hip/pga_backend.hip
+++ b/pangene_amd/csrc/hip/pga_backend.hip
@@ -138,7 +138,7 @@
 		"hip-gfx950", pga_create, pga_destroy, pga_begin, pga_ingest, pga_post_partials, pga_post_apply, pga_shadow, pga_set_filter,
 		pga_vtx_partials, pga_flag_vtx, pga_arc_round, pga_arc_merge, pga_arc_set_current, pga_rep_pos, pga_n_local, pga_branch_pairs, pga_branch_decide, pga_mark_hits, pga_override_order, pga_set_head, pga_fetch, pga_put, pga_copy, pga_scratch,
 		pga_download, pga_hazards, pga_is_device, pga_strerror, pga_timing_reset, pga_timing_get, pga_sync, pga_fetch_later, pga_hazard_segs, pga_host_alloc, pga_host_free, pga_arc_round_local, pga_ctg_counts, pga_gene_matrix, pga_arc_table, pga_arc_round_finish, pga_branch_decide_filter, pga_branch_loop, pga_host_trim, pga_set_device, pga_device_count, pga_arc_round_x, pga_copy_gbps, pga_warm, pga_reserve, pga_stage_h2d, pga_stage_drop, pga_call_bubbles, pga_pan_curves, pga_pan_shared, pga_pan_assoc, pga_pan_trait, pga_pan_join, pga_pan_boot, pga_pan_pairs,
-		pga_pan_qtrait, pga_pan_medoids, pga_pan_permanova, pga_pan_mantel, pga_final_arcs, pga_pan_gainloss, pga_pan_coevo
+		pga_pan_qtrait, pga_pan_medoids, pga_pan_permanova, pga_pan_mantel, pga_final_arcs, pga_pan_gainloss, pga_pan_coevo, pga_post_front
 	};
 	return &b;
 }
diff --git a/pangene_amd/csrc/hip/pga_host_common.hpp b/pangene_amd/csrc/hip/pga_host_common.hpp
--- a/pangene_amd/csrc/hip/pga_host_common.hpp
+++ b/pangene_amd/csrc/hip/pga_host_common.hpp
@@ -1,7 +1,7 @@
 #pragma once
 
 
-static int sync_st(pga_ctx *c)
+static int sync_st(pga_ctx *c, double poll_us = 200.0)
 {
 	static const bool poll = [] { const char *e = getenv("PANGENE_WAIT"); return !(e && strcmp(e, "sync") == 0); }();
 	++c->sync_epoch;
@@ -14,7 +14,7 @@
 			__builtin_ia32_pause();
 			if ((it & 0x3f) == 0) {
 				timespec t; clock_gettime(CLOCK_MONOTONIC, &t);
-				if ((t.tv_sec - t0.tv_sec) + (t.tv_nsec - t0.tv_nsec) * 1e-9 > 200e-6) break;
+				if ((t.tv_sec - t0.tv_sec) + (t.tv_nsec - t0.tv_nsec) * 1e-9 > poll_us * 1e-6) break;
 			}
 		}
 	}
diff --git a/pangene_amd/csrc/hip/pga_host_context.hpp b/pangene_amd/csrc/hip/pga_host_context.hpp
--- a/pangene_amd/csrc/hip/pga_host_context.hpp
+++ b/pangene_amd/csrc/hip/pga_host_context.hpp
@@ -128,7 +128,7 @@
 enum {
 	S_KEY_A, S_KEY_B, S_VAL_A, S_VAL_B, S_TABLE, S_TILE, S_I32_A, S_I32_B, S_I32_C, S_TAB_A, S_TAB_B, S_TAB_C, S_TAB_D,
 	S_TDIST, S_TS1, S_TS2, S_TGEN, S_SDIST, S_SS1, S_SS2, S_SGEN, S_HEAD, S_SLOT, S_ARCS, S_SEGCNT, S_BITS, S_TRIPLES,
-	S_WALK_VAL, S_WALK_PREV, S_PERM, S_OVPOS, S_OVFILE, S_RUNSTART, S_CDN, S_MG_KEY, S_MG_VAL, S_MG_SRC, S_MG_OUT, S_MG_HEAD, S_MG_SLOT, S_MG_RUN, S_BR_S1, S_BR_GID, S_BR_VS, S_BR_VE, S_BR_PC, S_BR_POFF, S_BR_GRP, S_BR_NDL, S_BR_SEGGID, S_PAIRS, S_NLCNT, S_ARCX, S_ARCW, S_WEAKNEW, S_RP_SEG, S_RP_R, S_RP_CM, S_RP_POS, S_RP_IV, S_DL, S_SCRATCH, S_UPLOAD, S_RAW, S_ARC_STAGE, S_GMETA, S_GOFF, S_DEG, S_BIGLIST, S_STAGE_SID, S_STATS, S_G2S, S_MISC, S_SLOW, S_HZLIST, S_VWK, S_XG_BUF, S_XG_OUT, S_XG_OUT2, S_XSTAT, S_GSLIST, S_UPLOAD2, S_BINS, S_FIN_ID,
+	S_WALK_VAL, S_WALK_PREV, S_PERM, S_OVPOS, S_OVFILE, S_RUNSTART, S_CDN, S_MG_KEY, S_MG_VAL, S_MG_SRC, S_MG_OUT, S_MG_HEAD, S_MG_SLOT, S_MG_RUN, S_BR_S1, S_BR_GID, S_BR_VS, S_BR_VE, S_BR_PC, S_BR_POFF, S_BR_GRP, S_BR_NDL, S_BR_SEGGID, S_PAIRS, S_NLCNT, S_ARCX, S_ARCW, S_WEAKNEW, S_RP_SEG, S_RP_R, S_RP_CM, S_RP_POS, S_RP_IV, S_DL, S_SCRATCH, S_UPLOAD, S_RAW, S_ARC_STAGE, S_GMETA, S_GOFF, S_DEG, S_BIGLIST, S_STAGE_SID, S_STATS, S_G2S, S_MISC, S_SLOW, S_HZLIST, S_VWK, S_XG_BUF, S_XG_OUT, S_XG_OUT2, S_XSTAT, S_GSLIST, S_UPLOAD2, S_BINS, S_FIN_ID, S_FRONT,
 	S_COUNT
 };
 
@@ -176,6 +176,10 @@
 	int64_t *h_box = 0;
 	void *h_stage = nullptr; size_t h_stage_cap = 0;
 	void *h_fetch = nullptr; size_t h_fetch_cap = 0;
+	int32_t *h_front = nullptr; size_t h_front_cap = 0;
+	bool front_keys_on = true, front_keys_done = false;
+	bool front_live = false; unsigned long long front_epoch = 0;
+	size_t lds_post_set = 0, lds_vtx_set = 0;
 	int32_t *h_g2s = nullptr; size_t h_g2s_cap = 0; hipEvent_t g2s_done = nullptr;
 	DevPool pool; PinArena pin;
 	bool walk_valid = false;
diff --git a/pangene_amd/csrc/hip/pga_host_selftest.hpp b/pangene_amd/csrc/hip/pga_host_selftest.hpp
--- a/pangene_amd/csrc/hip/pga_host_selftest.hpp
+++ b/pangene_amd/csrc/hip/pga_host_selftest.hpp
@@ -172,3 +172,29 @@
 	(void)hipFree(di); (void)hipFree(dout);
 	return 0;
 }
+
+extern "C" int pga_selftest_post_rep(const int64_t *sums, const int32_t *max_ori, const int32_t *prot_gid, int32_t P, int32_t Q, double min_cnt, int32_t joint_pseudo, int32_t drop_sgl_exon,
+                                     int32_t *words, uint8_t *rep, uint8_t *pj)
+{
+	int ndev = 0;
+	if (hipGetDeviceCount(&ndev) != hipSuccess || ndev <= 0) return PGA_ERR_NO_DEVICE;
+	if (P <= 0 || Q <= 0 || !sums || !max_ori || !prot_gid || !words || !rep || !pj) return PGA_ERR_ARG;
+	const size_t nw = 16 + 3 * (size_t)P + (size_t)Q;
+	unsigned long long *d_sums, *d_key; int32_t *d_mx, *d_gid, *d_rep1, *d_words; uint8_t *d_rep;
+	HIPCHK(hipMalloc((void **)&d_sums, sizeof(int64_t) * 6 * (size_t)P)); HIPCHK(hipMalloc((void **)&d_key, sizeof(int64_t) * (size_t)Q));
+	HIPCHK(hipMalloc((void **)&d_mx, sizeof(int32_t) * (size_t)P)); HIPCHK(hipMalloc((void **)&d_gid, sizeof(int32_t) * (size_t)P));
+	HIPCHK(hipMalloc((void **)&d_rep1, sizeof(int32_t) * (size_t)Q));
+	HIPCHK(hipMalloc((void **)&d_words, sizeof(int32_t) * nw)); HIPCHK(hipMalloc((void **)&d_rep, 2 * (size_t)P));
+	HIPCHK(hipMemcpy(d_sums, sums, sizeof(int64_t) * 6 * (size_t)P, hipMemcpyHostToDevice));
+	HIPCHK(hipMemcpy(d_mx, max_ori, sizeof(int32_t) * (size_t)P, hipMemcpyHostToDevice)); HIPCHK(hipMemcpy(d_gid, prot_gid, sizeof(int32_t) * (size_t)P, hipMemcpyHostToDevice));
+	HIPCHK(hipMemset(d_key, 0, sizeof(int64_t) * (size_t)Q)); HIPCHK(hipMemset(d_rep1, 0, sizeof(int32_t) * (size_t)Q));
+	HIPCHK(hipMemset(d_words, 0, sizeof(int32_t) * 16)); HIPCHK(hipMemset(d_words + 16, 0xff, sizeof(int32_t) * (nw - 16)));
+	hipLaunchKernelGGL(k_post_count, dim3(nblk(P)), dim3(BLOCK), 0, 0, d_sums, P, (const int32_t *)d_gid, Q, d_key);
+	PostFront a = { d_sums, d_mx, d_gid, P, Q, min_cnt, joint_pseudo ? 1 : 0, drop_sgl_exon ? 1 : 0, d_key, d_rep1, d_rep, d_rep + P, d_words };
+	hipLaunchKernelGGL(k_post_rep, dim3(nblk(P)), dim3(BLOCK), 0, 0, a);
+	HIPCHK(hipDeviceSynchronize());
+	HIPCHK(hipMemcpy(words, d_words, sizeof(int32_t) * nw, hipMemcpyDeviceToHost));
+	HIPCHK(hipMemcpy(rep, d_rep, (size_t)P, hipMemcpyDeviceToHost)); HIPCHK(hipMemcpy(pj, d_rep + P, (size_t)P, hipMemcpyDeviceToHost));
+	(void)hipFree(d_sums); (void)hipFree(d_key); (void)hipFree(d_mx); (void)hipFree(d_gid); (void)hipFree(d_rep1); (void)hipFree(d_words); (void)hipFree(d_rep);
+	return 0;
+}
diff --git a/pangene_amd/csrc/hip/pga_host_stage_b.hpp b/pangene_amd/csrc/hip/pga_host_stage_b.hpp
--- a/pangene_amd/csrc/hip/pga_host_stage_b.hpp
+++ b/pangene_amd/csrc/hip/pga_host_stage_b.hpp
@@ -1,9 +1,24 @@
 #pragma once
 
 
+struct FrontTabs { unsigned long long *gene_key; int32_t *gene_rep1; uint8_t *rep, *pj; };
+static bool front_tabs(pga_ctx *c, FrontTabs *t)
+{
+	const size_t Q = (size_t)std::max(1, c->Q), P = (size_t)std::max(1, c->P);
+	char *b = (char *)c->pool.get(S_FRONT, 12 * Q + 2 * P + 64);
+	if (!b) return false;
+	t->gene_key = (unsigned long long *)b, t->gene_rep1 = (int32_t *)(b + 8 * Q), t->rep = (uint8_t *)(b + 12 * Q), t->pj = t->rep + P;
+	return true;
+}
+
 extern "C" int pga_post_partials(pga_ctx_t *c, int32_t **max_ori, int64_t **sums)
 {
-	zero_multi(c, c->max_ori, sizeof(int32_t) * (size_t)std::max(1, c->P), c->sums, sizeof(int64_t) * 6 * (size_t)std::max(1, c->P));
+	FrontTabs ft;
+	if (!front_tabs(c, &ft)) return PGA_ERR_NOMEM;
+	const bool keys = c->front_keys_on;
+	c->front_keys_done = keys;
+	zero_multi(c, c->max_ori, sizeof(int32_t) * (size_t)std::max(1, c->P), c->sums, sizeof(int64_t) * 6 * (size_t)std::max(1, c->P),
+	           keys ? ft.gene_key : nullptr, keys ? 12 * (size_t)std::max(1, c->Q) : 0);
 	static const bool pp_atomics = env_has("PANGENE_POST", "atomics");
 	static const bool pp_force = env_has("PANGENE_POST", "lds");
 	bool lds_done = false;
@@ -13,20 +28,21 @@
 		if (p_tiles) {
 			const int PT = (c->P + p_tiles - 1) / p_tiles;
 			const size_t lds = (size_t)PT * 28 + 16;
-			static size_t lds_set = 0;
 			bool ok = true;
-			if (lds > lds_set) { ok = hipFuncSetAttribute(reinterpret_cast<const void *>(k_post_part_lds), hipFuncAttributeMaxDynamicSharedMemorySize, (int)lds) == hipSuccess; if (ok) lds_set = lds; else (void)hipGetLastError(); }
+			if (lds > c->lds_post_set) { ok = hipFuncSetAttribute(reinterpret_cast<const void *>(k_post_part_lds), hipFuncAttributeMaxDynamicSharedMemorySize, (int)lds) == hipSuccess; if (ok) c->lds_post_set = lds; else (void)hipGetLastError(); }
 			if (ok) {
 				const int n_chunk = (int)std::max<int64_t>(1, std::min<int64_t>(c->n_cu, c->N / 32768));
+				(void)hipGetLastError();
 				hipLaunchKernelGGL(k_post_part_lds, dim3((unsigned)(n_chunk * p_tiles)), dim3(PP_T), lds, c->st, c->flags, c->pid, c->rank, c->sori, c->sadj, c->nex, c->N, c->P, p_tiles, PT,
 				                   c->max_ori, (unsigned long long *)c->sums);
-				lds_done = true;
+				lds_done = hipGetLastError() == hipSuccess;
+				if (!lds_done) c->lds_post_set = 0;
 			}
 		}
 	}
 	if (c->N && !lds_done) hipLaunchKernelGGL(k_post_part, dim3(nblk(c->N)), dim3(BLOCK), 0, c->st, c->flags, c->pid, c->rank, c->sori, c->sadj, c->nex, c->N, c->P,
 	                             c->max_ori, (unsigned long long *)c->sums);
-	if (c->N && c->P) hipLaunchKernelGGL(k_post_count, dim3(nblk(c->P)), dim3(BLOCK), 0, c->st, (unsigned long long *)c->sums, c->P);
+	if (c->N && c->P) hipLaunchKernelGGL(k_post_count, dim3(nblk(c->P)), dim3(BLOCK), 0, c->st, (unsigned long long *)c->sums, c->P, (const int32_t *)c->prot_gid, c->Q, keys ? ft.gene_key : (unsigned long long *)nullptr);
 	*max_ori = c->max_ori, *sums = c->sums;
 	return 0;
 }
@@ -34,6 +50,7 @@
 extern "C" int pga_post_apply(pga_ctx_t *c, const uint8_t *prot_rep, const uint8_t *prot_pj, int64_t *n_pseudo)
 {
 	c->yrec_valid = false, c->wrec_valid = false;
+	c->front_keys_on = false;
 	uint8_t *d = (uint8_t *)c->pool.get(S_MISC, 2 * (size_t)c->P + 16);
 	if (!d) return PGA_ERR_NOMEM;
 	c->walk_valid = false, c->ha_valid = false;
@@ -45,6 +62,37 @@
 		TRY(sync_st(c));
 		*n_pseudo = c->h_cnt[2];
 	}
+	return 0;
+}
+
+extern "C" int pga_post_front(pga_ctx_t *c, double min_cnt, int32_t joint_pseudo, int32_t drop_sgl_exon, const int32_t **host_view)
+{
+	FrontTabs ft;
+	if (host_view == nullptr) return PGA_ERR_ARG;
+	if (!front_tabs(c, &ft)) return PGA_ERR_NOMEM;
+	const size_t P = (size_t)c->P, Q = (size_t)c->Q, words = 16 + 3 * P + Q;
+	if (c->front_live && c->front_epoch == c->sync_epoch) TRY(sync_st(c));
+	if (c->h_front_cap < words) {
+		c->h_front = (int32_t *)c->pin.get(sizeof(int32_t) * (words + words / 2) + 256);
+		if (!c->h_front) { c->h_front_cap = 0; return PGA_ERR_NOMEM; }
+		c->h_front_cap = words + words / 2;
+	}
+	memset(c->h_front, 0, sizeof(int32_t) * 16);
+	if (Q) memset(c->h_front + 16 + 3 * P, 0xff, sizeof(int32_t) * Q);
+	int32_t *hd = nullptr;
+	HIPCHK(hipHostGetDevicePointer((void **)&hd, c->h_front, 0));
+	c->yrec_valid = false, c->wrec_valid = false, c->walk_valid = false, c->ha_valid = false;
+	if (!c->front_keys_done) {
+		zero_multi(c, ft.gene_key, 12 * (size_t)std::max(1, c->Q));
+		if (c->N && c->P) hipLaunchKernelGGL(k_post_count, dim3(nblk(c->P)), dim3(BLOCK), 0, c->st, (unsigned long long *)c->sums, c->P, (const int32_t *)c->prot_gid, c->Q, ft.gene_key);
+		c->front_keys_done = true;
+	}
+	c->front_keys_on = true;
+	PostFront a = { (const unsigned long long *)c->sums, c->max_ori, c->prot_gid, c->P, c->Q, min_cnt, joint_pseudo ? 1 : 0, drop_sgl_exon ? 1 : 0, ft.gene_key, ft.gene_rep1, ft.rep, ft.pj, hd };
+	if (c->P) hipLaunchKernelGGL(k_post_rep, dim3(nblk(c->P)), dim3(BLOCK), 0, c->st, a);
+	if (c->N) hipLaunchKernelGGL(k_post_apply, dim3(nblk(c->N)), dim3(BLOCK), 0, c->st, c->flags, c->pid, c->nex, c->sdom, c->N, c->max_ori, (const uint8_t *)ft.rep, (const uint8_t *)ft.pj, (int64_t *)nullptr);
+	c->front_live = true, c->front_epoch = c->sync_epoch;
+	*host_view = c->h_front;
 	return 0;
 }
 
@@ -105,13 +153,16 @@
 		{
 			static const bool vx_atomics = env_has("PANGENE_POST", "atomics"), vx_force = env_has("PANGENE_POST", "lds");
 			const size_t lds = sizeof(int) * 2 * (size_t)std::max(1, Q);
-			static size_t lds_set = 0;
 			bool ok = !vx_atomics && (N >= (1 << 19) || vx_force) && lds <= ((size_t)144 << 10);
-			if (ok && lds > lds_set) { ok = hipFuncSetAttribute(reinterpret_cast<const void *>(k_vtx1_lds), hipFuncAttributeMaxDynamicSharedMemorySize, (int)lds) == hipSuccess; if (ok) lds_set = lds; else (void)hipGetLastError(); }
+			if (ok && lds > c->lds_vtx_set) { ok = hipFuncSetAttribute(reinterpret_cast<const void *>(k_vtx1_lds), hipFuncAttributeMaxDynamicSharedMemorySize, (int)lds) == hipSuccess; if (ok) c->lds_vtx_set = lds; else (void)hipGetLastError(); }
 			if (ok) {
 				const int n_chunk = (int)std::max<int64_t>(1, std::min<int64_t>(2 * c->n_cu, N / 32768));
+				(void)hipGetLastError();
 				hipLaunchKernelGGL(k_vtx1_lds, dim3((unsigned)n_chunk), dim3(VX_T), lds, c->st, c->flags, c->gnm, c->gid, c->rank, c->pdom, N, Q, c->vtx_cnt, bits, wpg, c->dcnt, c->live_cnt);
-			} else
+				ok = hipGetLastError() == hipSuccess;
+				if (!ok) c->lds_vtx_set = 0;
+			}
+			if (!ok)
 			hipLaunchKernelGGL(k_vtx1, dim3(nblk(N)), dim3(BLOCK), 0, c->st, c->flags, c->gnm, c->gid, c->rank, c->pdom, N, Q, c->vtx_cnt, bits, wpg, c->dcnt, c->live_cnt);
 		}
 		hipLaunchKernelGGL(k_live_sum, dim3(1), dim3(BLOCK), 0, c->st, (const int64_t *)c->live_cnt, c->dcnt);
@@ -121,7 +172,8 @@
 		if (!tile) return PGA_ERR_NOMEM;
 		device_scan<I32>(InDomSet{dom_tab}, OutExclI32{slot}, n_slot, tile, OpSum{}, I32{0}, c->st);
 		hipLaunchKernelGGL(k_vtx_compact, dim3(nblk(n_slot)), dim3(BLOCK), 0, c->st, dom_tab, slot, n_slot, pbits, nw, rec, c->dcnt, c->h_box);
-		TRY(sync_st(c));
+		const bool behind_front = c->front_live && c->front_epoch == c->sync_epoch;
+		TRY(sync_st(c, behind_front ? 1000.0 : 200.0));
 		if (c->h_cnt[3]) return PGA_ERR_INVARIANT;
 		c->live_hint = c->h_cnt[8];
 		const int64_t n_rec = c->h_cnt[10], n_ovf = c->h_cnt[0];
diff --git a/pangene_amd/csrc/host/graph_driver.cpp b/pangene_amd/csrc/host/graph_driver.cpp
--- a/pangene_amd/csrc/host/graph_driver.cpp
+++ b/pangene_amd/csrc/host/graph_driver.cpp
@@ -558,10 +558,12 @@
 	return rc;
 }
 
+static int front_settle(pg_data_t *d, DataExt *ext);
 int sync_host(pg_data_t *d, bool full)
 {
 	DataExt *ext = ext_of(d, false);
 	if (ext == nullptr || ext->ctx == nullptr) return g_err;
+	if (front_settle(d, ext) != 0) return g_err;
 	if (!ext->host_stale && !(full && !ext->host_full)) return g_err;
 	Phase ph(PH_SYNC_HOST);
 	const int64_t N = ext->n_hit_local;
@@ -722,6 +724,38 @@
 	return false;
 }
 
+static int post_host_step(const pg_opt_t *opt, pg_data_t *d, DataExt *ext, int32_t *b_max, int64_t *b_sum);
+static int post_process_impl(const pg_opt_t *opt, pg_data_t *d);
+
+static int front_fill(pg_data_t *d, DataExt *ext)
+{
+	ext->front_pending = false;
+	const int32_t *v = ext->front_view;
+	const size_t P = (size_t)d->n_prot;
+	if (v[0] != 0) {
+		ext->front_host = true;
+		if (std::getenv("PANGENE_TIMING")) std::fprintf(stderr, "[front] two proteins of a gene share its largest key: pg_post_process again, representatives on the host\n");
+		return 1;
+	}
+	const int32_t *mx = v + 16, *n = mx + P, *avg = n + P, *rep = avg + P;
+	for (size_t i = 0; i < P; ++i) d->prot[i].max_score_ori = mx[i], d->prot[i].n = n[i], d->prot[i].avg_score_adj = avg[i], d->prot[i].rep = 0;
+	for (int32_t g = 0; g < d->n_gene; ++g) {
+		d->gene[g].rep_pid = rep[g];
+		if (rep[g] >= 0) d->prot[rep[g]].rep = 1;
+	}
+	return 0;
+}
+
+static int front_settle(pg_data_t *d, DataExt *ext)
+{
+	if (!ext->front_pending) return 0;
+	BE_CALL(ext->be->sync(ext->ctx), "sync");
+	if (front_fill(d, ext) == 0) return 0;
+	const pg_opt_t opt = ext->front_opt;
+	ext->rerun = true;
+	return post_process_impl(&opt, d);
+}
+
 static int post_process_impl(const pg_opt_t *opt, pg_data_t *d)
 {
 	DataExt *ext = ext_of(d, true);
@@ -784,6 +818,33 @@
 	BE_CALL(be->post_partials(ctx, &b_max, &b_sum), "post_partials");
 	BE_CALL(xreduce(be, ext->ctx, b_max, P, PG_X_I32, PG_X_MAX), "allreduce(max_score_ori)");
 	BE_CALL(xreduce(be, ext->ctx, b_sum, 6 * (int64_t)P, PG_X_I64, PG_X_SUM), "allreduce(protein sums)");
+	ext->front_pending = false;
+	static const bool front_env_host = env_word("PANGENE_FRONT", "host");
+	const char *why_host = be->post_front == nullptr ? "the backend has no post_front" : front_env_host ? "PANGENE_FRONT=host" : sharded() ? "the sums are reduced across ranks"
+	                     : pg_verbose >= 3 ? "the log counts the pseudogene hits" : ext->front_host ? "a gene of this data set has two proteins at its largest key" : nullptr;
+	if (std::getenv("PANGENE_TIMING")) std::fprintf(stderr, "[front] pg_post_process: representatives on the %s%s%s\n", why_host ? "host: " : "device", why_host ? why_host : "", why_host ? "" : " (nothing fetched, no wait)");
+	if (why_host == nullptr) {
+		BE_CALL(be->post_front(ctx, d->n_genome * opt->min_vertex_ratio, !(opt->flag & PG_F_NO_JOINT_PSEUDO), !!(opt->flag & PG_F_DROP_SGL_EXON), &ext->front_view), "post_front");
+		ext->front_pending = true, ext->front_opt = *opt;
+	} else BE_CALL(post_host_step(opt, d, ext, b_max, b_sum), "post_apply");
+	std::vector<int32_t> st2((size_t)nl * 2);
+	BE_CALL(be->shadow(ctx, 0, pg_verbose >= 3 ? st2.data() : nullptr), "shadow");
+	if (pg_verbose >= 3)
+		for (int32_t k = 0; k < nl; ++k) {
+			const pg_genome_t *g = &d->genome[ext->local_genomes[(size_t)k]];
+			std::fprintf(stderr, "[M::%s::%s] genome[%d]: %s; %d hits remain, of which %d are shadowed\n", __func__, stamp(),
+			             ext->local_genomes[(size_t)k], g->label ? g->label : "-", st2[(size_t)k*2], st2[(size_t)k*2+1]);
+		}
+	ext->host_stale = true;
+	BE_CALL(trace_state(ext, "post_process", 0), "trace");
+	return 0;
+}
+
+static int post_host_step(const pg_opt_t *opt, pg_data_t *d, DataExt *ext, int32_t *b_max, int64_t *b_sum)
+{
+	const pga_backend_t *be = ext->be;
+	pga_ctx_t *ctx = ext->ctx;
+	const int32_t P = d->n_prot;
 	static thread_local std::vector<int32_t> mx;
 	static thread_local std::vector<int64_t> sm;
 	mx.resize((size_t)P), sm.resize((size_t)P * 6);
@@ -829,17 +890,7 @@
 	int64_t n_pj = 0;
 	BE_CALL(be->post_apply(ctx, rep.data(), pj.data(), (!(opt->flag & PG_F_NO_JOINT_PSEUDO) && pg_verbose >= 3) ? &n_pj : nullptr), "post_apply");
 	if (!(opt->flag & PG_F_NO_JOINT_PSEUDO) && pg_verbose >= 3)
-		std::fprintf(stderr, "[M::%s::%s] %ld pseudogene hits identified jointly\n", __func__, stamp(), (long)n_pj);
-	std::vector<int32_t> st2((size_t)nl * 2);
-	BE_CALL(be->shadow(ctx, 0, pg_verbose >= 3 ? st2.data() : nullptr), "shadow");
-	if (pg_verbose >= 3)
-		for (int32_t k = 0; k < nl; ++k) {
-			const pg_genome_t *g = &d->genome[ext->local_genomes[(size_t)k]];
-			std::fprintf(stderr, "[M::%s::%s] genome[%d]: %s; %d hits remain, of which %d are shadowed\n", __func__, stamp(),
-			             ext->local_genomes[(size_t)k], g->label ? g->label : "-", st2[(size_t)k*2], st2[(size_t)k*2+1]);
-		}
-	ext->host_stale = true;
-	BE_CALL(trace_state(ext, "post_process", 0), "trace");
+		std::fprintf(stderr, "[M::%s::%s] %ld pseudogene hits identified jointly\n", "post_process_impl", stamp(), (long)n_pj);
 	return 0;
 }
 
@@ -861,6 +912,7 @@
 			q->idx[q->arc[i0].x >> 32] = (uint64_t)i0 << 32 | (uint32_t)(i - i0), i0 = i;
 }
 
+enum { RC_FRONT_TIE = 1001 };
 static int gen_vtx(const pg_opt_t *opt, pg_graph_t *q, DataExt *ext)
 {
 	pg_data_t *d = q->d;
@@ -870,6 +922,7 @@
 	int32_t *b_cnt; uint64_t *b_tri; int64_t n_tri;
 	const double tv0 = now_sec();
 	BE_CALL(be->vtx_partials(ext->ctx, &b_cnt, &b_tri, &n_tri), "vtx_partials");
+	if (ext->front_pending && front_fill(d, ext) != 0) return RC_FRONT_TIE;
 	const double tv1 = now_sec();
 	BE_CALL(xreduce(be, ext->ctx, b_cnt, 2 * (int64_t)Q, PG_X_I32, PG_X_SUM), "allreduce(n_dom,n_sub)");
 	static thread_local std::vector<int32_t> cntv;
@@ -954,9 +1007,11 @@
 	}
 	if (std::getenv("PANGENE_TIMING")) std::fprintf(stderr, "[vtx] partials %.3f ms, fetch %.3f ms (records %ld / %ld), greedy %.3f ms\n", (tv1 - tv0) * 1e3, (tv2 - tv1) * 1e3, (long)n_tri, (long)n_rec, (now_sec() - tv2) * 1e3);
 	{
-		std::vector<int32_t> at((size_t)Q, -1);
+		static thread_local std::vector<int32_t> at;
+		static thread_local std::vector<pg_seg_t> tmp;
+		at.assign((size_t)Q, -1);
 		for (int32_t i = 0; i < q->n_seg; ++i) at[(size_t)q->seg[i].gid] = i;
-		std::vector<pg_seg_t> tmp(q->seg, q->seg + q->n_seg);
+		tmp.assign(q->seg, q->seg + q->n_seg);
 		int32_t k = 0;
 		for (int32_t g = 0; g < Q; ++g) if (at[(size_t)g] >= 0) q->seg[k++] = tmp[(size_t)at[(size_t)g]];
 	}
@@ -1322,7 +1377,11 @@
 	pga_ctx_t *ctx = ext->ctx;
 	ext->arc_pending = false;
 	BE_CALL(be->set_filter(ctx, PGA_FLT_PSEUDO), "set_filter");
-	BE_CALL(gen_vtx(opt, q, ext), "gen_vtx");
+	{
+		const int rc = gen_vtx(opt, q, ext);
+		if (rc == RC_FRONT_TIE) return rc;
+		BE_CALL(rc, "gen_vtx");
+	}
 	if (!exact_early(ext)) { Phase ph(PH_EXACT); BE_CALL(exact_sort(ext, 0), "set_head"); }
 	BE_CALL(flag_vtx(q, ext), "flag_vtx");
 	BE_CALL(trace_state(ext, "gen_vtx+flag_vtx", 0), "trace");
@@ -1511,15 +1570,17 @@
 	DataExt *ext = ext_of(q->d, false);
 	if (ext) ext->q_d = q->d;
 	auto run_graph = [&]() {
-		int rc = graph_gen_impl(opt, q);
-		if (rc == RC_REDO && ext) {
-			if (pg_verbose >= 2) std::fprintf(stderr, "[M::%s::%s] the queued branch rounds met a case they leave to the host: repeating stages A-C with host-driven rounds\n", "pg_graph_gen", stamp());
+		auto again = [&](const char *why) {
+			if (pg_verbose >= 2) std::fprintf(stderr, "[M::%s::%s] %s\n", "pg_graph_gen", stamp(), why);
 			q->n_seg = 0, q->n_arc = 0;
 			std::memset((void *)q->seg, 0, sizeof(pg_seg_t) * (size_t)q->m_seg);
 			ext->rerun = true;
-			rc = post_process_impl(opt, q->d);
-			if (rc == 0) rc = graph_gen_impl(opt, q);
-		}
+			const int rc = post_process_impl(opt, q->d);
+			return rc ? rc : graph_gen_impl(opt, q);
+		};
+		int rc = graph_gen_impl(opt, q);
+		if (rc == RC_FRONT_TIE && ext) rc = again("a gene has two proteins at its largest key: repeating stages A-C with the representatives picked on the host");
+		if (rc == RC_REDO && ext) rc = again("the queued branch rounds met a case they leave to the host: repeating stages A-C with host-driven rounds");
 		return rc;
 	};
 	if (g_err == 0 && run_graph() != 0) q->n_arc = 0;
diff --git a/pangene_amd/csrc/host/pg_internal.hpp b/pangene_amd/csrc/host/pg_internal.hpp
--- a/pangene_amd/csrc/host/pg_internal.hpp
+++ b/pangene_amd/csrc/host/pg_internal.hpp
@@ -171,6 +171,10 @@
 	std::vector<std::vector<int32_t>> file_of_host, host_of_file;
 	bool host_order_valid = false;
 	bool host_stale = false;
+	bool front_pending = false;
+	const int32_t *front_view = nullptr;
+	bool front_host = false;
+	pg_opt_t front_opt;
 	std::vector<GenomePack> packs;
 	double pack_sec = 0.0;
 	std::vector<HostSlab> slabs;
```

After: 226.5, median of 6. 3.4% higher.
